# quadram-institute-bioscience/uvaia

Hardware: AMD Instinct MI355X
Metric: ref-seqs scored/sec (higher is better)
Workload: dtype u32 bit-planes / int32 counts

## Files before the change

### include/uvaia_gpu.h

```cpp
#ifndef UVAIA_GPU_H
#define UVAIA_GPU_H

#include <stddef.h>
#include <stdint.h>

#ifdef __cplusplus
extern "C" {
#endif

#define UVAIA_GPU_NSCORE 6

enum {
  UVAIA_GPU_OK         =  0,
  UVAIA_GPU_EINVAL     = -1,
  UVAIA_GPU_ENODEV     = -2,
  UVAIA_GPU_ENOMEM     = -3,
  UVAIA_GPU_EHIP       = -4,
  UVAIA_GPU_EALPHABET  = -5,
  UVAIA_GPU_ESTATE     = -6
};

typedef struct uvaia_gpu_ctx uvaia_gpu_ctx;

typedef struct {
  int n_query;
  int nchar;
  const char *const *seq;
  const char *consensus;
  const size_t *idx_c, *idx_m, *idx;
  int n_idx_c, n_idx_m, n_idx;
  size_t trim;
  int acgt;
} uvaia_gpu_query;

int uvaia_gpu_open (uvaia_gpu_ctx **ctx, const uvaia_gpu_query *query, int heap_size, int device, size_t max_pool);

enum { UVAIA_GPU_SCAN_AUTO = 0,
       UVAIA_GPU_SCAN_PACKED = 1,
       UVAIA_GPU_SCAN_COMPRESSED = 2,
       UVAIA_GPU_SCAN_WIDE = 3 };
typedef struct {
  size_t subslice_refs;
  int rare_max;
  int scan;
  int serial;
  int scan_tiles_per_wave;
  int scan_waves_per_block;
  int rederive_streams;
  int ball_gather;
  int query_tables;
  int replay_extras;
  int replay_cus;
  int scan_streams;
  int pipeline;
  int head_scan;
} uvaia_gpu_tuning;
int uvaia_gpu_export_query_table (uvaia_gpu_ctx *ctx, int which, void *out, size_t cap, size_t *n_bytes);
int uvaia_gpu_open_tuned (uvaia_gpu_ctx **ctx, const uvaia_gpu_query *query, int heap_size, int device, size_t max_pool, const uvaia_gpu_tuning *tuning );
void uvaia_gpu_close (uvaia_gpu_ctx *ctx);
const char *uvaia_gpu_last_error (const uvaia_gpu_ctx *ctx);

int uvaia_gpu_push (uvaia_gpu_ctx *ctx, const char *const *seq, const int *non_n, int n_ref, int64_t ordinal0,
                    uint8_t *entered);

int uvaia_gpu_drain (uvaia_gpu_ctx *ctx, int *n_items, int *max_incompatible, int *scores, int64_t *ordinals);
int uvaia_gpu_heap_slots (const uvaia_gpu_ctx *ctx);
int uvaia_gpu_n_query (const uvaia_gpu_ctx *ctx);
int uvaia_gpu_reset (uvaia_gpu_ctx *ctx);

int uvaia_gpu_db_reserve (uvaia_gpu_ctx *ctx, size_t n_ref_capacity);
int uvaia_gpu_db_append (uvaia_gpu_ctx *ctx, const char *const *seq, const int *non_n, int n_ref);
int uvaia_gpu_db_append_block (uvaia_gpu_ctx *ctx, const char *rows, size_t pitch, const int *non_n, int n_ref);
size_t uvaia_gpu_db_size (const uvaia_gpu_ctx *ctx);
int uvaia_gpu_search_resident (uvaia_gpu_ctx *ctx, size_t pool, int64_t ordinal0, uint8_t *entered);
int uvaia_gpu_sync (uvaia_gpu_ctx *ctx);

size_t uvaia_gpu_state_bytes (const uvaia_gpu_ctx *ctx);
int uvaia_gpu_state_export (uvaia_gpu_ctx *ctx, void *dst);
int uvaia_gpu_state_import (uvaia_gpu_ctx *ctx, const void *src);
int uvaia_gpu_slice_scan (uvaia_gpu_ctx *ctx, size_t first, size_t n, int buf);
int uvaia_gpu_slice_replay (uvaia_gpu_ctx *ctx, int buf, int64_t ordinal0, int stripe_start);
int uvaia_gpu_slice_buffers (void);
size_t uvaia_gpu_state_range_bytes (const uvaia_gpu_ctx *ctx, int q0, int q1);
int uvaia_gpu_state_export_range (uvaia_gpu_ctx *ctx, void *dst, int q0, int q1);
int uvaia_gpu_state_import_range (uvaia_gpu_ctx *ctx, const void *src, int q0, int q1);
int uvaia_gpu_slice_replay_range (uvaia_gpu_ctx *ctx, int buf, int64_t ordinal0, int q0, int q1, int take_snapshot);
int uvaia_gpu_entered_flags (uvaia_gpu_ctx *ctx, uint8_t *out, int clear);

int uvaia_gpu_ball (uvaia_gpu_ctx *ctx, const char *const *seq, int n_ref, int radius, int *mindist);
int uvaia_gpu_ball_resident (uvaia_gpu_ctx *ctx, size_t first, size_t n, int radius, int *mindist);
int uvaia_gpu_ball_packed (uvaia_gpu_ctx *ctx, const void *planes, int n_ref, int radius, int *mindist);
int uvaia_gpu_unpack_rows (uvaia_gpu_ctx *ctx, const int *index, int n, char *rows, size_t pitch);
unsigned long long uvaia_gpu_ball_asked (uvaia_gpu_ctx *ctx, int reset);
void uvaia_gpu_ball_kernel_ms (uvaia_gpu_ctx *ctx, double out[3], int reset);

int uvaia_gpu_agree_on_polymorphic (uvaia_gpu_ctx *ctx, const char *const *seq, int n_seq, uint8_t *out);

int uvaia_gpu_query_columns (const char *const *seq, int n_query, int nchar, size_t trim, int acgt, int device, char *consensus, unsigned char *some_missing);

int uvaia_gpu_last_batch_scores (uvaia_gpu_ctx *ctx, int *out, int n_ref);
int uvaia_gpu_scan_stats (uvaia_gpu_ctx *ctx, double *ms, long long *launches, double *algorithmic_bytes, int reset);
int uvaia_gpu_replay_stats (uvaia_gpu_ctx *ctx, unsigned long long out[3], int reset);
int uvaia_gpu_replay_tiles_opened (uvaia_gpu_ctx *ctx, unsigned long long *out, int reset);
int uvaia_gpu_replay_timing (uvaia_gpu_ctx *ctx, unsigned long long out[12], int reset);
int uvaia_gpu_set_query_tile (uvaia_gpu_ctx *ctx, int qt);
int uvaia_gpu_set_active_queries (uvaia_gpu_ctx *ctx, int q0, int q1);
int uvaia_gpu_max_tolerance (uvaia_gpu_ctx *ctx, int *out);
int uvaia_gpu_search_resident_pool (uvaia_gpu_ctx *ctx, size_t first, size_t n, int64_t ordinal0, int snapshot);

int uvaia_gpu_db_set_shard (uvaia_gpu_ctx *ctx, int rank, int world, size_t piece_refs);
int uvaia_gpu_shard_rows (const uvaia_gpu_ctx *ctx);
size_t uvaia_gpu_shard_aux_bytes (const uvaia_gpu_ctx *ctx, size_t n_tiles);
int uvaia_gpu_shard_scan (uvaia_gpu_ctx *ctx, size_t first, size_t n, void *cnt, void *tmin, void *aux);
int uvaia_gpu_db_skip (uvaia_gpu_ctx *ctx, size_t n_ref);
int uvaia_gpu_shard_set_peer (uvaia_gpu_ctx *ctx, int rank, const void *planes, const void *side_rows);
const void *uvaia_gpu_shard_planes (const uvaia_gpu_ctx *ctx);
const void *uvaia_gpu_shard_side_rows (const uvaia_gpu_ctx *ctx);
int uvaia_gpu_shard_ipc_handle_bytes (void);
int uvaia_gpu_shard_ipc_handles (uvaia_gpu_ctx *ctx, void *out );
int uvaia_gpu_shard_ipc_open (uvaia_gpu_ctx *ctx, int rank, const void *handles);
int uvaia_gpu_shard_ipc_close (uvaia_gpu_ctx *ctx);
int uvaia_gpu_scan_wait (uvaia_gpu_ctx *ctx);
int uvaia_gpu_replay_wait (uvaia_gpu_ctx *ctx);
int uvaia_gpu_set_snapshot (uvaia_gpu_ctx *ctx, int snapshot);
enum { UVAIA_GPU_SCANS = 0, UVAIA_GPU_REPLAYS = 1 };
int uvaia_gpu_mark (uvaia_gpu_ctx *ctx, int what, int slot);
int uvaia_gpu_stream_wait_mark (uvaia_gpu_ctx *ctx, void *stream, int slot);
int uvaia_gpu_wait_stream (uvaia_gpu_ctx *ctx, int what, void *stream);
int uvaia_gpu_shard_replay (uvaia_gpu_ctx *ctx, const void *cnt, const void *tmin, const void *aux, int owner, size_t first, size_t n, int64_t ordinal0, int q0, int q1);

typedef struct uvaia_gpu_group uvaia_gpu_group;
int  uvaia_gpu_group_open (uvaia_gpu_group **group, const uvaia_gpu_query *query, int heap_size, const int *devices, int n_devices, size_t max_pool, size_t piece_refs);
void uvaia_gpu_group_close (uvaia_gpu_group *group);
const char *uvaia_gpu_group_last_error (const uvaia_gpu_group *group);
int  uvaia_gpu_group_size (const uvaia_gpu_group *group);
uvaia_gpu_ctx *uvaia_gpu_group_member (uvaia_gpu_group *group, int i);
int  uvaia_gpu_group_query_shard (const uvaia_gpu_group *group, int i, int *q0, int *q1);
int  uvaia_gpu_group_db_reserve (uvaia_gpu_group *group, size_t n_ref_capacity);
int  uvaia_gpu_group_db_append (uvaia_gpu_group *group, const char *const *seq, const int *non_n, int n_ref);
int  uvaia_gpu_group_db_append_packed (uvaia_gpu_group *group, const void *planes, const int *non_n, const int *side_rows, int n_ref);
int  uvaia_gpu_group_db_clear (uvaia_gpu_group *group);
int  uvaia_gpu_group_db_rederive (uvaia_gpu_group *group);
size_t uvaia_gpu_group_db_size (const uvaia_gpu_group *group);
int  uvaia_gpu_group_reset (uvaia_gpu_group *group);
int  uvaia_gpu_group_search_resident (uvaia_gpu_group *group, size_t pool, int64_t ordinal0, uint8_t *entered);
int  uvaia_gpu_group_push (uvaia_gpu_group *group, const char *const *seq, const int *non_n, int n_ref, int64_t ordinal0, uint8_t *entered);
int  uvaia_gpu_group_drain (uvaia_gpu_group *group, int *n_items, int *max_incompatible, int *scores, int64_t *ordinals);
int  uvaia_gpu_group_sync (uvaia_gpu_group *group);

size_t uvaia_gpu_db_tile_bytes (const uvaia_gpu_ctx *ctx);
int    uvaia_gpu_db_clear (uvaia_gpu_ctx *ctx);
int    uvaia_gpu_db_rederive (uvaia_gpu_ctx *ctx);
int    uvaia_gpu_db_side_row_ints (void);
int    uvaia_gpu_db_export (uvaia_gpu_ctx *ctx, size_t first_tile, size_t n_tiles, void *planes, int *non_n, int *side_rows);
int    uvaia_gpu_db_append_packed (uvaia_gpu_ctx *ctx, const void *planes, const int *non_n, const int *side_rows, int n_ref);

int uvaia_gpu_db_stage_reserve (uvaia_gpu_ctx *ctx, size_t n_tiles);
int uvaia_gpu_db_stage_packed (uvaia_gpu_ctx *ctx, int slot, const void *planes, const int *non_n, const int *side_rows, int n_tiles);
int uvaia_gpu_db_load_staged (uvaia_gpu_ctx *ctx, int slot, const int *sel, int n_ref);
int uvaia_gpu_db_stage_packed_at (uvaia_gpu_ctx *ctx, int slot, size_t tile_offset, const void *planes, const int *non_n, const int *side_rows, int n_tiles);
int uvaia_gpu_db_append_staged (uvaia_gpu_ctx *ctx, int slot, const int *sel, int n_ref);
int uvaia_gpu_db_unpack_rows (uvaia_gpu_ctx *ctx, const int *index, int n, char *rows, size_t pitch);
void uvaia_gpu_window_ms (uvaia_gpu_ctx *ctx, double out[3], int reset);
size_t uvaia_gpu_free_bytes (uvaia_gpu_ctx *ctx);

int uvaia_gpu_rows_census (uvaia_gpu_ctx *ctx, const void *d_rows, size_t pitch, int n, int *non_n, int *n_exc);
int uvaia_gpu_db_append_device (uvaia_gpu_ctx *ctx, const void *d_rows, size_t pitch, const int *row_index, int n_sel, const int *non_n);
int uvaia_gpu_rows_exceptions (uvaia_gpu_ctx *ctx, const void *d_rows, size_t pitch, const int *row_index, int n_sel, const uint64_t *offsets, void *exc_out);
int uvaia_gpu_db_drop_tiles (uvaia_gpu_ctx *ctx, size_t n_tiles);
void uvaia_gpu_rows_kernel_ms (uvaia_gpu_ctx *ctx, double out[3], int reset);
int uvaia_gpu_rows_set_run_cut (uvaia_gpu_ctx *ctx, unsigned cut);

size_t uvaia_gpu_scan_bytes_per_ref (const uvaia_gpu_ctx *ctx);
int uvaia_gpu_scan_variant (const uvaia_gpu_ctx *ctx);
size_t uvaia_gpu_derived_bytes_per_ref (const uvaia_gpu_ctx *ctx);
size_t uvaia_gpu_packed_bytes_per_ref (const uvaia_gpu_ctx *ctx);

#ifdef __cplusplus
}
#endif
#endif
```

### uvaia_amd/capi.py

```python
import ctypes as C
import os
import subprocess

import numpy as np

_HERE = os.path.dirname(os.path.abspath(__file__))
ROOT = os.path.dirname(_HERE)
_LIB = os.path.join(_HERE, "lib", "libuvaia_gpu.so")
NSCORE = 6

SYMBOLS = [
    "uvaia_gpu_open", "uvaia_gpu_open_tuned", "uvaia_gpu_close", "uvaia_gpu_last_error", "uvaia_gpu_push", "uvaia_gpu_drain",
    "uvaia_gpu_heap_slots", "uvaia_gpu_n_query", "uvaia_gpu_reset", "uvaia_gpu_db_reserve", "uvaia_gpu_db_append",
    "uvaia_gpu_db_append_block", "uvaia_gpu_db_size", "uvaia_gpu_search_resident", "uvaia_gpu_sync", "uvaia_gpu_ball", "uvaia_gpu_ball_resident", "uvaia_gpu_ball_packed", "uvaia_gpu_unpack_rows", "uvaia_gpu_ball_asked", "uvaia_gpu_ball_kernel_ms", "uvaia_gpu_export_query_table", "uvaia_gpu_agree_on_polymorphic", "uvaia_gpu_query_columns",
    "uvaia_gpu_last_batch_scores", "uvaia_gpu_scan_stats", "uvaia_gpu_replay_stats", "uvaia_gpu_replay_tiles_opened", "uvaia_gpu_replay_timing",
    "uvaia_gpu_state_bytes", "uvaia_gpu_state_export", "uvaia_gpu_state_import", "uvaia_gpu_slice_scan", "uvaia_gpu_slice_replay",
    "uvaia_gpu_entered_flags", "uvaia_gpu_state_range_bytes", "uvaia_gpu_state_export_range", "uvaia_gpu_state_import_range",
    "uvaia_gpu_slice_replay_range", "uvaia_gpu_slice_buffers", "uvaia_gpu_scan_bytes_per_ref", "uvaia_gpu_derived_bytes_per_ref", "uvaia_gpu_scan_variant", "uvaia_gpu_set_query_tile", "uvaia_gpu_packed_bytes_per_ref",
    "uvaia_gpu_db_tile_bytes", "uvaia_gpu_db_side_row_ints", "uvaia_gpu_db_export", "uvaia_gpu_db_append_packed", "uvaia_gpu_db_clear", "uvaia_gpu_db_rederive",
    "uvaia_gpu_set_active_queries", "uvaia_gpu_max_tolerance", "uvaia_gpu_search_resident_pool",
    "uvaia_gpu_db_set_shard", "uvaia_gpu_shard_rows", "uvaia_gpu_shard_scan", "uvaia_gpu_scan_wait", "uvaia_gpu_replay_wait", "uvaia_gpu_set_snapshot", "uvaia_gpu_shard_replay",
    "uvaia_gpu_mark", "uvaia_gpu_stream_wait_mark", "uvaia_gpu_wait_stream",
    "uvaia_gpu_shard_aux_bytes", "uvaia_gpu_db_skip", "uvaia_gpu_shard_set_peer", "uvaia_gpu_shard_planes", "uvaia_gpu_shard_side_rows",
    "uvaia_gpu_shard_ipc_handle_bytes", "uvaia_gpu_shard_ipc_handles", "uvaia_gpu_shard_ipc_open", "uvaia_gpu_shard_ipc_close",
    "uvaia_gpu_group_open", "uvaia_gpu_group_close", "uvaia_gpu_group_last_error", "uvaia_gpu_group_size", "uvaia_gpu_group_member", "uvaia_gpu_group_query_shard",
    "uvaia_gpu_group_db_reserve", "uvaia_gpu_group_db_append", "uvaia_gpu_group_db_append_packed", "uvaia_gpu_group_db_clear", "uvaia_gpu_group_db_rederive",
    "uvaia_gpu_group_db_size", "uvaia_gpu_group_reset", "uvaia_gpu_group_search_resident", "uvaia_gpu_group_push", "uvaia_gpu_group_drain", "uvaia_gpu_group_sync",
    "uvaia_gpu_rows_census", "uvaia_gpu_db_append_device", "uvaia_gpu_rows_exceptions", "uvaia_gpu_db_drop_tiles", "uvaia_gpu_rows_kernel_ms", "uvaia_gpu_rows_set_run_cut",
    "uvaia_gpu_db_stage_reserve", "uvaia_gpu_db_stage_packed", "uvaia_gpu_db_load_staged", "uvaia_gpu_db_unpack_rows", "uvaia_gpu_window_ms", "uvaia_gpu_free_bytes",
    "uvaia_gpu_db_stage_packed_at", "uvaia_gpu_db_append_staged",
]


class GpuError(RuntimeError):
    def __init__(self, code, msg):
        super().__init__("uvaia_gpu error %d: %s" % (code, msg))
        self.code = code


class Tuning(C.Structure):
    _fields_ = [("subslice_refs", C.c_size_t), ("rare_max", C.c_int), ("scan", C.c_int), ("serial", C.c_int),
                ("scan_tiles_per_wave", C.c_int), ("scan_waves_per_block", C.c_int), ("rederive_streams", C.c_int), ("ball_gather", C.c_int), ("query_tables", C.c_int), ("replay_extras", C.c_int), ("replay_cus", C.c_int), ("scan_streams", C.c_int), ("pipeline", C.c_int), ("head_scan", C.c_int)]

    SCAN = {"auto": 0, "packed": 1, "compressed": 2, "wide": 3}

    @classmethod
    def make(cls, tuning):
        if tuning is None or isinstance(tuning, cls):
            return tuning
        t = cls()
        for k, v in tuning.items():
            setattr(t, k, cls.SCAN[v] if k == "scan" and isinstance(v, str) else int(v))
        return t


class _Query(C.Structure):
    _fields_ = [
        ("n_query", C.c_int), ("nchar", C.c_int),
        ("seq", C.POINTER(C.c_char_p)), ("consensus", C.c_char_p),
        ("idx_c", C.POINTER(C.c_size_t)), ("idx_m", C.POINTER(C.c_size_t)), ("idx", C.POINTER(C.c_size_t)),
        ("n_idx_c", C.c_int), ("n_idx_m", C.c_int), ("n_idx", C.c_int),
        ("trim", C.c_size_t), ("acgt", C.c_int),
    ]


def library_path():
    return _LIB


def build_library(force=False):
    csrc = os.path.join(_HERE, "csrc")
    srcs = [os.path.join(csrc, f) for f in os.listdir(csrc) if f.endswith((".hip", ".inc"))] + [os.path.join(ROOT, "include", "uvaia_gpu.h")]
    if not force and os.path.exists(_LIB) and os.path.getmtime(_LIB) >= max(os.path.getmtime(f) for f in srcs):
        return _LIB
    subprocess.check_call(["make", "-C", os.path.join(_HERE, "csrc"), "-s"])
    return _LIB


_lib = None


def load_library():
    global _lib
    if _lib is not None:
        return _lib
    if not os.path.exists(_LIB):
        raise GpuError(-2, "HIP library %s is missing: run __graft_entry__.build() (no CPU fallback exists)" % _LIB)
    L = C.CDLL(_LIB)
    vp = C.c_void_p
    pp = C.POINTER(C.c_char_p)
    pi = C.POINTER(C.c_int)
    sig = {
        "uvaia_gpu_open": (C.c_int, [C.POINTER(vp), C.POINTER(_Query), C.c_int, C.c_int, C.c_size_t]),
        "uvaia_gpu_open_tuned": (C.c_int, [C.POINTER(vp), C.POINTER(_Query), C.c_int, C.c_int, C.c_size_t, C.POINTER(Tuning)]),
        "uvaia_gpu_close": (None, [vp]),
        "uvaia_gpu_last_error": (C.c_char_p, [vp]),
        "uvaia_gpu_push": (C.c_int, [vp, pp, pi, C.c_int, C.c_int64, C.POINTER(C.c_uint8)]),
        "uvaia_gpu_drain": (C.c_int, [vp, pi, pi, pi, C.POINTER(C.c_int64)]),
        "uvaia_gpu_heap_slots": (C.c_int, [vp]),
        "uvaia_gpu_n_query": (C.c_int, [vp]),
        "uvaia_gpu_reset": (C.c_int, [vp]),
        "uvaia_gpu_db_reserve": (C.c_int, [vp, C.c_size_t]),
        "uvaia_gpu_db_append": (C.c_int, [vp, pp, pi, C.c_int]),
        "uvaia_gpu_db_append_block": (C.c_int, [vp, C.c_void_p, C.c_size_t, pi, C.c_int]),
        "uvaia_gpu_db_size": (C.c_size_t, [vp]),
        "uvaia_gpu_search_resident": (C.c_int, [vp, C.c_size_t, C.c_int64, C.POINTER(C.c_uint8)]),
        "uvaia_gpu_sync": (C.c_int, [vp]),
        "uvaia_gpu_ball": (C.c_int, [vp, pp, C.c_int, C.c_int, pi]),
        "uvaia_gpu_ball_resident": (C.c_int, [vp, C.c_size_t, C.c_size_t, C.c_int, pi]),
        "uvaia_gpu_ball_packed": (C.c_int, [vp, C.c_void_p, C.c_int, C.c_int, pi]),
        "uvaia_gpu_unpack_rows": (C.c_int, [vp, pi, C.c_int, C.c_void_p, C.c_size_t]),
        "uvaia_gpu_ball_asked": (C.c_ulonglong, [vp, C.c_int]),
        "uvaia_gpu_ball_kernel_ms": (None, [vp, C.POINTER(C.c_double), C.c_int]),
        "uvaia_gpu_export_query_table": (C.c_int, [vp, C.c_int, vp, C.c_size_t, C.POINTER(C.c_size_t)]),
        "uvaia_gpu_agree_on_polymorphic": (C.c_int, [vp, pp, C.c_int, C.POINTER(C.c_uint8)]),
        "uvaia_gpu_query_columns": (C.c_int, [pp, C.c_int, C.c_int, C.c_size_t, C.c_int, C.c_int, C.c_char_p, C.POINTER(C.c_uint8)]),
        "uvaia_gpu_last_batch_scores": (C.c_int, [vp, pi, C.c_int]),
        "uvaia_gpu_scan_stats": (C.c_int, [vp, C.POINTER(C.c_double), C.POINTER(C.c_longlong), C.POINTER(C.c_double), C.c_int]),
        "uvaia_gpu_replay_stats": (C.c_int, [vp, C.POINTER(C.c_ulonglong), C.c_int]),
        "uvaia_gpu_replay_tiles_opened": (C.c_int, [vp, C.POINTER(C.c_ulonglong), C.c_int]),
        "uvaia_gpu_replay_timing": (C.c_int, [vp, C.POINTER(C.c_ulonglong), C.c_int]),
        "uvaia_gpu_state_bytes": (C.c_size_t, [vp]),
        "uvaia_gpu_state_export": (C.c_int, [vp, C.c_void_p]),
        "uvaia_gpu_state_import": (C.c_int, [vp, C.c_void_p]),
        "uvaia_gpu_slice_scan": (C.c_int, [vp, C.c_size_t, C.c_size_t, C.c_int]),
        "uvaia_gpu_slice_replay": (C.c_int, [vp, C.c_int, C.c_int64, C.c_int]),
        "uvaia_gpu_entered_flags": (C.c_int, [vp, C.POINTER(C.c_uint8), C.c_int]),
        "uvaia_gpu_state_range_bytes": (C.c_size_t, [vp, C.c_int, C.c_int]),
        "uvaia_gpu_state_export_range": (C.c_int, [vp, C.c_void_p, C.c_int, C.c_int]),
        "uvaia_gpu_state_import_range": (C.c_int, [vp, C.c_void_p, C.c_int, C.c_int]),
        "uvaia_gpu_slice_replay_range": (C.c_int, [vp, C.c_int, C.c_int64, C.c_int, C.c_int, C.c_int]),
        "uvaia_gpu_slice_buffers": (C.c_int, []),
        "uvaia_gpu_scan_bytes_per_ref": (C.c_size_t, [vp]),
        "uvaia_gpu_derived_bytes_per_ref": (C.c_size_t, [vp]),
        "uvaia_gpu_scan_variant": (C.c_int, [vp]),
        "uvaia_gpu_set_query_tile": (C.c_int, [vp, C.c_int]),
        "uvaia_gpu_packed_bytes_per_ref": (C.c_size_t, [vp]),
        "uvaia_gpu_set_active_queries": (C.c_int, [vp, C.c_int, C.c_int]),
        "uvaia_gpu_max_tolerance": (C.c_int, [vp, pi]),
        "uvaia_gpu_search_resident_pool": (C.c_int, [vp, C.c_size_t, C.c_size_t, C.c_int64, C.c_int]),
        "uvaia_gpu_db_tile_bytes": (C.c_size_t, [vp]),
        "uvaia_gpu_db_clear": (C.c_int, [vp]),
        "uvaia_gpu_db_rederive": (C.c_int, [vp]),
        "uvaia_gpu_db_side_row_ints": (C.c_int, []),
        "uvaia_gpu_db_export": (C.c_int, [vp, C.c_size_t, C.c_size_t, C.c_void_p, pi, pi]),
        "uvaia_gpu_db_append_packed": (C.c_int, [vp, C.c_void_p, pi, pi, C.c_int]),
        "uvaia_gpu_db_set_shard": (C.c_int, [vp, C.c_int, C.c_int, C.c_size_t]),
        "uvaia_gpu_shard_rows": (C.c_int, [vp]),
        "uvaia_gpu_shard_scan": (C.c_int, [vp, C.c_size_t, C.c_size_t, C.c_void_p, C.c_void_p, C.c_void_p]),
        "uvaia_gpu_shard_aux_bytes": (C.c_size_t, [vp, C.c_size_t]), "uvaia_gpu_db_skip": (C.c_int, [vp, C.c_size_t]),
        "uvaia_gpu_shard_set_peer": (C.c_int, [vp, C.c_int, C.c_void_p, C.c_void_p]),
        "uvaia_gpu_shard_planes": (C.c_void_p, [vp]), "uvaia_gpu_shard_side_rows": (C.c_void_p, [vp]),
        "uvaia_gpu_shard_ipc_handle_bytes": (C.c_int, []), "uvaia_gpu_shard_ipc_handles": (C.c_int, [vp, C.c_void_p]),
        "uvaia_gpu_shard_ipc_open": (C.c_int, [vp, C.c_int, C.c_void_p]), "uvaia_gpu_shard_ipc_close": (C.c_int, [vp]),
        "uvaia_gpu_scan_wait": (C.c_int, [vp]),
        "uvaia_gpu_replay_wait": (C.c_int, [vp]),
        "uvaia_gpu_set_snapshot": (C.c_int, [vp, C.c_int]),
        "uvaia_gpu_shard_replay": (C.c_int, [vp, C.c_void_p, C.c_void_p, C.c_void_p, C.c_int, C.c_size_t, C.c_size_t, C.c_int64, C.c_int, C.c_int]),
        "uvaia_gpu_mark": (C.c_int, [vp, C.c_int, C.c_int]), "uvaia_gpu_stream_wait_mark": (C.c_int, [vp, C.c_void_p, C.c_int]),
        "uvaia_gpu_wait_stream": (C.c_int, [vp, C.c_int, C.c_void_p]),
        "uvaia_gpu_group_open": (C.c_int, [C.POINTER(vp), C.POINTER(_Query), C.c_int, pi, C.c_int, C.c_size_t, C.c_size_t]),
        "uvaia_gpu_group_close": (None, [vp]),
        "uvaia_gpu_group_last_error": (C.c_char_p, [vp]),
        "uvaia_gpu_group_size": (C.c_int, [vp]),
        "uvaia_gpu_group_member": (vp, [vp, C.c_int]),
        "uvaia_gpu_group_query_shard": (C.c_int, [vp, C.c_int, pi, pi]),
        "uvaia_gpu_group_db_reserve": (C.c_int, [vp, C.c_size_t]),
        "uvaia_gpu_group_db_append": (C.c_int, [vp, pp, pi, C.c_int]),
        "uvaia_gpu_group_db_append_packed": (C.c_int, [vp, C.c_void_p, pi, pi, C.c_int]),
        "uvaia_gpu_group_db_clear": (C.c_int, [vp]),
        "uvaia_gpu_group_db_rederive": (C.c_int, [vp]),
        "uvaia_gpu_group_db_size": (C.c_size_t, [vp]),
        "uvaia_gpu_group_reset": (C.c_int, [vp]),
        "uvaia_gpu_group_search_resident": (C.c_int, [vp, C.c_size_t, C.c_int64, C.POINTER(C.c_uint8)]),
        "uvaia_gpu_group_push": (C.c_int, [vp, pp, pi, C.c_int, C.c_int64, C.POINTER(C.c_uint8)]),
        "uvaia_gpu_group_drain": (C.c_int, [vp, pi, pi, pi, C.POINTER(C.c_int64)]),
        "uvaia_gpu_group_sync": (C.c_int, [vp]),
        "uvaia_gpu_rows_census": (C.c_int, [vp, C.c_void_p, C.c_size_t, C.c_int, pi, pi]),
        "uvaia_gpu_db_append_device": (C.c_int, [vp, C.c_void_p, C.c_size_t, pi, C.c_int, pi]),
        "uvaia_gpu_rows_exceptions": (C.c_int, [vp, C.c_void_p, C.c_size_t, pi, C.c_int, C.POINTER(C.c_uint64), C.c_void_p]),
        "uvaia_gpu_db_drop_tiles": (C.c_int, [vp, C.c_size_t]),
        "uvaia_gpu_rows_kernel_ms": (None, [vp, C.POINTER(C.c_double), C.c_int]),
        "uvaia_gpu_rows_set_run_cut": (C.c_int, [vp, C.c_uint]),
        "uvaia_gpu_db_stage_reserve": (C.c_int, [vp, C.c_size_t]),
        "uvaia_gpu_db_stage_packed": (C.c_int, [vp, C.c_int, C.c_void_p, pi, pi, C.c_int]),
        "uvaia_gpu_db_load_staged": (C.c_int, [vp, C.c_int, pi, C.c_int]),
        "uvaia_gpu_db_stage_packed_at": (C.c_int, [vp, C.c_int, C.c_size_t, C.c_void_p, pi, pi, C.c_int]),
        "uvaia_gpu_db_append_staged": (C.c_int, [vp, C.c_int, pi, C.c_int]),
        "uvaia_gpu_db_unpack_rows": (C.c_int, [vp, pi, C.c_int, C.c_void_p, C.c_size_t]),
        "uvaia_gpu_window_ms": (None, [vp, C.POINTER(C.c_double), C.c_int]),
        "uvaia_gpu_free_bytes": (C.c_size_t, [vp]),
    }
    for name, (res, args) in sig.items():
        fn = getattr(L, name)
        fn.restype, fn.argtypes = res, args
    _lib = L
# ... 361 lines not shown
        self._staged[int(slot)] = (planes, non_n, side_rows)
        self._chk(self.L.uvaia_gpu_db_stage_packed(self.ctx, int(slot), planes.ctypes.data, non_n.ctypes.data_as(C.POINTER(C.c_int)),
                                                   side_rows.ctypes.data_as(C.POINTER(C.c_int)), int(n_tiles)))

    def db_load_staged(self, slot, sel, n_ref):
        _k, sp = _int_ptr(sel)
        self._chk(self.L.uvaia_gpu_db_load_staged(self.ctx, int(slot), sp, int(n_ref)))

    def db_stage_packed_at(self, slot, tile_offset, planes, non_n, side_rows, n_tiles):
        planes = np.ascontiguousarray(planes, dtype=np.uint8)
        non_n = np.ascontiguousarray(non_n, dtype=np.int32)
        side_rows = np.ascontiguousarray(side_rows, dtype=np.int32)
        tb = self.L.uvaia_gpu_db_tile_bytes(self.ctx)
        if planes.size < int(n_tiles) * tb or non_n.size < int(n_tiles) * 64 or side_rows.size < int(n_tiles) * 64 * self.L.uvaia_gpu_db_side_row_ints():
            raise ValueError("arrays shorter than %d tiles" % n_tiles)
        if not hasattr(self, "_staged_at"):
            self._staged_at = {}
        if int(tile_offset) == 0:
            self._staged_at[int(slot)] = []
        self._staged_at.setdefault(int(slot), []).append((planes, non_n, side_rows))
        self._chk(self.L.uvaia_gpu_db_stage_packed_at(self.ctx, int(slot), int(tile_offset), planes.ctypes.data, non_n.ctypes.data_as(C.POINTER(C.c_int)),
                                                      side_rows.ctypes.data_as(C.POINTER(C.c_int)), int(n_tiles)))

    def db_append_staged(self, slot, sel, n_ref):
        _k, sp = _int_ptr(sel)
        self._chk(self.L.uvaia_gpu_db_append_staged(self.ctx, int(slot), sp, int(n_ref)))

    def db_unpack_rows(self, index, pitch=None):
        idx = np.ascontiguousarray(index, dtype=np.int32)
        pitch = (self.nchar + 15) // 16 * 16 if pitch is None else int(pitch)
        rows = np.zeros((max(len(idx), 1), pitch), dtype=np.uint8)
        self._chk(self.L.uvaia_gpu_db_unpack_rows(self.ctx, idx.ctypes.data_as(C.POINTER(C.c_int)), len(idx), rows.ctypes.data, pitch))
        return [rows[k, :self.nchar].tobytes() for k in range(len(idx))]

    def window_ms(self, reset=False):
        out = (C.c_double * 3)()
        self.L.uvaia_gpu_window_ms(self.ctx, out, int(reset))
        return tuple(out)

    def free_bytes(self):
        return int(self.L.uvaia_gpu_free_bytes(self.ctx))

    def ball_asked(self, reset=False):
        return int(self.L.uvaia_gpu_ball_asked(self.ctx, int(reset)))

    def query_table(self, which):
        n = C.c_size_t(0)
        self._chk(self.L.uvaia_gpu_export_query_table(self.ctx, int(which), None, 0, C.byref(n)))
        out = np.zeros(n.value, dtype=np.uint8)
        if n.value:
            self._chk(self.L.uvaia_gpu_export_query_table(self.ctx, int(which), out.ctypes.data_as(C.c_void_p), n.value, C.byref(n)))
        return out

    def ball_kernel_ms(self, reset=False):
        out = (C.c_double * 3)()
        self.L.uvaia_gpu_ball_kernel_ms(self.ctx, out, int(reset))
        return tuple(out)


def finalise_heaps(n, scores, ordinals):
    out = []
    for q in range(len(n)):
        k = int(n[q])
        order = ([k] + list(range(1, k))) if k else []
        rows = [(tuple(int(x) for x in scores[q, s]), int(ordinals[q, s])) for s in order]
        rows.sort(key=lambda r: tuple(-v for v in r[0]))
        out.append(rows)
    return out


class Group:

    def __init__(self, q, devices, nbest=100, max_pool=4096, piece_refs=0):
        self.L = load_library()
        self.nq, self.nchar = len(q.seqs), len(q.consensus)
        self._keep = [_cstrs(q.seqs), q.consensus,
                      (C.c_size_t * len(q.idx_c))(*[int(x) for x in q.idx_c]),
                      (C.c_size_t * len(q.idx_m))(*[int(x) for x in q.idx_m]),
                      (C.c_size_t * len(q.idx))(*[int(x) for x in q.idx])]
        qq = _Query(self.nq, self.nchar, self._keep[0], q.consensus, self._keep[2], self._keep[3], self._keep[4],
                    len(q.idx_c), len(q.idx_m), len(q.idx), int(q.trim), int(bool(q.acgt)))
        self.g = C.c_void_p()
        dev = (C.c_int * len(devices))(*[int(d) for d in devices])
        rc = self.L.uvaia_gpu_group_open(C.byref(self.g), C.byref(qq), int(nbest), dev, len(devices), int(max_pool), int(piece_refs))
        if rc != 0:
            msg = self.L.uvaia_gpu_group_last_error(None)
            self.g = None
            raise GpuError(rc, msg.decode() if msg else "?")
        self.slots = self.L.uvaia_gpu_heap_slots(self.L.uvaia_gpu_group_member(self.g, 0))

    def _chk(self, rc):
        if rc != 0:
            msg = self.L.uvaia_gpu_group_last_error(self.g)
            raise GpuError(rc, msg.decode() if msg else "?")

    def close(self):
        if getattr(self, "g", None):
            self.L.uvaia_gpu_group_close(self.g)
            self.g = None

    def __enter__(self):
        return self

    def __exit__(self, *a):
        self.close()

# ... 68 lines not shown
```

### uvaia_amd/csrc/host_batch.inc

```

extern "C" {

int uvaia_gpu_agree_on_polymorphic(uvaia_gpu_ctx *c, const char *const *seq, int n_seq, uint8_t *out)
{
  if (!c) return UVAIA_GPU_EINVAL;
  if (n_seq < 0 || (n_seq > 0 && (!seq || !out))) return fail(c, UVAIA_GPU_EINVAL, "bad batch");
  if ((size_t)n_seq > c->max_pool) return fail(c, UVAIA_GPU_ESTATE, "batch of %d exceeds max_pool %zu", n_seq, c->max_pool);
  if (n_seq == 0) return 0;
  int rc = ensure_batch_buffers(c); if (rc) return rc;
  rc = pack_rows(c, seq, nullptr, 0, nullptr, n_seq, c->batch, 0);
  if (rc) return rc;
  const int n_tiles = (n_seq + 63) / 64, ppad = n_tiles * 64;
  rc = ensure_cnt4(c, (size_t)c->nq_pad * c->pool_pad); if (rc) return rc;
  const bool prof = c->profile; c->profile = false;
  rc = ensure_qpoly(c); if (rc) return rc;
  rc = launch_scan(c, c->batch, 0, n_tiles, c->d_qpoly, c->nq, c->d_cnt, ppad, 0.0);
  c->profile = prof;
  if (rc) return rc;
  uint8_t *d_out = nullptr;
  const size_t bytes = (size_t)n_seq * c->nq;
  HIPCHK(c, hipMalloc(&d_out, bytes));
  dim3 grid((n_seq + 255) / 256, c->nq);
  if (c->acgt) hipLaunchKernelGGL((agree_kernel<true>), grid, dim3(256), 0, c->stream, c->d_cnt, ppad, c->nq, n_seq, d_out);
  else         hipLaunchKernelGGL((agree_kernel<false>), grid, dim3(256), 0, c->stream, c->d_cnt, ppad, c->nq, n_seq, d_out);
// ... 35 lines not shown
  QCHK(hipMalloc(&d_first, (size_t)nchar)); QCHK(hipMalloc(&d_flags, (size_t)nchar));
  QCHK(hipMemsetAsync(d_first, 'N', (size_t)nchar, st)); QCHK(hipMemsetAsync(d_flags, 0, (size_t)nchar, st));
  for (int i = 0; i < 2; i++) QCHK(hipEventCreateWithFlags(&freed[i], hipEventDisableTiming));
  const unsigned gx = (unsigned)((hi - lo + 255) / 256);
  int k = 0;
  for (int a = 0; a < n_query; a += batch, k++) {
    const int m = std::min(batch, n_query - a), b = k & 1;
    if (k >= 2) QCHK(hipEventSynchronize(freed[b]));
    uint8_t *hb = h_rows + (size_t)b * batch * pitch, *db = d_rows + (size_t)b * batch * pitch;
    for (int i = 0; i < m; i++) if (!seq[a + i]) return done(fail(nullptr, UVAIA_GPU_EINVAL, "query %d is NULL", a + i));
    parallel_for(m, [&](int i) { memcpy(hb + (size_t)i * pitch, seq[a + i], (size_t)nchar); });
    QCHK(hipMemcpyAsync(db, hb, (size_t)m * pitch, hipMemcpyHostToDevice, st));
    const int ng = (m + 63) / 64;
    hipLaunchKernelGGL(query_columns_partial_kernel, dim3(gx, (unsigned)ng), dim3(256), 0, st, db, pitch, m, lo, hi, acgt ? 1 : 0, d_pf, d_pl, nchar);
    hipLaunchKernelGGL(query_columns_merge_kernel, dim3(gx), dim3(256), 0, st, d_pf, d_pl, ng, lo, hi, nchar, d_first, d_flags);
    QCHK(hipGetLastError());
    QCHK(hipEventRecord(freed[b], st));
  }
  std::vector<uint8_t> first((size_t)nchar), flags((size_t)nchar);
  QCHK(hipMemcpyAsync(first.data(), d_first, (size_t)nchar, hipMemcpyDeviceToHost, st));
  QCHK(hipMemcpyAsync(flags.data(), d_flags, (size_t)nchar, hipMemcpyDeviceToHost, st));
  QCHK(hipStreamSynchronize(st));
#undef QCHK
  for (int c = lo; c < hi; c++) {
    consensus[c] = (flags[(size_t)c] & 1) ? '#' : (char)first[(size_t)c];
    some_missing[c] = (flags[(size_t)c] & 2) ? 1 : 0;
  }
  return done(0);
}

int uvaia_gpu_push(uvaia_gpu_ctx *c, const char *const *seq, const int *non_n, int n_ref, int64_t ordinal0, uint8_t *entered)
{
  if (!c) return UVAIA_GPU_EINVAL;
  if (n_ref < 0 || (n_ref > 0 && !seq)) return fail(c, UVAIA_GPU_EINVAL, "bad batch");
  if ((size_t)n_ref > c->max_pool) return fail(c, UVAIA_GPU_ESTATE, "batch of %d exceeds max_pool %zu", n_ref, c->max_pool);
  if (c->act_q0 != 0 || c->act_q1 != c->nq) return fail(c, UVAIA_GPU_ESTATE, "streamed batches act on the whole query set: query shards use the resident calls");
  if (n_ref == 0) return 0;
  int rc = ensure_batch_buffers(c); if (rc) return rc;
  rc = pack_rows(c, seq, nullptr, 0, non_n, n_ref, c->batch, 0);
  if (rc) return rc;
  const int n_tiles = (n_ref + 63) / 64;
  HIPCHK(c, hipMemsetAsync(c->d_entered, 0, (size_t)n_tiles * 64, c->stream));
  rc = run_batch(c, c->batch, 0, n_tiles, 0, n_ref, ordinal0);
  if (rc) return rc;
  if (entered) HIPCHK(c, hipMemcpyAsync(entered, c->d_entered, (size_t)n_ref, hipMemcpyDeviceToHost, c->stream));
  HIPCHK(c, hipStreamSynchronize(c->stream));
  return collect_events(c);
}

int uvaia_gpu_drain(uvaia_gpu_ctx *c, int *n_items, int *max_incompatible, int *scores, int64_t *ordinals)
{
  if (!c || !n_items || !scores || !ordinals) return c ? fail(c, UVAIA_GPU_EINVAL, "NULL output") : UVAIA_GPU_EINVAL;
  HIPCHK(c, hipStreamSynchronize(c->stream));
  const size_t ne = (size_t)c->nq * (c->k + 1);
  std::vector<int> h(ne * HEAP_ENTRY), T(c->nq);
  HIPCHK(c, hipMemcpy(h.data(), c->d_heap, h.size() * sizeof(int), hipMemcpyDeviceToHost));
  HIPCHK(c, hipMemcpy(n_items, c->d_n, (size_t)c->nq * sizeof(int), hipMemcpyDeviceToHost));
  HIPCHK(c, hipMemcpy(T.data(), c->d_T, (size_t)c->nq * sizeof(int), hipMemcpyDeviceToHost));
  for (size_t e = 0; e < ne; e++) {
    for (int s = 0; s < 6; s++) scores[e * 6 + s] = h[e * HEAP_ENTRY + s];
    ordinals[e] = (int64_t)(((uint64_t)(uint32_t)h[e * HEAP_ENTRY + 7] << 32) | (uint32_t)h[e * HEAP_ENTRY + 6]);
  }
  if (max_incompatible) memcpy(max_incompatible, T.data(), (size_t)c->nq * sizeof(int));
  return collect_events(c);
}


}
```

### uvaia_amd/csrc/host_launch.inc

```

namespace {

template <class F>
static void parallel_for(int n, F f)
{
  const unsigned nt = std::min<unsigned>(std::max(1u, std::thread::hardware_concurrency()), 64u);
  if (n < 32 || nt < 2) { for (int i = 0; i < n; i++) f(i); return; }
  std::atomic<int> next(0);
  std::vector<std::thread> th;
  for (unsigned t = 0; t < nt; t++) th.emplace_back([&]() { for (;;) { const int a = next.fetch_add(4); if (a >= n) break; for (int i = a; i < std::min(n, a + 4); i++) f(i); } });
  for (auto &x : th) x.join();
}

__global__ void mask_query_planes_kernel(const uint32_t *__restrict__ qp, const uint32_t *__restrict__ pmask, uint32_t *__restrict__ out, size_t n_words_total, int words_per_row, int nq_planes)
{
  const size_t i = (size_t)blockIdx.x * blockDim.x + threadIdx.x;
  if (i >= n_words_total) return;
  const int w = (int)((i / (size_t)nq_planes) % (size_t)words_per_row);
  out[i] = qp[i] & pmask[w];
}

int ensure_qpoly(uvaia_gpu_ctx *c)
{
  if (c->d_qpoly) return 0;
// ... 78 lines not shown
int store_alloc(uvaia_gpu_ctx *c, TileStore &s, size_t tiles)
{
  store_free(s);
  uint4 *planes = nullptr;
  const size_t refs = tiles * 64, tile_u4 = (size_t)c->W4 * c->P * 64;
  HIPCHK(c, hipMalloc(&s.nonn, refs * sizeof(int)));
  HIPCHK(c, hipMemset(s.nonn, 0, refs * sizeof(int)));
  HIPCHK(c, hipMalloc(&s.ev, tiles * (size_t)c->W4 * 2 * 64 * sizeof(uint4)));
  HIPCHK(c, hipMalloc(&s.grp, tiles * (size_t)c->W4 * 64 * sizeof(uint32_t)));
  HIPCHK(c, hipMalloc(&s.poly, tiles * (size_t)std::max(c->NP4 + c->NR4, 1) * 3 * 64 * sizeof(uint4)));
  HIPCHK(c, hipMalloc(&s.tote, refs * sizeof(int)));
  HIPCHK(c, hipMalloc(&s.tot, refs * sizeof(int)));
  HIPCHK(c, hipMemset(s.tot, 0, refs * sizeof(int)));
  HIPCHK(c, hipMalloc(&s.amb, refs * AMB_ROW * sizeof(int)));
  HIPCHK(c, hipMemset(s.amb, 0, refs * AMB_ROW * sizeof(int)));
  HIPCHK(c, hipMalloc(&planes, tiles * tile_u4 * sizeof(uint4)));
  HIPCHK(c, hipMemset(planes, 0, tiles * tile_u4 * sizeof(uint4)));
  s.planes = planes;
  return 0;
}

int ensure_batch_buffers(uvaia_gpu_ctx *c)
{
  if (c->batch.planes) return 0;
  HIPCHK(c, hipSetDevice(c->device));
  return store_alloc(c, c->batch, c->pool_pad / 64);
}

int pack_query_row(const uint8_t *code_tab, const char *row, int nchar, int lo, int hi, const uint8_t *keep, const uint8_t *is_poly,
                   bool acgt, int NQ, uint32_t *dst, int *bad_byte)
{
  for (int s = lo; s < hi; s++) {
    if (keep && !keep[s]) continue;
    const uint8_t code = code_tab[(unsigned char)row[s]];
    if (code == 0xFF) { *bad_byte = (unsigned char)row[s]; return -1; }
    if (!code) continue;
    const int w = s >> 5, b = s & 31;
    uint32_t *d = dst + (size_t)w * NQ;
    const bool one = (code & (code - 1)) == 0;
    if (acgt) {
      if (!one) continue;
      const uint32_t two = code == 2 ? 1u : code == 4 ? 2u : code == 8 ? 3u : 0u;
      d[0] |= (two & 1u) << b; d[1] |= (two >> 1) << b; d[2] |= 1u << b;
      if (is_poly && is_poly[s]) d[3] |= 1u << b;
    } else {
      for (int p = 0; p < 4; p++) d[p] |= (uint32_t)((code >> p) & 1u) << b;
      d[4] |= 1u << b;
      if (one) d[5] |= 1u << b;
    }
  }
  return 0;
}

int take_scan_events(uvaia_gpu_ctx *c, ScanEvt &ev)
{
  for (hipEvent_t *e : {&ev.a, &ev.b}) {
    if (!c->ev_pool.empty()) { *e = c->ev_pool.back(); c->ev_pool.pop_back(); }
    else HIPCHK(c, hipEventCreate(e));
  }
  return 0;
}

int launch_scan(uvaia_gpu_ctx *c, const TileStore &s, long long tile_first, int n_tiles, const uint32_t *qp, int n_rows, int4 *out, int ppad, double bytes)
{
  if (n_tiles <= 0) return 0;
  dim3 grid((unsigned)((n_rows + c->qt - 1) / c->qt), (unsigned)((n_tiles + 3) / 4)), block(256);
  ScanEvt ev{};
  if (c->profile) {
    { int rc_ = take_scan_events(c, ev); if (rc_) return rc_; }
    HIPCHK(c, hipEventRecord(ev.a, c->stream));
  }
#define LAUNCH(K, QT) hipLaunchKernelGGL((K<QT>), grid, block, 0, c->stream, s.planes, tile_first, n_tiles, c->W4, qp, out, ppad)
  if (c->acgt) { switch (c->qt) { case 8: LAUNCH(scan_acgt_kernel, 8); break; case 32: LAUNCH(scan_acgt_kernel, 32); break; default: LAUNCH(scan_acgt_kernel, 16); } }
  else         { switch (c->qt) { case 8: LAUNCH(scan_iupac_kernel, 8); break; case 32: LAUNCH(scan_iupac_kernel, 32); break; default: LAUNCH(scan_iupac_kernel, 16); } }
#undef LAUNCH
  HIPCHK(c, hipGetLastError());
  if (c->profile) { HIPCHK(c, hipEventRecord(ev.b, c->stream)); ev.bytes = bytes; c->evts.push_back(ev); }
  return 0;
}

int launch_pair_extras(uvaia_gpu_ctx *c, const TileStore &s, long long tile_first, int n_tiles, uint32_t *ext, int ppad, hipStream_t stream)
{
  if (n_tiles <= 0) return 0;
  hipLaunchKernelGGL(pair_extras_kernel, dim3((unsigned)n_tiles, (unsigned)((c->nq + 15) / 16)), dim3(256), 0, stream, s.planes, tile_first, n_tiles, c->W4,
                     s.amb, c->d_qp, c->d_amb_q, c->nq, ext, ppad);
  HIPCHK(c, hipGetLastError());
  return 0;
}

int launch_scan2(uvaia_gpu_ctx *c, const TileStore &s, long long tile_first, int n_tiles, uint32_t *out, int ppad, double bytes, hipStream_t stream,
                 int2 *tmin, int r_lo, int r_hi, int4 *rt, uint32_t *ext = nullptr , uint32_t *rtp = nullptr, uint4 *tb8 = nullptr,
                 unsigned *progress = nullptr )
{
  if (n_tiles <= 0) return 0;
  if (!stream) stream = c->stream;
  const bool cons = c->n_idx_c > 0;
  if (cons && !rt) return fail(c, UVAIA_GPU_ESTATE, "no buffer for the consensus pre-score");
  const uint4 *tiles = s.planes; const int *tot_tile0 = s.tot + tile_first * 64;
  const long long ptile_first = tile_first;
  auto consensus_rt = [&]() {
    if (!cons) return;
    if (c->acgt) hipLaunchKernelGGL((consensus_rt_kernel<true>), dim3((n_tiles + 3) / 4), dim3(256), 0, stream, tiles, ptile_first, n_tiles, c->W4, c->d_cp, rt);
    else         hipLaunchKernelGGL((consensus_rt_kernel<false>), dim3((n_tiles + 3) / 4), dim3(256), 0, stream, tiles, ptile_first, n_tiles, c->W4, c->d_cp, rt);
  };
  const int qt2 = c->qt != 8 ? 16 : c->nq <= 1 ? 1 : c->nq <= 2 ? 2 : c->nq <= 4 ? 4 : 8;
  const int n_qtiles = (c->nq + qt2 - 1) / qt2;
  dim3 grid(scan_grid_size(n_qtiles, n_tiles)), block(256);
  ScanEvt ev_{};
  if (c->profile) {
    { int rc_ = take_scan_events(c, ev_); if (rc_) return rc_; }
    HIPCHK(c, hipEventRecord(ev_.a, stream));
  }
  const uint32_t *qp = c->acgt ? c->d_qp : c->d_qp2;
  if (c->scan_variant == 2) {
    const int *tote = s.tote + tile_first * 64;
    constexpr int QS = 64;
    if (c->act_q0 % QS) return fail(c, UVAIA_GPU_ESTATE, "the scan works on super-tiles of %d queries: active queries start at a multiple of that", QS);
    const int st_first = c->act_q0 / QS, n_st = (c->act_q1 + QS - 1) / QS - st_first;
    const int R = c->scan_R;
    dim3 grid3(scan_grid_size(n_st, (n_tiles + R - 1) / R));
#define SCAN3_LAUNCH(NWW, A, RR) hipLaunchKernelGGL((scan3_kernel<NWW, A, RR>), grid3, dim3(64 * NWW), 0, stream, s.ev, s.poly, tile_first, n_tiles, c->W4, c->NP4, c->NP4 + c->NR4, c->d_qpl, c->d_stream, c->d_sdir, s.grp, tote, tot_tile0, out, ppad, n_st, tmin, r_lo, r_hi, st_first, progress)
#define SCAN3_NW(A, RR) { if (c->scan_NW == 8) SCAN3_LAUNCH(8, A, RR); else SCAN3_LAUNCH(4, A, RR); }
    if (progress) { consensus_rt(); HIPCHK(c, hipGetLastError()); }
    if (R == 4)      { if (c->acgt) SCAN3_LAUNCH(8, true, 4); else SCAN3_LAUNCH(8, false, 4); }
    else if (R == 2) { if (c->acgt) SCAN3_NW(true, 2) else SCAN3_NW(false, 2) }
    else             { if (c->acgt) SCAN3_NW(true, 1) else SCAN3_NW(false, 1) }
#undef SCAN3_NW
#undef SCAN3_LAUNCH
    HIPCHK(c, hipGetLastError());
    if (c->profile) { HIPCHK(c, hipEventRecord(ev_.b, stream)); ev_.bytes = bytes; c->evts.push_back(ev_); }
    if (!progress) consensus_rt();
    HIPCHK(c, hipGetLastError());
    if (tb8 && !c->acgt) {
      hipLaunchKernelGGL(tile_bounds_kernel, dim3((unsigned)n_tiles), dim3(256), 0, stream, out, ppad, n_tiles, c->nq, r_lo, r_hi, tb8, cons ? rt : (const int4 *)nullptr, rtp);
      HIPCHK(c, hipGetLastError());
      if (ext) { int rc_ = launch_pair_extras(c, s, ptile_first, n_tiles, ext, ppad, stream); if (rc_) return rc_; }
    }
    return 0;
  }
  const int *amb0 = s.amb;
#define LAUNCH(K, QT, CN) hipLaunchKernelGGL((K<QT, CN>), grid, block, 0, stream, tiles, tile_first, n_tiles, c->W4, qp, out, ppad, n_qtiles, tot_tile0, tmin, r_lo, r_hi, c->d_cp, rt)
#define LAUNCHX(K, QT, CN) hipLaunchKernelGGL((K<QT, CN>), grid, block, 0, stream, tiles, tile_first, n_tiles, c->W4, qp, out, ppad, n_qtiles, tot_tile0, tmin, r_lo, r_hi, c->d_cp, rt, ext, rtp, tb8, amb0, c->d_qp, c->d_amb_q, c->nq)
#define LAUNCH_QT(L, K, CN) switch (qt2) { case 1: L(K, 1, CN); break; case 2: L(K, 2, CN); break; case 4: L(K, 4, CN); break; case 8: L(K, 8, CN); break; default: L(K, 16, CN); }
  if (c->acgt) { if (cons) { LAUNCH_QT(LAUNCH, scan2_acgt_kernel, true) } else { LAUNCH_QT(LAUNCH, scan2_acgt_kernel, false) } }
  else         { if (cons) { LAUNCH_QT(LAUNCHX, scan2_iupac_kernel, true) } else { LAUNCH_QT(LAUNCHX, scan2_iupac_kernel, false) } }
#undef LAUNCH_QT
#undef LAUNCHX
#undef LAUNCH
  HIPCHK(c, hipGetLastError());
  if (c->profile) { HIPCHK(c, hipEventRecord(ev_.b, stream)); ev_.bytes = bytes; c->evts.push_back(ev_); }
  return 0;
}

size_t replay3_lds_bytes(const uvaia_gpu_ctx *c)
{ return (size_t)(c->k + 1) * HEAP_ENTRY * sizeof(int) + 128 + (size_t)16 * 1024 + (size_t)2 * c->replay_half * (c->n_idx_c > 0 ? 4 : 3) * 256; }
int ensure_cnt4(uvaia_gpu_ctx *c, size_t elems)
{
  if (c->cnt_cap >= elems) return 0;
  if (c->d_cnt) { HIPCHK(c, hipFree(c->d_cnt)); c->d_cnt = nullptr; c->cnt_cap = 0; }
  HIPCHK(c, hipMalloc(&c->d_cnt, elems * sizeof(int4)));
  c->cnt_cap = elems;
  return 0;
}

int collect_events(uvaia_gpu_ctx *c)
{
  for (auto &e : c->evts) {
    HIPCHK(c, hipEventSynchronize(e.b));
    float ms = 0; HIPCHK(c, hipEventElapsedTime(&ms, e.a, e.b));
    c->scan_ms += ms; c->scan_bytes += e.bytes; c->scan_launches++;
    c->ev_pool.push_back(e.a); c->ev_pool.push_back(e.b);
  }
  c->evts.clear();
  return 0;
}

struct ReplayLaunch {
  hipStream_t stream; int q0, q1;
  const uint32_t *cnt, *ext; int ppad; const int4 *rt; const uint32_t *rtp; const int2 *tmin; const uint4 *tb8;
  const uint4 *planes; long long tile_first; const int *nonn, *amb; uint8_t *entered;
  int rb, re; long long ord_base;
  const uint32_t *qpl; const uint4 *poly; int nr4; const uint32_t *qrare;
  int prefetch;
  const unsigned *progress; unsigned blocks_per_group; int scan_R; int *pipe_err;
};
int launch_replay(uvaia_gpu_ctx *c, const ReplayLaunch &L)
{
  const dim3 grid(L.q1 - L.q0), block(64);
  const size_t lds = (size_t)(c->k + 1) * HEAP_ENTRY * sizeof(int);
  if (c->fullscan) {
#define REPLAY(A) hipLaunchKernelGGL((replay_kernel<A>), grid, block, lds, L.stream, c->d_cnt, L.ppad, c->d_rt, c->d_tr, L.nonn, L.rb, L.re, L.ord_base, c->d_heap, c->d_n, c->d_T, c->d_snap, L.entered, c->k)
    if (c->acgt) REPLAY(true); else REPLAY(false);
#undef REPLAY
  } else if (L.ext) {
#define REPLAY3(B, H) hipLaunchKernelGGL((replay3_kernel<B, H>), grid, block, replay3_lds_bytes(c), L.stream, L.cnt, L.ext, L.ppad, L.rt, L.rtp, c->d_cp, L.nonn, L.amb, L.rb, L.re, L.ord_base, \
                                         c->d_heap, c->d_n, c->d_T, c->d_snap, L.entered, c->k, L.planes, L.tile_first, c->W4, c->d_qp, c->d_amb_q, c->d_stats, L.q0, L.tb8, c->replay_prio)
#define REPLAY3_HALF(B) { if (c->replay_half == 32) REPLAY3(B, 32); else if (c->replay_half == 16) REPLAY3(B, 16); else REPLAY3(B, 8); }
    if (c->n_idx_c > 0) REPLAY3_HALF(true) else REPLAY3_HALF(false)
#undef REPLAY3_HALF
#undef REPLAY3
  } else {
    const int lq_words = (c->replay_lq && !c->acgt && lds + (size_t)c->W4 * 4 * 6 * 4 + 128 <= 64 * 1024) ? c->W4 * 4 * 6 : 0;
    const int2 *tmin = (c->scan_variant == 2 || c->scan_variant == 0) ? L.tmin : nullptr;
#define REPLAY2(A, B, PF_) hipLaunchKernelGGL((replay2_kernel<A, B, PF_>), grid, block, lds + (size_t)lq_words * 4 + 128, L.stream, L.cnt, L.ppad, L.rt, c->d_cp, L.nonn, L.amb, L.rb, L.re, L.ord_base, \
                                              c->d_heap, c->d_n, c->d_T, c->d_snap, L.entered, c->k, L.planes, L.tile_first, c->W4, c->d_qp, c->d_amb_q, c->d_stats, L.q0, tmin, L.qpl, lq_words, c->replay_prio, \
                                              L.poly, c->NP4 + c->NR4, c->NP4, L.nr4, L.qrare, L.progress, L.blocks_per_group, L.scan_R, L.pipe_err)
#define REPLAY2_PF(A, B) { if (L.prefetch == 1) REPLAY2(A, B, 1); else if (L.prefetch == 2) REPLAY2(A, B, 2); else REPLAY2(A, B, 3); }
    if (c->acgt) { if (c->n_idx_c > 0) REPLAY2_PF(true, true) else REPLAY2_PF(true, false) }
    else         { if (c->n_idx_c > 0) REPLAY2_PF(false, true) else REPLAY2_PF(false, false) }
#undef REPLAY2_PF
#undef REPLAY2
  }
  HIPCHK(c, hipGetLastError());
  return 0;
}

int run_batch(uvaia_gpu_ctx *c, const TileStore &s, long long tile_first, int n_tiles, int r_begin, int r_end,
              long long ord_base, size_t cnt4_cols = 0 )
{
  if (r_end <= r_begin) return 0;
  const int ppad = n_tiles * 64;
  const SliceBuf &b = c->slice[0];
  hipLaunchKernelGGL(snapshot_kernel, dim3(1), dim3(256), 0, c->stream, c->d_T, c->nq, c->d_snap);
  if (c->n_idx_c > 0 && c->fullscan) {
    if (c->acgt) hipLaunchKernelGGL((consensus_kernel<true>), dim3((n_tiles + 3) / 4), dim3(256), 0, c->stream, s.planes, tile_first, n_tiles, c->W4, c->d_cp, c->d_snap, c->d_rt, c->d_tr);
    else         hipLaunchKernelGGL((consensus_kernel<false>), dim3((n_tiles + 3) / 4), dim3(256), 0, c->stream, s.planes, tile_first, n_tiles, c->W4, c->d_cp, c->d_snap, c->d_rt, c->d_tr);
  }
  HIPCHK(c, hipGetLastError());
  const double bytes = (double)(r_end - r_begin) * (double)c->W4 * 16.0 * c->P + (double)c->nq * (double)c->W4 * 16.0 * c->P;
  uint32_t *ext = c->use_ext ? b.ext : nullptr;
  int rc = 0;
  if (c->fullscan) {
    rc = ensure_cnt4(c, (size_t)c->nq_pad * (cnt4_cols ? std::max<size_t>(cnt4_cols, (size_t)ppad) : c->pool_pad)); if (rc) return rc;
    rc = launch_scan(c, s, tile_first, n_tiles, c->d_qp, c->nq, c->d_cnt, ppad, bytes);
  } else rc = launch_scan2(c, s, tile_first, n_tiles, b.cnt, ppad, bytes, nullptr, b.tmin, r_begin, r_end, b.rt, ext, b.rtp, b.tb8);
  if (rc) return rc;
  rc = launch_replay(c, {c->stream, 0, c->nq, b.cnt, ext, ppad, b.rt, b.rtp, b.tmin, b.tb8,
                             s.planes, tile_first, s.nonn + tile_first * 64, s.amb + tile_first * 64 * AMB_ROW, c->d_entered + tile_first * 64, r_begin, r_end, ord_base,
                             c->scan_variant == 2 ? c->d_qpl : nullptr, s.poly, c->NR4, c->d_qrare, 3, nullptr, 0, 2, nullptr});
  if (rc) return rc;
  c->last = {&s, tile_first, n_tiles, r_end - r_begin, r_begin, ppad, c->fullscan ? c->d_rt : b.rt};
  return 0;
}

int derive_rows(uvaia_gpu_ctx *c, const TileStore &s, long long slot0, int n_ref, hipStream_t st = nullptr, bool v_in_place = false)
{
  if (!st) st = c->stream;
  if (c->fullscan || c->scan_variant != 2 || n_ref <= 0 || !c->d_split) return 0;
  const long long a = slot0 / 64, t1 = (slot0 + n_ref - 1) / 64;
  const int nblk = (int)(t1 - a + 1);
#define DERIVE_ALL(A, V) hipLaunchKernelGGL((derive_all_kernel<A, V>), dim3(nblk), dim3(256), 0, st, s.planes, a, a, c->W4, c->d_cls, c->d_rmask, c->d_split, c->NP4, c->NR4, s.ev, s.tote, s.grp, s.poly)
  if (c->acgt) { if (v_in_place) DERIVE_ALL(true, false); else DERIVE_ALL(true, true); }
  else         { if (v_in_place) DERIVE_ALL(false, false); else DERIVE_ALL(false, true); }
#undef DERIVE_ALL
  HIPCHK(c, hipGetLastError());
  return 0;
}

int sync_scan_streams(uvaia_gpu_ctx *c) { for (hipStream_t st : c->scan_streams) if (st) HIPCHK(c, hipStreamSynchronize(st)); return 0; }
int sync_derive_streams(uvaia_gpu_ctx *c) { for (hipStream_t st : c->derive_streams) if (st) HIPCHK(c, hipStreamSynchronize(st)); return 0; }

template <class T> int regrow(uvaia_gpu_ctx *c, T *&p, size_t n) { if (p) hipFree(p); p = nullptr; HIPCHK(c, hipMalloc(&p, n * sizeof(T))); return 0; }

int slice_reserve(uvaia_gpu_ctx *c, SliceBuf &b, size_t need, size_t ppad)
{
  need = std::max(need, b.cap);
  if (need <= b.cap && b.tmin) return 0;
  if (int rc = sync_scan_streams(c)) return rc;
  HIPCHK(c, hipStreamSynchronize(c->stream));
  const size_t cap = std::max(need, (size_t)c->nq_pad * c->pool_pad), refs = std::max(cap / (size_t)c->nq_pad, ppad) + 64;
  if (cap > b.cap || !b.cnt) { if (int rc = regrow(c, b.cnt, cap)) return rc; }
  if (int rc = regrow(c, b.tmin, cap / 64)) return rc;
  if (c->use_ext) {
    if (int rc = regrow(c, b.ext, cap)) return rc;
    if (int rc = regrow(c, b.tb8, cap / 64)) return rc;
    if (int rc = regrow(c, b.rtp, refs)) return rc;
  }
  if (int rc = regrow(c, b.rt, refs)) return rc;
  b.cap = cap;
  return 0;
}

static int settle_derive(uvaia_gpu_ctx *c)
{
  if (c->derive_pending) { if (int rc = sync_derive_streams(c)) return rc; c->derive_pending = 0; }
  return 0;
}

int pack_rows(uvaia_gpu_ctx *c, const char *const *seq, const char *rows, size_t rows_pitch, const int *non_n, int n_ref, const TileStore &s, long long slot0)
{
  for (int done = 0, k = 0; done < n_ref; done += PACK_CHUNK, k ^= 1) {
    const int m = std::min(PACK_CHUNK, n_ref - done);
    if (c->stage_busy[k]) { HIPCHK(c, hipEventSynchronize(c->stage_free[k])); c->stage_busy[k] = false; }
    uint8_t *hs = c->h_stage + (size_t)k * PACK_CHUNK * c->pitch, *ds = c->d_stage + (size_t)k * PACK_CHUNK * c->pitch;
    for (int i = 0; i < m; i++) if (!(seq ? seq[done + i] : rows)) return fail(c, UVAIA_GPU_EINVAL, "NULL sequence at position %d", done + i);
    parallel_for(m, [&](int i) {
      const char *src = seq ? seq[done + i] : rows + (size_t)(done + i) * rows_pitch;
      memcpy(hs + (size_t)i * c->pitch, src, (size_t)c->nchar);
    });
    HIPCHK(c, hipMemcpyAsync(ds, hs, (size_t)m * c->pitch, hipMemcpyHostToDevice, c->stream));
    const long long s0 = slot0 + done, t0 = s0 / 64, t1 = (s0 + m - 1) / 64;
    const int nblk = (int)(t1 - t0 + 1);
    int *nn_out = non_n ? nullptr : s.nonn;
    if (c->acgt) hipLaunchKernelGGL((pack_refs_kernel<3>), dim3(nblk), dim3(256), 0, c->stream, ds, c->pitch, c->nchar, s0, m, c->W4, s.planes, t0, nn_out, (int *)nullptr, s.tot, c->d_err);
    else         hipLaunchKernelGGL((pack_refs_kernel<4>), dim3(nblk), dim3(256), 0, c->stream, ds, c->pitch, c->nchar, s0, m, c->W4, s.planes, t0, nn_out, s.amb, s.tot, c->d_err);
    HIPCHK(c, hipGetLastError());
    if (non_n) HIPCHK(c, hipMemcpyAsync(s.nonn + s0, non_n + done, (size_t)m * sizeof(int), hipMemcpyHostToDevice, c->stream));
    HIPCHK(c, hipEventRecord(c->stage_free[k], c->stream)); c->stage_busy[k] = true;
  }
  { int rc = derive_rows(c, s, slot0, n_ref); if (rc) return rc; }
  HIPCHK(c, hipStreamSynchronize(c->stream));
  int bad = 0;
  HIPCHK(c, hipMemcpy(&bad, c->d_err, sizeof(int), hipMemcpyDeviceToHost));
  if (bad) {
    HIPCHK(c, hipMemset(c->d_err, 0, sizeof(int)));
    return fail(c, UVAIA_GPU_EALPHABET, "a reference sequence holds a byte outside ACGT / MRWSYKVHDB / NX-?O.");
  }
  return 0;
}

}
```

### uvaia_amd/csrc/host_open.inc

```

extern "C" {

const char *uvaia_gpu_last_error(const uvaia_gpu_ctx *ctx) { return ctx ? ctx->err.c_str() : g_open_error.c_str(); }

void uvaia_gpu_close(uvaia_gpu_ctx *c)
{
  if (!c) return;
  if (c->stream) hipStreamSynchronize(c->stream);
  for (auto &e : c->evts) { hipEventDestroy(e.a); hipEventDestroy(e.b); }
  for (hipEvent_t e : c->ev_pool) hipEventDestroy(e);
  for (hipEvent_t e : c->rows_evs) hipEventDestroy(e);
  void *dev[] = {c->d_idx_cols, c->d_qg, c->d_ball_masks, c->d_ball_key, c->d_split, c->d_qrare, c->d_rmask, c->d_cls, c->d_qpl, c->d_stream, c->d_sdir, c->d_mindist, c->d_ball_list, c->d_ball_cdist, c->d_ball_n, c->d_ball_tiles, c->d_ball_ga,
                 c->d_qp2, c->d_amb_q, c->d_stats, c->d_qp, c->d_cp, c->d_cpm, c->d_qpoly, c->d_pmask, c->d_heap, c->d_n, c->d_T, c->d_snap, c->d_err, c->d_cnt, c->d_rt, c->d_tr, c->d_entered, c->d_stage, c->d_pipe_err, c->d_pk, c->d_rows, c->d_row_idx, c->d_rsel, c->d_rcnt, c->d_roff, c->d_rexc, c->d_wsel, c->d_win4};
  for (void *p : dev) if (p) hipFree(p);
  store_free(c->batch); store_free(c->db);
  for (SliceBuf &b : c->slice) slice_free(b);
  if (c->h_stage) hipHostFree(c->h_stage);
  for (int i = 0; i < 2; i++) if (c->stage_free[i]) hipEventDestroy(c->stage_free[i]);
  for (int i = 0; i < 16; i++) if (c->order_ev[i]) hipEventDestroy(c->order_ev[i]);
  for (int i = 0; i < 4; i++) if (c->ball_ev[i]) hipEventDestroy(c->ball_ev[i]);
  if (c->copy_stream) { hipStreamSynchronize(c->copy_stream); hipStreamDestroy(c->copy_stream); }
  for (auto &sl : c->wstage) { for (void *p : {(void *)sl.planes, (void *)sl.nonn, (void *)sl.side}) if (p) hipFree(p); for (hipEvent_t e : {sl.copied, sl.read}) if (e) hipEventDestroy(e); }
  for (int i = 0; i < 5; i++) if (c->win_ev[i]) hipEventDestroy(c->win_ev[i]);
  for (int i = 0; i < 64; i++) for (int j = 0; j < 2; j++) if (c->ipc_opened[i][j]) hipIpcCloseMemHandle(c->ipc_opened[i][j]);
  for (int i = 0; i < 8; i++) for (int j = 0; j < 3; j++) if (c->mark_ev[i][j]) hipEventDestroy(c->mark_ev[i][j]);
  for (int i_ = 0; i_ < 3; i_++) if (c->derive_streams[i_]) { hipStreamSynchronize(c->derive_streams[i_]); hipStreamDestroy(c->derive_streams[i_]); }
  for (auto &d : c->derive_chunks) hipEventDestroy(d.done);
  for (int i = 0; i < 4; i++) if (c->derive_fence[i]) hipEventDestroy(c->derive_fence[i]);
  if (c->scan_stream) hipStreamDestroy(c->scan_stream);
  for (int i = 1; i < 3; i++) if (c->scan_streams[i]) hipStreamDestroy(c->scan_streams[i]);
  if (c->stream) hipStreamDestroy(c->stream);
  if (c->rep_stream) { hipStreamSynchronize(c->rep_stream); hipStreamDestroy(c->rep_stream); }
  for (int i = 0; i < 2; i++) if (c->rep_ev[i]) hipEventDestroy(c->rep_ev[i]);
  delete c;
}

int uvaia_gpu_open(uvaia_gpu_ctx **out, const uvaia_gpu_query *q, int heap_size, int device, size_t max_pool)
{ return uvaia_gpu_open_tuned(out, q, heap_size, device, max_pool, nullptr); }

int uvaia_gpu_open_tuned(uvaia_gpu_ctx **out, const uvaia_gpu_query *q, int heap_size, int device, size_t max_pool, const uvaia_gpu_tuning *tune)
{
  uvaia_gpu_tuning tn;
  memset(&tn, 0, sizeof tn);
  if (tune) tn = *tune;
  if (tn.scan < 0 || tn.scan > UVAIA_GPU_SCAN_WIDE || tn.query_tables < 0 || tn.query_tables > 2 || (tn.scan_tiles_per_wave != 0 && tn.scan_tiles_per_wave != 1 && tn.scan_tiles_per_wave != 2 && tn.scan_tiles_per_wave != 4) ||
      (tn.scan_waves_per_block != 0 && tn.scan_waves_per_block != 4 && tn.scan_waves_per_block != 8) || (tn.subslice_refs != 0 && tn.subslice_refs < 64))
    return fail(nullptr, UVAIA_GPU_EINVAL, "bad tuning values");
  if (!out) return fail(nullptr, UVAIA_GPU_EINVAL, "ctx is NULL");
  *out = nullptr;
  if (!q || q->n_query < 1 || q->nchar < 1 || !q->seq || !q->consensus) return fail(nullptr, UVAIA_GPU_EINVAL, "empty or incomplete query set");
  if ((q->n_idx_c && !q->idx_c) || (q->n_idx_m && !q->idx_m) || (q->n_idx && !q->idx)) return fail(nullptr, UVAIA_GPU_EINVAL, "index arrays missing");
  if (max_pool < 1) return fail(nullptr, UVAIA_GPU_EINVAL, "max_pool must be >= 1");
  int ndev = 0;
  if (hipGetDeviceCount(&ndev) != hipSuccess || ndev < 1) return fail(nullptr, UVAIA_GPU_ENODEV, "no HIP device available: the MI355X engine has no CPU fallback");
  if (device < 0) { if (hipGetDevice(&device) != hipSuccess) device = 0; }
  if (device >= ndev) return fail(nullptr, UVAIA_GPU_ENODEV, "device %d out of range (%d devices)", device, ndev);
  if (hipSetDevice(device) != hipSuccess) return fail(nullptr, UVAIA_GPU_ENODEV, "hipSetDevice(%d) failed", device);

  uvaia_gpu_ctx *c = new uvaia_gpu_ctx();
  c->device = device;
  c->nq = q->n_query; c->act_q0 = 0; c->act_q1 = q->n_query; c->nchar = q->nchar; c->acgt = q->acgt ? 1 : 0; c->trim = q->trim; c->n_idx_c = q->n_idx_c; c->n_idx_m = q->n_idx_m;
  c->P = c->acgt ? 3 : 4; c->NQ = c->acgt ? 4 : 6;
  c->W = (c->nchar + 31) / 32; c->W4 = (c->W + 3) / 4;
  c->k = heap_size < 2 ? 2 : heap_size;
  c->qt = c->nq <= 8 ? 8 : 16;
  c->scan_variant = tn.scan == UVAIA_GPU_SCAN_PACKED ? 0 : tn.scan == UVAIA_GPU_SCAN_COMPRESSED ? 2 : (c->nq <= 32 ? 0 : 2);
  c->fullscan = tn.scan == UVAIA_GPU_SCAN_WIDE;
  c->serial = tn.serial != 0;
  if (tn.scan_tiles_per_wave) c->scan_R = tn.scan_tiles_per_wave;
  if (tn.scan_waves_per_block) c->scan_NW = tn.scan_waves_per_block;
  if (c->scan_R == 4 && c->scan_NW != 8) { delete c; return fail(nullptr, UVAIA_GPU_EINVAL, "four reference tiles per wave go with eight waves per block"); }
  if (tn.subslice_refs) { c->subslice = tn.subslice_refs; c->subslice_forced = true; }
  if (tn.scan_streams >= 1 && tn.scan_streams <= 3) c->scan_nstreams_forced = tn.scan_streams;
  if (tn.scan_streams > 100 && tn.scan_streams < 200) c->first_slice_pct = tn.scan_streams == 199 ? 0 : tn.scan_streams - 100;
  if (tn.pipeline == 2) c->pipeline = true;
  if (tn.head_scan == 2) c->head_full = true;
  if (tn.ball_gather == 1 || tn.ball_gather == 2) c->ball_fused = tn.ball_gather == 2;
  if (tn.rederive_streams >= 1 && tn.rederive_streams <= 3) { c->derive_nstreams = tn.rederive_streams; c->derive_forced = true; }
  if (c->nchar > 49000) c->fullscan = true;
  c->nq_pad = ((c->nq + 127) / 128) * 128;
  c->max_pool = max_pool; c->pool_pad = ((max_pool + 63) / 64) * 64 + 64;
  c->pitch = ((size_t)c->nchar + 63) / 64 * 64;
  if ((size_t)(c->k + 1) * HEAP_ENTRY * sizeof(int) + 128 > 160 * 1024) { delete c; return fail(nullptr, UVAIA_GPU_EINVAL, "nbest=%d does not fit the per-query LDS heap (max 5115)", heap_size); }

#define OPENCHK(call) HIP_TRY(call, { const int rc_ = fail(nullptr, code_, "%s failed: %s", #call, hipGetErrorString(e_)); uvaia_gpu_close(c); return rc_; })
  c->use_ext = !c->fullscan && !c->acgt && tn.replay_extras != 1 && (c->scan_variant == 0 || (c->scan_variant == 2 && c->nq <= 128 && tn.replay_extras == 2));
  {
    int prio_least = 0, prio_greatest = 0;
    OPENCHK(hipDeviceGetStreamPriorityRange(&prio_least, &prio_greatest));
    bool split = false;
    const int want_half = tn.replay_cus >= 1000 ? tn.replay_cus / 1000 : 0, want_cus = tn.replay_cus >= 1000 ? tn.replay_cus % 1000 : tn.replay_cus;
    c->replay_half = (want_half == 32 || want_half == 16 || want_half == 8) ? want_half : c->nq <= 8 ? 32 : c->nq <= 24 ? 16 : 8;
    int per_cu = (int)std::min<size_t>(4, (size_t)160 * 1024 / replay3_lds_bytes(c));
    while (c->use_ext && c->replay_half > 8 && per_cu * 8 < std::min(c->nq, 32)) { c->replay_half /= 2; per_cu = (int)std::min<size_t>(4, (size_t)160 * 1024 / replay3_lds_bytes(c)); }
    if (c->use_ext && replay3_lds_bytes(c) > (size_t)160 * 1024) c->use_ext = false;
    const int rep_cus = want_cus < 0 ? 0 : want_cus > 0 ? want_cus : (c->use_ext && per_cu > 0 ? std::max(8, ((c->nq + per_cu - 1) / per_cu + 7) / 8 * 8) : 0);
    hipDeviceProp_t prop;
    if (rep_cus > 0 && hipGetDeviceProperties(&prop, device) == hipSuccess && prop.multiProcessorCount >= 4 * rep_cus) {
      const int ncu = prop.multiProcessorCount, words = (ncu + 31) / 32;
      std::vector<uint32_t> m_rep((size_t)words, 0u), m_scan((size_t)words, 0u);
      for (int b = 0; b < ncu; b++) (b < rep_cus ? m_rep : m_scan)[(size_t)b >> 5] |= 1u << (b & 31);
      hipStream_t st[7] = {};
      bool ok = hipExtStreamCreateWithCUMask(&st[0], (uint32_t)words, m_rep.data()) == hipSuccess;
      for (int i = 1; i < 7 && ok; i++) ok = hipExtStreamCreateWithCUMask(&st[i], (uint32_t)words, m_scan.data()) == hipSuccess;
      if (ok) ok = hipEventCreateWithFlags(&c->rep_ev[0], hipEventDisableTiming) == hipSuccess && hipEventCreateWithFlags(&c->rep_ev[1], hipEventDisableTiming) == hipSuccess;
      if (ok) {
        c->rep_stream = st[0]; c->scan_stream = st[1]; c->scan_streams[0] = st[1]; c->scan_streams[1] = st[2]; c->scan_streams[2] = st[3];
        for (int i = 0; i < 3; i++) c->derive_streams[i] = st[4 + i];
        split = true; c->replay_cus = rep_cus;
      } else { (void)hipGetLastError(); for (int i = 0; i < 7; i++) if (st[i]) hipStreamDestroy(st[i]); }
    }
    OPENCHK(hipStreamCreateWithPriority(&c->stream, hipStreamNonBlocking, prio_greatest));
    if (!split) {
      OPENCHK(hipStreamCreateWithPriority(&c->scan_stream, hipStreamNonBlocking, prio_least));
      c->scan_streams[0] = c->scan_stream;
      for (int i = 1; i < 3; i++) OPENCHK(hipStreamCreateWithPriority(&c->scan_streams[i], hipStreamNonBlocking, prio_least));
      for (int i = 0; i < 3; i++) OPENCHK(hipStreamCreateWithPriority(&c->derive_streams[i], hipStreamNonBlocking, (prio_least + prio_greatest) / 2));
    }
    for (SliceBuf &b : c->slice) { OPENCHK(hipEventCreateWithFlags(&b.scan_done, hipEventDisableTiming)); OPENCHK(hipEventCreateWithFlags(&b.replay_done, hipEventDisableTiming)); }
    c->derive_stream = c->derive_streams[0];
  }
  uint8_t code_tab[256]; fill_code_table(code_tab);
  OPENCHK(hipMemcpyToSymbol(HIP_SYMBOL(c_code), code_tab, 256));

  const int lo = (int)std::min<size_t>(c->trim, (size_t)c->nchar), hi = std::max(lo, c->nchar - (int)c->trim);
  const size_t row_words = (size_t)c->W4 * 4 * c->NQ;
  std::vector<uint8_t> in_c(c->nchar, 0), in_m(c->nchar, 0), in_p(c->nchar, 0);
  for (int i = 0; i < q->n_idx_c; i++) if (q->idx_c[i] < (size_t)c->nchar) in_c[q->idx_c[i]] = 1;
  for (int i = 0; i < q->n_idx_m; i++) if (q->idx_m[i] < (size_t)c->nchar) in_m[q->idx_m[i]] = 1;
// ... 41 lines not shown
    const size_t l3 = replay3_lds_bytes(c);
    if (l3 > 160 * 1024) { uvaia_gpu_close(c); return fail(nullptr, UVAIA_GPU_EINVAL, "nbest=%d does not fit the LDS of the replay next to its staging buffers", heap_size); }
#define BIGLDS(K, N) OPENCHK(hipFuncSetAttribute(reinterpret_cast<const void *>(&K), hipFuncAttributeMaxDynamicSharedMemorySize, (int)(N)))
    BIGLDS((replay3_kernel<true, 32>), l3); BIGLDS((replay3_kernel<false, 32>), l3); BIGLDS((replay3_kernel<true, 16>), l3);
    BIGLDS((replay3_kernel<false, 16>), l3); BIGLDS((replay3_kernel<true, 8>), l3); BIGLDS((replay3_kernel<false, 8>), l3);
  }
  OPENCHK(hipMalloc(&b0.tmin, (size_t)c->nq_pad * (c->pool_pad / 64) * sizeof(int2)));
  OPENCHK(hipMalloc(&b0.rt, c->pool_pad * sizeof(int4)));
  OPENCHK(hipMemset(b0.rt, 0, c->pool_pad * sizeof(int4)));
  OPENCHK(hipMalloc(&c->d_stats, 16 * sizeof(unsigned long long)));
  OPENCHK(hipMemset(c->d_stats, 0, 16 * sizeof(unsigned long long)));
  OPENCHK(hipMalloc(&c->d_rt, c->pool_pad * sizeof(int4)));
  OPENCHK(hipMalloc(&c->d_tr, c->pool_pad * sizeof(int4)));
  OPENCHK(hipMemset(c->d_rt, 0, c->pool_pad * sizeof(int4)));
  OPENCHK(hipMemset(c->d_tr, 0, c->pool_pad * sizeof(int4)));
  OPENCHK(hipMalloc(&c->d_entered, c->pool_pad)); c->entered_cap = c->pool_pad;
  OPENCHK(hipMemset(c->d_entered, 0, c->pool_pad));
  const size_t lds = (size_t)(c->k + 1) * HEAP_ENTRY * sizeof(int) + 128;
  if (lds > 64 * 1024) {
    BIGLDS(replay_kernel<true>, lds); BIGLDS(replay_kernel<false>, lds);
#define BIGHEAP(PF_) BIGLDS((replay2_kernel<true, true, PF_>), lds); BIGLDS((replay2_kernel<true, false, PF_>), lds); BIGLDS((replay2_kernel<false, true, PF_>), lds); BIGLDS((replay2_kernel<false, false, PF_>), lds)
    BIGHEAP(1); BIGHEAP(2); BIGHEAP(3);
#undef BIGHEAP
  }
#undef BIGLDS
#undef OPENCHK
  int rc = uvaia_gpu_reset(c);
  if (rc) { g_open_error = c->err; uvaia_gpu_close(c); return rc; }
  *out = c;
  return UVAIA_GPU_OK;
}

int uvaia_gpu_export_query_table(uvaia_gpu_ctx *c, int which, void *out, size_t cap, size_t *n_bytes)
{
  if (!c || !n_bytes || which < 0 || which > 10) return UVAIA_GPU_EINVAL;
  if (which == 10) {
    const int v[11] = {c->NP, c->NR, c->NP4, c->NR4, c->rare_max, c->scan_variant, c->need_e_groups, c->need_v_groups, c->need_g_groups, c->need_r_groups, c->replay_lq};
    *n_bytes = sizeof v;
    if (out && cap >= sizeof v) memcpy(out, v, sizeof v);
    return UVAIA_GPU_OK;
  }
  *n_bytes = c->qtab[which].p ? c->qtab[which].n : 0;
  if (out && *n_bytes && cap >= *n_bytes) {
    HIPCHK(c, hipSetDevice(c->device));
    HIPCHK(c, hipStreamSynchronize(c->stream));
    HIPCHK(c, hipMemcpy(out, c->qtab[which].p, *n_bytes, hipMemcpyDeviceToHost));
  }
  return UVAIA_GPU_OK;
}

int uvaia_gpu_reset(uvaia_gpu_ctx *c)
{
  if (!c) return UVAIA_GPU_EINVAL;
  HIPCHK(c, hipMemsetAsync(c->d_heap, 0, (size_t)c->nq * (c->k + 1) * HEAP_ENTRY * sizeof(int), c->stream));
  hipLaunchKernelGGL(init_state_kernel, dim3((c->nq + 255) / 256), dim3(256), 0, c->stream, c->d_T, c->d_n, c->nq, c->nchar);
  HIPCHK(c, hipGetLastError());
  HIPCHK(c, hipMemcpyAsync(c->d_snap, &c->nchar, sizeof(int), hipMemcpyHostToDevice, c->stream));
  if (c->d_entered && c->db_n) HIPCHK(c, hipMemsetAsync(c->d_entered, 0, ((c->db_n + 63) / 64) * 64, c->stream));
  if (int rc = sync_scan_streams(c)) return rc;
  HIPCHK(c, hipStreamSynchronize(c->stream));
  return 0;
}

int uvaia_gpu_heap_slots(const uvaia_gpu_ctx *c) { return c ? c->k : 0; }
int uvaia_gpu_n_query(const uvaia_gpu_ctx *c) { return c ? c->nq : 0; }
size_t uvaia_gpu_packed_bytes_per_ref(const uvaia_gpu_ctx *c) { return c ? (size_t)c->W4 * 16 * c->P : 0; }
size_t uvaia_gpu_scan_bytes_per_ref(const uvaia_gpu_ctx *c)
{
  if (!c) return 0;
  return (c->fullscan || c->scan_variant != 2) ? (size_t)c->W4 * 16 * c->P
                                                : (size_t)(c->need_e_groups + c->need_v_groups) * 16 + (size_t)c->need_g_groups * 4 + (size_t)(c->NP4 + c->need_r_groups) * 16 * 3;
}

int uvaia_gpu_scan_variant(const uvaia_gpu_ctx *c)
{
  return !c ? -2 : c->fullscan ? -1 : c->scan_variant;
}

size_t uvaia_gpu_derived_bytes_per_ref(const uvaia_gpu_ctx *c)
{
  if (!c || c->fullscan || c->scan_variant != 2) return 0;
  return (size_t)c->W4 * 16 + (size_t)c->W4 * 4 + (size_t)(c->NP4 + c->NR4) * 48 + 4;
}

int uvaia_gpu_set_query_tile(uvaia_gpu_ctx *c, int qt)
{
  if (!c) return UVAIA_GPU_EINVAL;
  if (qt == 0) qt = 16;
  if (qt != 8 && qt != 16 && qt != 32) return fail(c, UVAIA_GPU_EINVAL, "query tile must be 8, 16 or 32");
  c->qt = qt;
  return 0;
}


}
```

### uvaia_amd/csrc/host_qprep.inc

```
namespace {

template <typename T>
int qprep_alloc(T **p, size_t n_elems, bool zero, hipStream_t s)
{
  hipError_t e = hipMalloc(p, std::max<size_t>(n_elems, 1) * sizeof(T));
  if (e == hipSuccess && zero) e = hipMemsetAsync(*p, 0, std::max<size_t>(n_elems, 1) * sizeof(T), s);
  if (e != hipSuccess) { *p = nullptr; return fail(nullptr, e == hipErrorOutOfMemory ? UVAIA_GPU_ENOMEM : UVAIA_GPU_EHIP, "query tables: %s", hipGetErrorString(e)); }
  return 0;
}

struct QprepScratch { std::vector<void *> p; ~QprepScratch() { for (void *x : p) if (x) hipFree(x); } };

int build_query_tables_device(uvaia_gpu_ctx *c, const uvaia_gpu_query *q, const uvaia_gpu_tuning &tn, int lo, int hi)
{
#define OPENCHK(call) HIP_TRY(call, return fail(nullptr, code_, "%s failed: %s", #call, hipGetErrorString(e_)))
#define QALLOC(ptr, n, zero) do { const int rc_ = qprep_alloc(&(ptr), (n), (zero), s); if (rc_) return rc_; } while (0)
  hipStream_t s = c->stream;
  const int Wp = c->W4 * 4, nq = c->nq;
  const size_t row_words = (size_t)Wp * c->NQ;
  QprepScratch tmp;
#define TALLOC(ptr, n, zero) do { const int rc_ = qprep_alloc(&(ptr), (n), (zero), s); if (rc_) return rc_; tmp.p.push_back(ptr); } while (0)

  QALLOC(c->d_qp, (size_t)c->nq_pad * row_words, true);
  c->qtab[0] = {c->d_qp, (size_t)c->nq_pad * row_words * 4};
// ... 11 lines not shown
    else         hipLaunchKernelGGL((qprep_pack_rows_kernel<false>), grid, dim3(128), 0, s, ds, c->pitch, m, done, c->nchar, lo, hi, c->d_pmask, Wp, c->d_qp, d_bad);
    OPENCHK(hipGetLastError());
    OPENCHK(hipEventRecord(c->stage_free[k], s)); c->stage_busy[k] = true;
  }
  QALLOC(c->d_amb_q, (size_t)nq * AMB_STRIDE, true);
  c->qtab[2] = {c->d_amb_q, (size_t)nq * AMB_STRIDE * sizeof(int)};
  if (!c->acgt) {
    QALLOC(c->d_qp2, (size_t)c->nq_pad * Wp * 4, true);
    c->qtab[1] = {c->d_qp2, (size_t)c->nq_pad * Wp * 4 * 4};
    hipLaunchKernelGGL(qprep_recode_kernel, dim3((unsigned)nq), dim3(64), 0, s, c->d_qp, Wp, c->d_qp2, c->d_amb_q);
    OPENCHK(hipGetLastError());
  }
  const int n_shares = std::max(1, std::min(64, nq / 32)), per_share = (nq + n_shares - 1) / n_shares;
  uint32_t *d_acc = nullptr; int *d_cnt = nullptr;
  TALLOC(d_acc, (size_t)Wp * 5, true);
  QALLOC(c->d_cls, (size_t)Wp * 4, true);
  QALLOC(c->d_rmask, (size_t)Wp, true);
  c->qtab[3] = {c->d_cls, (size_t)Wp * 4 * 4}; c->qtab[4] = {c->d_rmask, (size_t)Wp * 4};
  {
    dim3 grid((unsigned)((Wp + 63) / 64), (unsigned)n_shares);
    if (c->acgt) hipLaunchKernelGGL((qprep_classes_kernel<true>), grid, dim3(64), 0, s, c->d_qp, nq, Wp, per_share, d_acc);
    else         hipLaunchKernelGGL((qprep_classes_kernel<false>), grid, dim3(64), 0, s, c->d_qp, nq, Wp, per_share, d_acc);
    hipLaunchKernelGGL(qprep_classes_finish_kernel, dim3((unsigned)((Wp + 63) / 64)), dim3(64), 0, s, d_acc, Wp, c->d_cls);
    OPENCHK(hipGetLastError());
  }
  c->rare_max = tn.rare_max > 0 ? tn.rare_max : tn.rare_max < 0 ? 0 : (nq < 64 ? 0 : std::min(64, std::max(4, nq / 64)));
  if (c->fullscan || c->scan_variant != 2) c->rare_max = 0;
  if (c->rare_max > 0) {
    TALLOC(d_cnt, (size_t)Wp * 32 * 4, true);
    dim3 grid((unsigned)((Wp * 32 + 63) / 64), (unsigned)n_shares);
    if (c->acgt) hipLaunchKernelGGL((qprep_rare_count_kernel<true>), grid, dim3(64), 0, s, c->d_qp, nq, Wp, per_share, c->d_cls, d_cnt);
    else         hipLaunchKernelGGL((qprep_rare_count_kernel<false>), grid, dim3(64), 0, s, c->d_qp, nq, Wp, per_share, c->d_cls, d_cnt);
    hipLaunchKernelGGL(qprep_rare_finish_kernel, dim3((unsigned)((Wp * 32 + 63) / 64)), dim3(64), 0, s, d_cnt, Wp, c->rare_max, c->d_cls, c->d_rmask);
    OPENCHK(hipGetLastError());
  }
  std::vector<uint32_t> cls((size_t)Wp * 4), rmask((size_t)Wp);
  unsigned long long bad = ~0ull;
  OPENCHK(hipMemcpyAsync(cls.data(), c->d_cls, cls.size() * 4, hipMemcpyDeviceToHost, s));
  OPENCHK(hipMemcpyAsync(rmask.data(), c->d_rmask, rmask.size() * 4, hipMemcpyDeviceToHost, s));
  OPENCHK(hipMemcpyAsync(&bad, d_bad, sizeof bad, hipMemcpyDeviceToHost, s));
  OPENCHK(hipStreamSynchronize(s));
  c->stage_busy[0] = c->stage_busy[1] = false;
  if (bad != ~0ull) return fail(nullptr, UVAIA_GPU_EALPHABET, "query %d holds byte 0x%02x outside the supported alphabet", (int)(bad >> 40), (unsigned)(bad & 0xFFu));
  std::vector<int> cols_p, cols_r;
  for (int w = 0; w < Wp; w++) {
    for (uint32_t m = cls[(size_t)w * 4 + 3]; m; m &= m - 1) cols_p.push_back(w * 32 + __builtin_ctz(m));
    for (uint32_t m = rmask[(size_t)w]; m; m &= m - 1) cols_r.push_back(w * 32 + __builtin_ctz(m));
  }
  c->NP = (int)cols_p.size(); c->NR = (int)cols_r.size();
  c->NP4 = ((c->NP + 31) / 32 + 3) / 4;
  c->NR4 = ((c->NR + 31) / 32 + 3) / 4;
  if (c->scan_variant == 2 && (size_t)c->NP4 * 128 + (size_t)c->NR4 * 128 > SCAN3_BIAS - 256) c->scan_variant = 0;
  {
    int split[15];
    for (int v = 0; v <= 4; v++) split[v] = (int)((long long)c->W4 * v / 4);
    for (int v = 0; v <= 4; v++) {
      int nd = 0, nr = 0;
      for (int w = 0; w < split[v] * 4; w++) { nd += __builtin_popcount(cls[(size_t)w * 4 + 3]); nr += __builtin_popcount(rmask[(size_t)w]); }
      split[5 + v] = nd; split[10 + v] = nr;
    }
    QALLOC(c->d_split, 15, false);
    OPENCHK(hipMemcpyAsync(c->d_split, split, sizeof split, hipMemcpyHostToDevice, s));
    OPENCHK(hipStreamSynchronize(s));
    c->qtab[9] = {c->d_split, sizeof split};
  }
  const size_t prow = (size_t)std::max(c->NP4, 1) * 16;
  QALLOC(c->d_qpl, (size_t)c->nq_pad * prow, true);
  QALLOC(c->d_qrare, (size_t)nq * std::max(c->NR4, 1) * 12, true);
  c->qtab[5] = {c->d_qpl, (size_t)c->nq_pad * prow * 4}; c->qtab[6] = {c->d_qrare, (size_t)nq * std::max(c->NR4, 1) * 12 * 4};
  int *d_cols = nullptr; uint32_t *d_qmin = nullptr;
  TALLOC(d_cols, cols_p.size() + cols_r.size(), false);
  TALLOC(d_qmin, (size_t)nq * std::max(c->NR4, 1) * 12, true);
  if (!cols_p.empty()) OPENCHK(hipMemcpyAsync(d_cols, cols_p.data(), cols_p.size() * sizeof(int), hipMemcpyHostToDevice, s));
  if (!cols_r.empty()) OPENCHK(hipMemcpyAsync(d_cols + cols_p.size(), cols_r.data(), cols_r.size() * sizeof(int), hipMemcpyHostToDevice, s));
  if (c->NP4 > 0) {
    dim3 grid((unsigned)nq, (unsigned)((c->NP4 * 4 + 63) / 64));
    if (c->acgt) hipLaunchKernelGGL((qprep_compress_kernel<true, false>), grid, dim3(64), 0, s, c->d_qp, nq, Wp, d_cols, c->NP, c->NP4 * 4, c->d_cls, c->d_qpl, prow, (uint32_t *)nullptr);
    else         hipLaunchKernelGGL((qprep_compress_kernel<false, false>), grid, dim3(64), 0, s, c->d_qp, nq, Wp, d_cols, c->NP, c->NP4 * 4, c->d_cls, c->d_qpl, prow, (uint32_t *)nullptr);
    OPENCHK(hipGetLastError());
  }
  if (c->NR4 > 0) {
    dim3 grid((unsigned)nq, (unsigned)((c->NR4 * 4 + 63) / 64));
    if (c->acgt) hipLaunchKernelGGL((qprep_compress_kernel<true, true>), grid, dim3(64), 0, s, c->d_qp, nq, Wp, d_cols + cols_p.size(), c->NR, c->NR4 * 4, c->d_cls, c->d_qrare, (size_t)0, d_qmin);
    else         hipLaunchKernelGGL((qprep_compress_kernel<false, true>), grid, dim3(64), 0, s, c->d_qp, nq, Wp, d_cols + cols_p.size(), c->NR, c->NR4 * 4, c->d_cls, c->d_qrare, (size_t)0, d_qmin);
    OPENCHK(hipGetLastError());
  }
  const int NWs = c->scan_NW, QS = 64, n_st = c->nq_pad / QS, NX = c->W4 + c->NR4;
  const uint32_t row_b = 256u * (uint32_t)c->scan_R;
  uint8_t *d_kind = nullptr; int *d_need = nullptr, *d_len = nullptr, *d_cost = nullptr;
  TALLOC(d_kind, (size_t)nq * c->W4, false);
  TALLOC(d_need, (size_t)c->W4, true);
  TALLOC(d_len, (size_t)n_st * NX, false);
  TALLOC(d_cost, (size_t)n_st * NX, false);
  {
    dim3 grid((unsigned)nq, (unsigned)((c->W4 + 63) / 64));
    if (c->acgt) hipLaunchKernelGGL((qprep_kinds_kernel<true>), grid, dim3(64), 0, s, c->d_qp, nq, Wp, c->d_cls, d_kind, d_need);
    else         hipLaunchKernelGGL((qprep_kinds_kernel<false>), grid, dim3(64), 0, s, c->d_qp, nq, Wp, c->d_cls, d_kind, d_need);
    hipLaunchKernelGGL(qprep_stream_sizes_kernel, dim3((unsigned)NX, (unsigned)n_st), dim3(64), 0, s, d_kind, d_qmin, nq, c->W4, c->NR4, d_len, d_cost);
    OPENCHK(hipGetLastError());
  }
  std::vector<int> need((size_t)c->W4), len((size_t)n_st * NX), cost((size_t)n_st * NX);
  OPENCHK(hipMemcpyAsync(need.data(), d_need, need.size() * sizeof(int), hipMemcpyDeviceToHost, s));
  OPENCHK(hipMemcpyAsync(len.data(), d_len, len.size() * sizeof(int), hipMemcpyDeviceToHost, s));
  OPENCHK(hipMemcpyAsync(cost.data(), d_cost, cost.size() * sizeof(int), hipMemcpyDeviceToHost, s));
  OPENCHK(hipStreamSynchronize(s));
  for (int g = 0; g < c->W4; g++) { c->need_e_groups += (need[(size_t)g] & 1) != 0; c->need_v_groups += (need[(size_t)g] & 2) != 0; c->need_g_groups += (need[(size_t)g] & 4) != 0; }
  if (c->replay_lq < 0) c->replay_lq = (nq < 256) ? 1 : 0;
  std::vector<long long> at((size_t)n_st * (NX + 1), 0);
  std::vector<uint32_t> sdir((size_t)n_st * 4 * NWs, 0u);
  std::vector<uint8_t> rare_group_used((size_t)std::max(c->NR4, 1), 0);
  size_t total = 0;
  struct Rec { size_t at; uint32_t cost; };
  auto shares = [NWs](const std::vector<Rec> &r, size_t base, size_t end_at, uint32_t *dir) {
    uint64_t tot = 0;
// ... 46 lines not shown
```

### uvaia_amd/csrc/host_qtables.inc

```
namespace {

int build_query_tables_host(uvaia_gpu_ctx *c, const uvaia_gpu_query *q, const uvaia_gpu_tuning &tn, const uint8_t *code_tab, int lo, int hi, const std::vector<uint8_t> &in_p)
{
#define OPENCHK(call) HIP_TRY(call, return fail(nullptr, code_, "%s failed: %s", #call, hipGetErrorString(e_)))
  const size_t row_words = (size_t)c->W4 * 4 * c->NQ;
  std::vector<uint32_t> qp((size_t)c->nq_pad * row_words, 0u);
  {
    std::atomic<int> first_bad(c->nq);
    std::vector<int> bad_byte((size_t)c->nq, 0);
    parallel_for(c->nq, [&](int i) {
      if (pack_query_row(code_tab, q->seq[i], c->nchar, lo, hi, nullptr, in_p.data(), c->acgt, c->NQ, qp.data() + (size_t)i * row_words, &bad_byte[(size_t)i])) {
        int cur = first_bad.load();
        while (i < cur && !first_bad.compare_exchange_weak(cur, i)) {}
      }
    });
    if (first_bad.load() < c->nq) {
      const int i = first_bad.load();
      return fail(nullptr, UVAIA_GPU_EALPHABET, "query %d holds byte 0x%02x outside the supported alphabet", i, bad_byte[(size_t)i]);
    }
  }
  OPENCHK(hipMalloc(&c->d_qp, qp.size() * 4)); OPENCHK(hipMemcpy(c->d_qp, qp.data(), qp.size() * 4, hipMemcpyHostToDevice));
  c->qtab[0] = {c->d_qp, qp.size() * 4};
  {
    std::vector<int> ambq((size_t)c->nq * AMB_STRIDE, 0);
// ... 56 lines not shown
      }
      for (int w = 0; w < Wp; w++) { c->NP += __builtin_popcount(cls[(size_t)w * 4 + 3]); c->NR += __builtin_popcount(rmask[(size_t)w]); }
      c->NP4 = ((c->NP + 31) / 32 + 3) / 4;
      c->NR4 = ((c->NR + 31) / 32 + 3) / 4;
      if (c->scan_variant == 2 && (size_t)c->NP4 * 128 + (size_t)c->NR4 * 128 > SCAN3_BIAS - 256) c->scan_variant = 0;
      struct RareWord { int word; uint32_t m, l, h; };
      std::vector<std::vector<RareWord>> rare_q((size_t)c->nq_pad);
      std::vector<uint32_t> qrare((size_t)c->nq * std::max(c->NR4, 1) * 12, 0u);
      const size_t prow = (size_t)std::max(c->NP4, 1) * 16, crow = (size_t)c->W4 * 8;
      std::vector<uint32_t> qpl((size_t)c->nq_pad * prow, 0u), qcv((size_t)c->nq_pad * crow, 0u), flg((size_t)(c->nq_pad / 16) * c->W4 * 2, 0u);
      parallel_for(c->nq_pad / 16, [&](int tile_) { for (int i = tile_ * 16; i < tile_ * 16 + 16; i++) {
        int k = 0, kr = 0;
        bool full = false;
        for (int w = 0; w < Wp; w++) {
          const bool real = i < c->nq;
          const uint32_t qL = real ? QL(i, w, 0) : 0u, qH = real ? QL(i, w, 1) : 0u, qI = real ? QL(i, w, 2) : 0u, qV = real ? QL(i, w, 3) : 0u;
          for (uint32_t m = cls[(size_t)w * 4 + 3]; m; m &= m - 1, k++) {
            const int b = __builtin_ctz(m);
            uint32_t *d = qpl.data() + (size_t)i * prow + (size_t)(k >> 7) * 16 + ((k >> 5) & 3);
            d[0] |= ((qL >> b) & 1u) << (k & 31); d[4] |= ((qH >> b) & 1u) << (k & 31); d[8] |= ((qI >> b) & 1u) << (k & 31);
          }
          const uint32_t eqb = qI & ~((qL ^ cls[(size_t)w * 4 + 0]) | (qH ^ cls[(size_t)w * 4 + 1]));
          const uint32_t nI = ~eqb & cls[(size_t)w * 4 + 2], nV = ~qV;
          for (uint32_t m = rmask[(size_t)w]; m; m &= m - 1, kr++) {
            const int b = __builtin_ctz(m);
            if (real) { uint32_t *d = qrare.data() + ((size_t)i * c->NR4 * 4 + (size_t)(kr >> 5)) * 3;
                        d[0] |= ((qL >> b) & 1u) << (kr & 31); d[1] |= ((qH >> b) & 1u) << (kr & 31); d[2] |= ((qI >> b) & 1u) << (kr & 31); }
            if (!real || !((qI >> b) & 1u) || ((eqb >> b) & 1u)) continue;
            if (rare_q[(size_t)i].empty() || rare_q[(size_t)i].back().word != (kr >> 5)) rare_q[(size_t)i].push_back({kr >> 5, 0u, 0u, 0u});
            RareWord &rw = rare_q[(size_t)i].back();
            rw.m |= 1u << (kr & 31); rw.l |= ((qL >> b) & 1u) << (kr & 31); rw.h |= ((qH >> b) & 1u) << (kr & 31);
          }
          qcv[(size_t)i * crow + (size_t)(w >> 2) * 8 + (w & 3)] = nI; qcv[(size_t)i * crow + (size_t)(w >> 2) * 8 + 4 + (w & 3)] = nV;
          uint32_t *fw = &flg[((size_t)(i / 16) * c->W4 + (w >> 2)) * 2];
          if (real && nI) fw[0] |= 1u << (i % 16);
          if (real && nV) fw[0] |= 0x10000u << (i % 16);
          if ((w & 3) == 0) full = real;
          full = full && nI == cls[(size_t)w * 4 + 2] && nV == 0xFFFFFFFFu;
          if ((w & 3) == 3 && full) { fw[0] &= ~(0x10001u << (i % 16)); fw[1] |= 1u << (i % 16); }
        }
      } });
      for (int g = 0; g < c->W4; g++) {
        uint32_t u = 0;
        uint32_t uy = 0;
        for (int t = 0; t < c->nq_pad / 16; t++) { u |= flg[((size_t)t * c->W4 + g) * 2]; uy |= flg[((size_t)t * c->W4 + g) * 2 + 1]; }
        c->need_e_groups += (u & 0xFFFFu) != 0; c->need_v_groups += (u >> 16) != 0; c->need_g_groups += uy != 0;
      }
      if (c->replay_lq < 0) c->replay_lq = (c->nq < 256) ? 1 : 0;
      OPENCHK(hipMalloc(&c->d_cls, cls.size() * 4)); OPENCHK(hipMemcpy(c->d_cls, cls.data(), cls.size() * 4, hipMemcpyHostToDevice));
      OPENCHK(hipMalloc(&c->d_qrare, qrare.size() * 4)); OPENCHK(hipMemcpy(c->d_qrare, qrare.data(), qrare.size() * 4, hipMemcpyHostToDevice));
      OPENCHK(hipMalloc(&c->d_rmask, rmask.size() * 4)); OPENCHK(hipMemcpy(c->d_rmask, rmask.data(), rmask.size() * 4, hipMemcpyHostToDevice));
      c->qtab[3] = {c->d_cls, cls.size() * 4}; c->qtab[4] = {c->d_rmask, rmask.size() * 4}; c->qtab[6] = {c->d_qrare, qrare.size() * 4};
      {
        int split[15];
        for (int v = 0; v <= 4; v++) split[v] = (int)((long long)c->W4 * v / 4);
        for (int v = 0; v <= 4; v++) {
          int nd = 0, nr = 0;
          for (int w = 0; w < split[v] * 4; w++) { nd += __builtin_popcount(cls[(size_t)w * 4 + 3]); nr += __builtin_popcount(rmask[(size_t)w]); }
          split[5 + v] = nd; split[10 + v] = nr;
        }
        OPENCHK(hipMalloc(&c->d_split, sizeof split)); OPENCHK(hipMemcpy(c->d_split, split, sizeof split, hipMemcpyHostToDevice));
        c->qtab[9] = {c->d_split, sizeof split};
      }
      OPENCHK(hipMalloc(&c->d_qpl, qpl.size() * 4)); OPENCHK(hipMemcpy(c->d_qpl, qpl.data(), qpl.size() * 4, hipMemcpyHostToDevice));
      c->qtab[5] = {c->d_qpl, qpl.size() * 4};
      const int NWs = c->scan_NW, QS = 64;
      const uint32_t row_b = 256u * (uint32_t)c->scan_R;
      struct Rec { size_t at; uint32_t cost; };
      struct TileStream { std::vector<uint32_t> u; std::vector<Rec> rec, rare; };
      const int n_st = c->nq_pad / QS;
      std::vector<TileStream> ts((size_t)n_st);
      std::vector<uint8_t> rare_groups_needed((size_t)std::max(c->NR4, 1), 0);
      parallel_for(n_st, [&](int st) {
        TileStream &S = ts[(size_t)st];
        std::vector<uint32_t> &strm = S.u;
        std::vector<int> full, gen, wrd[4];
        for (int g = 0; g < c->W4; g++) {
          full.clear(); gen.clear(); for (auto &w : wrd) w.clear();
          uint32_t wmask[64]; bool any_run = false;
          for (int ql = 0; ql < QS; ql++) {
            const int q = st * QS + ql, t = q / 16, b = q % 16;
            const uint32_t fx = flg[((size_t)t * c->W4 + g) * 2], fy = flg[((size_t)t * c->W4 + g) * 2 + 1];
            if ((fy >> b) & 1u) { full.push_back(ql); continue; }
            if (!(((fx | (fx >> 16)) >> b) & 1u)) continue;
            const uint32_t *src = qcv.data() + (size_t)q * crow + (size_t)g * 8;
            int n_part = 0, part = 0, last_full = 0;
            uint32_t fm = 0u;
            for (int j = 0; j < 4; j++) {
              if (!(src[j] | src[4 + j])) continue;
              if (src[4 + j] == 0xFFFFFFFFu && src[j] == cls[(size_t)(g * 4 + j) * 4 + 2]) { last_full = j; fm |= 0xFFu << (8 * j); }
              else { n_part++; part = j; }
            }
            int jsel = -1;
            if (n_part == 1) jsel = part;
            else if (n_part == 0) { jsel = last_full; fm &= ~(0xFFu << (8 * last_full)); }
            if (jsel >= 0) { wrd[jsel].push_back(ql); wmask[ql] = fm; any_run |= fm != 0u; } else gen.push_back(ql);
          }
          if (full.empty() && gen.empty() && wrd[0].empty() && wrd[1].empty() && wrd[2].empty() && wrd[3].empty()) continue;
          const size_t hdr = strm.size();
          const uint32_t n_full4 = (uint32_t)(full.size() + 3) / 4u;
          strm.push_back((uint32_t)g * 2048u | (any_run ? 1u : 0u));
          strm.push_back(n_full4 | (uint32_t)gen.size() << 16);
          strm.push_back((uint32_t)wrd[0].size() | (uint32_t)wrd[1].size() << 8 | (uint32_t)wrd[2].size() << 16 | (uint32_t)wrd[3].size() << 24);
          strm.push_back(0u);
          for (int ql : full) strm.push_back((uint32_t)ql * row_b);
          while (strm.size() & 3) strm.push_back((uint32_t)QS * row_b);
          for (int ql : gen) {
            const uint32_t *src = qcv.data() + (size_t)(st * QS + ql) * crow + (size_t)g * 8;
            strm.insert(strm.end(), src, src + 8);
            strm.push_back((uint32_t)ql * row_b); strm.push_back(0u); strm.push_back(0u); strm.push_back(0u);
          }
          for (int j = 0; j < 4; j++)
            for (int ql : wrd[j]) {
// ... 59 lines not shown
```

### uvaia_amd/csrc/host_resident.inc

```

extern "C" {

int uvaia_gpu_db_reserve(uvaia_gpu_ctx *c, size_t cap)
{
  if (!c) return UVAIA_GPU_EINVAL;
  if (cap <= c->db_cap) return 0;
  if (c->db_n) return fail(c, UVAIA_GPU_ESTATE, "reserve the database before appending to it");
  const size_t tiles = (cap + 63) / 64 + 1;
  const size_t dtiles = derived_tiles(c, tiles) + (c->shard_world > 1 ? 1 : 0);
  if (int rc = store_alloc(c, c->db, dtiles)) return rc;
  c->db_local_tiles = dtiles;
  c->peer_db[c->shard_rank] = c->db.planes; c->peer_amb[c->shard_rank] = c->db.amb;
  c->db_cap = tiles * 64 - 64;
  if (c->entered_cap < tiles * 64) {
    hipFree(c->d_entered); c->d_entered = nullptr;
    HIPCHK(c, hipMalloc(&c->d_entered, tiles * 64)); c->entered_cap = tiles * 64;
  }
  HIPCHK(c, hipMemset(c->d_entered, 0, c->entered_cap));
  return 0;
}

static int db_canonical_side_rows(uvaia_gpu_ctx *c, long long slot0, int n_ref)
{
  if (c->acgt || n_ref <= 0 || !c->db.amb) return 0;
  const long long t0 = slot0 / 64, t1 = (slot0 + n_ref - 1) / 64;
  hipLaunchKernelGGL(side_rows_canonical_kernel, dim3((unsigned)(t1 - t0 + 1)), dim3(64), 0, c->stream, c->db.planes, c->W4, t0, slot0, n_ref, c->db.amb);
  HIPCHK(c, hipGetLastError());
  HIPCHK(c, hipStreamSynchronize(c->stream));
  return 0;
}

static int db_append_common(uvaia_gpu_ctx *c, const char *const *seq, const char *rows, size_t pitch, const int *non_n, int n_ref)
{
  if (!c) return UVAIA_GPU_EINVAL;
  if (n_ref < 0) return fail(c, UVAIA_GPU_EINVAL, "negative count");
  if (n_ref == 0) return 0;
  { int rc = settle_derive(c); if (rc) return rc; }
  if (c->db_n + (size_t)n_ref > c->db_cap) {
    if (c->db_n) return fail(c, UVAIA_GPU_ESTATE, "database capacity %zu exceeded: call uvaia_gpu_db_reserve first", c->db_cap);
    int rc = uvaia_gpu_db_reserve(c, (size_t)n_ref); if (rc) return rc;
  }
  const long long s0 = (long long)c->db_n, s1 = s0 + n_ref;
  for (long long a = s0; a < s1;) {
    const long long pe = c->shard_world == 1 ? s1 : std::min(s1, (a / (c->shard_pt * 64) + 1) * c->shard_pt * 64);
    if (owns_tile(c, a / 64)) {
      const long long off = a - s0, local = dtile_of(c, a / 64) * 64 + a % 64;
      int rc = pack_rows(c, seq ? seq + off : nullptr, rows ? rows + (size_t)off * pitch : nullptr, pitch, non_n ? non_n + off : nullptr, (int)(pe - a), c->db, local);
      if (rc) return rc;
      rc = db_canonical_side_rows(c, local, (int)(pe - a));
      if (rc) return rc;
    }
    a = pe;
  }
  c->db_n += (size_t)n_ref;
  c->win_n = 0;
  return 0;
}

int uvaia_gpu_db_skip(uvaia_gpu_ctx *c, size_t n_ref)
{
  if (!c) return UVAIA_GPU_EINVAL;
  if (!n_ref) return 0;
  if (c->db_n + n_ref > c->db_cap) return fail(c, UVAIA_GPU_ESTATE, "database capacity %zu exceeded: call uvaia_gpu_db_reserve first", c->db_cap);
  for (size_t a = c->db_n; a < c->db_n + n_ref; a = (a / 64 + 1) * 64)
    if (owns_tile(c, (long long)(a / 64))) return fail(c, UVAIA_GPU_EINVAL, "reference %zu belongs to a piece of this context: it cannot be skipped", a);
  c->db_n += n_ref;
  return 0;
}

int uvaia_gpu_db_append(uvaia_gpu_ctx *c, const char *const *seq, const int *non_n, int n_ref)
{ if (c && n_ref > 0 && !seq) return fail(c, UVAIA_GPU_EINVAL, "NULL seq"); return db_append_common(c, seq, nullptr, 0, non_n, n_ref); }

int uvaia_gpu_db_append_block(uvaia_gpu_ctx *c, const char *rows, size_t pitch, const int *non_n, int n_ref)
{
  if (c && n_ref > 0 && (!rows || pitch < (size_t)c->nchar)) return fail(c, UVAIA_GPU_EINVAL, "bad block");
  return db_append_common(c, nullptr, rows, pitch, non_n, n_ref);
}

size_t uvaia_gpu_db_size(const uvaia_gpu_ctx *c) { return c ? c->db_n : 0; }

int uvaia_gpu_db_clear(uvaia_gpu_ctx *c)
{
  if (!c) return UVAIA_GPU_EINVAL;
  c->win_n = 0;
  if (!c->db.planes || !c->db_n) { c->db_n = 0; return 0; }
  { int rc = settle_derive(c); if (rc) return rc; }
  HIPCHK(c, hipStreamSynchronize(c->stream));
  if (int rc = sync_scan_streams(c)) return rc;
  const size_t tiles = c->shard_world == 1 ? (c->db_n + 63) / 64 : c->db_local_tiles;
  HIPCHK(c, hipMemsetAsync(c->db.planes, 0, tiles * (size_t)c->W4 * c->P * 64 * sizeof(uint4), c->stream));
  HIPCHK(c, hipMemsetAsync(c->db.nonn, 0, tiles * 64 * sizeof(int), c->stream));
  HIPCHK(c, hipMemsetAsync(c->db.tot, 0, tiles * 64 * sizeof(int), c->stream));
  HIPCHK(c, hipMemsetAsync(c->db.amb, 0, tiles * 64 * AMB_ROW * sizeof(int), c->stream));
  HIPCHK(c, hipStreamSynchronize(c->stream));
  c->db_n = 0;
  return 0;
}

size_t uvaia_gpu_db_tile_bytes(const uvaia_gpu_ctx *c) { return c ? (size_t)c->W4 * 4 * 64 * sizeof(uint4) : 0; }
int uvaia_gpu_db_side_row_ints(void) { return AMB_ROW; }

int uvaia_gpu_db_export(uvaia_gpu_ctx *c, size_t first_tile, size_t n_tiles, void *planes, int *non_n, int *side_rows)
{
  if (!c || !planes || !non_n || !side_rows) return UVAIA_GPU_EINVAL;
  if (c->acgt) return fail(c, UVAIA_GPU_ESTATE, "the interchange form is the four IUPAC planes: export from a default-mode context");
  if (c->shard_world > 1) return fail(c, UVAIA_GPU_ESTATE, "a context of a reference shard holds its own pieces only: export from a plain context");
  if ((first_tile + n_tiles) * 64 > ((c->db_n + 63) / 64) * 64) return fail(c, UVAIA_GPU_EINVAL, "tiles %zu..%zu lie outside the database", first_tile, first_tile + n_tiles);
  if (!n_tiles) return 0;
  HIPCHK(c, hipStreamSynchronize(c->stream));
  const size_t tb = uvaia_gpu_db_tile_bytes(c);
  HIPCHK(c, hipMemcpy(planes, reinterpret_cast<const char *>(c->db.planes) + first_tile * tb, n_tiles * tb, hipMemcpyDeviceToHost));
  HIPCHK(c, hipMemcpy(non_n, c->db.nonn + first_tile * 64, n_tiles * 64 * sizeof(int), hipMemcpyDeviceToHost));
  HIPCHK(c, hipMemcpy(side_rows, c->db.amb + first_tile * 64 * AMB_ROW, n_tiles * 64 * AMB_ROW * sizeof(int), hipMemcpyDeviceToHost));
  return 0;
}

int uvaia_gpu_db_append_packed(uvaia_gpu_ctx *c, const void *planes, const int *non_n, const int *side_rows, int n_ref)
{
  if (!c) return UVAIA_GPU_EINVAL;
  if (n_ref < 0) return fail(c, UVAIA_GPU_EINVAL, "negative count");
  if (n_ref == 0) return 0;
  if (!planes || !non_n || (!c->acgt && !side_rows)) return fail(c, UVAIA_GPU_EINVAL, "NULL packed arrays");
  if (c->db_n % 64) return fail(c, UVAIA_GPU_ESTATE, "packed tiles can only follow a whole number of tiles (database holds %zu references)", c->db_n);
  { int rc = settle_derive(c); if (rc) return rc; }
  if (c->db_n + (size_t)n_ref > c->db_cap) {
    if (c->db_n) return fail(c, UVAIA_GPU_ESTATE, "database capacity %zu exceeded: call uvaia_gpu_db_reserve first", c->db_cap);
    int rc = uvaia_gpu_db_reserve(c, (size_t)n_ref); if (rc) return rc;
  }
  const size_t tb = uvaia_gpu_db_tile_bytes(c), n_tiles_all = ((size_t)n_ref + 63) / 64;
  const long long t0g = (long long)(c->db_n / 64);
  int rc = for_owned_tiles(c, t0g, t0g + (long long)n_tiles_all, [&](long long gt, long long t0, long long nt) -> int {
    const size_t n_tiles = (size_t)nt, off = (size_t)(gt - t0g);
    const char *pl = reinterpret_cast<const char *>(planes) + off * tb;
    if (!c->acgt) {
      HIPCHK(c, hipMemcpyAsync(reinterpret_cast<char *>(c->db.planes) + (size_t)t0 * tb, pl, n_tiles * tb, hipMemcpyHostToDevice, c->stream));
      hipLaunchKernelGGL((import_tiles_kernel<4>), dim3((unsigned)n_tiles), dim3(256), 0, c->stream, c->db.planes + (size_t)t0 * c->W4 * 4 * 64, c->W4, (uint4 *)nullptr, t0, c->db.tot);
      HIPCHK(c, hipGetLastError());
      HIPCHK(c, hipMemcpyAsync(c->db.amb + (size_t)t0 * 64 * AMB_ROW, side_rows + off * 64 * AMB_ROW, n_tiles * 64 * AMB_ROW * sizeof(int), hipMemcpyHostToDevice, c->stream));
    } else {
      const size_t chunk = 64;
      uint4 *d_tmp = nullptr;
      HIPCHK(c, hipMalloc(&d_tmp, chunk * tb));
      for (size_t a = 0; a < n_tiles; a += chunk) {
        const size_t m = std::min(chunk, n_tiles - a);
        hipError_t e = hipMemcpyAsync(d_tmp, pl + a * tb, m * tb, hipMemcpyHostToDevice, c->stream);
        if (e == hipSuccess) { hipLaunchKernelGGL((import_tiles_kernel<3>), dim3((unsigned)m), dim3(256), 0, c->stream, d_tmp, c->W4, c->db.planes, t0 + (long long)a, c->db.tot); e = hipGetLastError(); }
        if (e == hipSuccess) e = hipStreamSynchronize(c->stream);
        if (e != hipSuccess) { hipFree(d_tmp); return fail(c, UVAIA_GPU_EHIP, "import of packed tiles: %s", hipGetErrorString(e)); }
      }
      hipFree(d_tmp);
    }
    HIPCHK(c, hipMemcpyAsync(c->db.nonn + (size_t)t0 * 64, non_n + off * 64, n_tiles * 64 * sizeof(int), hipMemcpyHostToDevice, c->stream));
    hipLaunchKernelGGL(sanitise_import_kernel, dim3((unsigned)((n_tiles * 64 + 255) / 256)), dim3(256), 0, c->stream, c->acgt ? (int *)nullptr : c->db.amb + (size_t)t0 * 64 * AMB_ROW,
                       c->db.nonn + (size_t)t0 * 64, (long long)(n_tiles * 64), c->W4 * 4, c->nchar);
    HIPCHK(c, hipGetLastError());
    return derive_rows(c, c->db, t0 * 64, (int)(n_tiles * 64));
  });
  if (rc) return rc;
  HIPCHK(c, hipStreamSynchronize(c->stream));
  c->db_n += (size_t)n_ref;
  c->win_n = 0;
  return 0;
}

struct SubSlice { size_t first, n; bool pool_start; };
#ifndef HEAD_TAIL_NQT
#define HEAD_TAIL_NQT 17
#endif
static std::vector<SubSlice> plan_subslices(const uvaia_gpu_ctx *c, size_t first, size_t n, size_t pool)
{
  std::vector<SubSlice> subs;
  const int nq_act = c->act_q1 - c->act_q0, nqt = (c->act_q1 + 15) / 16 - c->act_q0 / 16;
  if (c->n_idx_c == 0) pool = std::max<size_t>(n, 1);
  size_t sub = c->subslice;
  if (nqt <= 32) sub /= 2;
  if (nqt < 63) sub = std::min(pool, (sub * 63 / (size_t)std::max(nqt, 1) + 63) / 64 * 64);
  if (nqt < 4) sub = std::min(pool, std::max<size_t>(65536, ((pool + 3) / 4 + 63) / 64 * 64));
  if (c->subslice_forced) sub = std::min(pool, c->subslice);
  (void)nq_act;
  for (size_t a = first; a < first + n; a += pool) {
    const size_t pe = std::min(first + n, a + pool);
    if (nqt < HEAD_TAIL_NQT && !c->subslice_forced && pe - a >= 8 * 65536) {
      const size_t head = 65536, tail = 65536, pre = (nqt < 4 && pe - a >= 12 * 65536) ? 131072 : 0, mid = pe - a - head - tail - pre, nm = std::max<size_t>(1, (mid + sub / 2) / sub);
      const size_t each = ((mid + nm - 1) / nm + 63) / 64 * 64;
      subs.push_back({a, head, true});
      for (size_t x = a + head; x < pe - tail - pre; x += each) subs.push_back({x, std::min(each, pe - tail - pre - x), false});
      if (pre) subs.push_back({pe - tail - pre, pre, false});
      subs.push_back({pe - tail, tail, false});
      continue;
    }
    const size_t len = pe - a, ns = std::max<size_t>(1, (len + sub / 2) / sub);
    const size_t each = ((len + ns - 1) / ns + 63) / 64 * 64;
    if (c->first_slice_pct > 0 && c->first_slice_pct < 100 && ns >= 3 && !c->subslice_forced) {
      const size_t first_n = std::max<size_t>(64, each * (size_t)c->first_slice_pct / 100 / 64 * 64), rest = len - first_n;
      const size_t each2 = ((rest + (ns - 1) - 1) / (ns - 1) + 63) / 64 * 64;
      subs.push_back({a, first_n, true});
      for (size_t x = a + first_n; x < pe; x += each2) subs.push_back({x, std::min(each2, pe - x), false});
      continue;
    }
    for (size_t x = a; x < pe; x += each) subs.push_back({x, std::min(each, pe - x), x == a});
  }
  return subs;
}

int uvaia_gpu_db_rederive(uvaia_gpu_ctx *c)
{
  if (!c) return UVAIA_GPU_EINVAL;
  if (!c->db.planes || !c->db_n || c->fullscan || c->scan_variant != 2) return 0;
  HIPCHK(c, hipSetDevice(c->device));
  {
    hipStream_t busy[4] = {c->stream, c->scan_streams[0], c->scan_streams[1], c->scan_streams[2]};
    for (int i = 0; i < 4; i++) {
      if (!busy[i]) continue;
      if (!c->derive_fence[i]) HIPCHK(c, hipEventCreateWithFlags(&c->derive_fence[i], hipEventDisableTiming));
      HIPCHK(c, hipEventRecord(c->derive_fence[i], busy[i]));
      for (int j = 0; j < c->derive_nstreams; j++) HIPCHK(c, hipStreamWaitEvent(c->derive_streams[j], c->derive_fence[i], 0));
    }
  }
  std::vector<SubSlice> plan;
  if (c->shard_world == 1) plan = plan_subslices(c, 0, c->db_n, c->max_pool);
  else {
    const size_t piece = (size_t)c->shard_pt * 64;
    for (size_t a = (size_t)c->shard_rank * piece; a < c->db_n; a += piece * (size_t)c->shard_world) plan.push_back({a, std::min(piece, c->db_n - a), false});
  }
  const int n_derive_streams = (c->derive_forced || plan.size() <= 3) ? c->derive_nstreams : 1;
  size_t k = 0;
  long long t_done = 0;
  for (const SubSlice &sl : plan) {
    const long long t0 = std::max(t_done, (long long)(sl.first / 64)), t1 = (long long)((sl.first + sl.n + 63) / 64);
    if (t0 >= t1) continue;
    t_done = t1;
    if (k == c->derive_chunks.size()) {
      uvaia_gpu_ctx::DeriveChunk d{0, 0, nullptr};
      HIPCHK(c, hipEventCreateWithFlags(&d.done, hipEventDisableTiming));
      c->derive_chunks.push_back(d);
    }
    hipStream_t ds = c->derive_streams[k % (size_t)n_derive_streams];
    int rc = for_owned_tiles(c, t0, t1, [&](long long, long long lt, long long nt) -> int { return derive_rows(c, c->db, lt * 64, (int)(nt * 64), ds, true); });
    if (rc) return rc;
    c->derive_chunks[k].t0 = t0; c->derive_chunks[k].t1 = t1;
    HIPCHK(c, hipEventRecord(c->derive_chunks[k].done, ds));
    k++;
  }
  c->derive_pending = k;
  return 0;
}

static int pipe_check(uvaia_gpu_ctx *c)
{
  if (!c->pipe_used || !c->d_pipe_err) return 0;
  int bad = 0;
  HIPCHK(c, hipMemcpy(&bad, c->d_pipe_err, sizeof(int), hipMemcpyDeviceToHost));
  c->pipe_used = false;
  if (bad) { HIPCHK(c, hipMemset(c->d_pipe_err, 0, sizeof(int))); return fail(c, UVAIA_GPU_EHIP, "pipelined search: a replay gave up waiting for the scan of its slice (results are incomplete)"); }
  return 0;
}

static int run_subslices(uvaia_gpu_ctx *c, const std::vector<SubSlice> &subs_in, int64_t ordinal_of_db0, int snapshot)
{
  std::vector<SubSlice> subs = subs_in;
  const bool piped = c->pipeline && c->scan_variant == 2 && !c->use_ext && !c->fullscan && !c->serial && c->shard_world == 1 && subs_in.size() > 1;
  if (piped) {
    const size_t rows = std::min<size_t>((size_t)c->nq_pad, ((size_t)c->act_q1 + 63) / 64 * 64);
    const size_t cap_refs = std::max<size_t>(subs_in[0].n, std::min<size_t>(262144, ((size_t)512 << 20) / (rows * 4) / 64 * 64));
    subs.clear();
    for (size_t i = 0; i < subs_in.size(); i++) {
      const bool first_of_pool = subs_in[i].pool_start, second_of_pool = i > 0 && subs_in[i - 1].pool_start;
      if (!subs.empty() && !first_of_pool && !second_of_pool && subs.back().n + subs_in[i].n <= cap_refs && !(c->n_idx_c > 0 && subs.back().n + subs_in[i].n > c->max_pool)) subs.back().n += subs_in[i].n;
      else subs.push_back(subs_in[i]);
    }
  }
  struct PipeGuard { uvaia_gpu_ctx *c; ~PipeGuard() { c->pipeline_now = false; } } guard{c};
  c->pipeline_now = piped;
  const size_t ns = subs.size();
  size_t issued = 0;
  {
    const int nqt = (c->act_q1 + 15) / 16 - c->act_q0 / 16;
    size_t longest = 0;
    for (const SubSlice &sl : subs) longest = std::max(longest, sl.n);
    const size_t waves = ns ? (size_t)nqt * ((longest + 63) / 64) : 0;
    c->scan_nstreams = (waves && waves < 16000 && nqt >= 4 && !c->use_ext) ? 3 : 1;
    if (c->scan_nstreams_forced) c->scan_nstreams = c->scan_nstreams_forced;
  }
  for (size_t i = 0; i < ns; i++) {
    const bool serial_ = c->serial;
    while (issued < ns && issued < i + (serial_ ? 1 : NBUF)) {
      int rc = uvaia_gpu_slice_scan(c, subs[issued].first, subs[issued].n, (int)(issued % NBUF));
      if (rc) return rc;
      issued++;
      if (serial_) (void)sync_scan_streams(c);
    }
    int take = subs[i].pool_start ? 1 : 0;
    if (take && snapshot >= 0) { HIPCHK(c, hipMemcpyAsync(c->d_snap, &snapshot, sizeof(int), hipMemcpyHostToDevice, c->stream)); HIPCHK(c, hipStreamSynchronize(c->stream)); take = 0; }
    int rc = uvaia_gpu_slice_replay(c, (int)(i % NBUF), ordinal_of_db0 + (long long)subs[i].first, take);
    if (rc) return rc;
    if (serial_) hipStreamSynchronize(c->stream);
  }
  return 0;
}

int uvaia_gpu_search_resident(uvaia_gpu_ctx *c, size_t pool, int64_t ordinal0, uint8_t *entered)
{
  if (!c) return UVAIA_GPU_EINVAL;
  if (c->shard_world > 1) return fail(c, UVAIA_GPU_ESTATE, "a context of a reference shard keeps its own pieces only: use uvaia_gpu_shard_scan / uvaia_gpu_shard_replay (or a group)");
  if (pool < 1 || pool > c->max_pool) return fail(c, UVAIA_GPU_EINVAL, "pool must be in [1, max_pool=%zu]", c->max_pool);
  if (!c->db_n) return 0;
  HIPCHK(c, hipMemsetAsync(c->d_entered, 0, ((c->db_n + 63) / 64) * 64, c->stream));
  if (!c->fullscan) {
    size_t head = 0;
    if (c->scan_variant == 2 && c->head_full && c->n_idx_c == 0 && c->db_n > 4096 && !c->serial) {
      head = 128;
      const bool fs = c->fullscan, prof = c->profile;
      c->fullscan = true; c->profile = false;
      const int rc = run_batch(c, c->db, 0, 2, 0, (int)head, (long long)ordinal0, 128);
      c->fullscan = fs; c->profile = prof;
      if (rc) return rc;
    }
    int rc = run_subslices(c, plan_subslices(c, head, c->db_n - head, pool), ordinal0, -1);
    if (rc) return rc;
  } else
  for (size_t a = 0; a < c->db_n; a += pool) {
    const size_t b = std::min(c->db_n, a + pool);
    const long long tf = (long long)(a / 64);
    const int n_tiles = (int)((b + 63) / 64 - a / 64);
    const int rb = (int)(a - (size_t)tf * 64), re = (int)(b - (size_t)tf * 64);
    int rc = run_batch(c, c->db, tf, n_tiles, rb, re, ordinal0 + (long long)a);
    if (rc) return rc;
  }
  if (entered) {
    HIPCHK(c, hipMemcpyAsync(entered, c->d_entered, c->db_n, hipMemcpyDeviceToHost, c->stream));
    HIPCHK(c, hipStreamSynchronize(c->stream));
    { int rc = pipe_check(c); if (rc) return rc; }
    return collect_events(c);
  }
  return 0;
}

int uvaia_gpu_search_resident_pool(uvaia_gpu_ctx *c, size_t first, size_t n, int64_t ordinal0, int snapshot)
{
  if (!c) return UVAIA_GPU_EINVAL;
  if (c->fullscan) return fail(c, UVAIA_GPU_ESTATE, "per-pool search needs the default scan");
  if (n < 1 || n > c->max_pool || first + n > c->db_n) return fail(c, UVAIA_GPU_EINVAL, "pool [%zu,+%zu) outside the database or above max_pool=%zu", first, n, c->max_pool);
  return run_subslices(c, plan_subslices(c, first, n, n), ordinal0 - (int64_t)first, snapshot);
}

int uvaia_gpu_sync(uvaia_gpu_ctx *c)
{
  if (!c) return UVAIA_GPU_EINVAL;
  if (int rc = sync_derive_streams(c)) return rc;
  c->derive_pending = 0;
  if (int rc = sync_scan_streams(c)) return rc;
  HIPCHK(c, hipStreamSynchronize(c->stream));
  if (c->rep_stream) HIPCHK(c, hipStreamSynchronize(c->rep_stream));
  { int rc = pipe_check(c); if (rc) return rc; }
  return collect_events(c);
}

int uvaia_gpu_last_batch_scores(uvaia_gpu_ctx *c, int *out, int n_ref)
{
  if (!c || !out) return UVAIA_GPU_EINVAL;
  if (n_ref != c->last.n || !c->last.store) return fail(c, UVAIA_GPU_ESTATE, "last batch held %d references, not %d", c->last.n, n_ref);
  const int *nonn = c->last.store->nonn + c->last.tile_first * 64;
  int *d_out = nullptr;
  const size_t bytes = (size_t)n_ref * c->nq * 6 * sizeof(int);
  if (!c->fullscan) {
    int rc = ensure_cnt4(c, (size_t)c->nq_pad * c->last.ppad); if (rc) return rc;
    const bool prof = c->profile; c->profile = false;
    rc = launch_scan(c, *c->last.store, c->last.tile_first, c->last.n_tiles, c->d_qp, c->nq, c->d_cnt, c->last.ppad, 0.0);
    c->profile = prof;
    if (rc) return rc;
  }
  HIPCHK(c, hipMalloc(&d_out, bytes));
  dim3 grid((n_ref + 255) / 256, c->nq);
  if (c->acgt) hipLaunchKernelGGL((batch_scores_kernel<true>), grid, dim3(256), 0, c->stream, c->d_cnt, c->last.ppad, c->last.rt, nonn, c->last.rbegin, n_ref, c->nq, d_out);
  else         hipLaunchKernelGGL((batch_scores_kernel<false>), grid, dim3(256), 0, c->stream, c->d_cnt, c->last.ppad, c->last.rt, nonn, c->last.rbegin, n_ref, c->nq, d_out);
  hipError_t e = hipGetLastError();
  if (e == hipSuccess) e = hipMemcpyAsync(out, d_out, bytes, hipMemcpyDeviceToHost, c->stream);
  if (e == hipSuccess) e = hipStreamSynchronize(c->stream);
  hipFree(d_out);
  if (e != hipSuccess) return fail(c, UVAIA_GPU_EHIP, "batch_scores: %s", hipGetErrorString(e));
  return 0;
}

int uvaia_gpu_scan_stats(uvaia_gpu_ctx *c, double *ms, long long *launches, double *bytes, int reset)
{
  if (!c) return UVAIA_GPU_EINVAL;
  int rc = collect_events(c); if (rc) return rc;
  if (ms) *ms = c->scan_ms;
  if (launches) *launches = c->scan_launches;
  if (bytes) *bytes = c->scan_bytes;
  if (reset) { c->scan_ms = 0; c->scan_bytes = 0; c->scan_launches = 0; }
  return 0;
}

int uvaia_gpu_replay_stats(uvaia_gpu_ctx *c, unsigned long long out[3], int reset)
{
  if (!c || !out) return UVAIA_GPU_EINVAL;
  HIPCHK(c, hipStreamSynchronize(c->stream));
  unsigned long long h[3] = {0, 0, 0};
  HIPCHK(c, hipMemcpy(h, c->d_stats, sizeof h, hipMemcpyDeviceToHost));
  out[0] = h[0]; out[1] = h[1]; out[2] = h[2];
  if (reset) HIPCHK(c, hipMemset(c->d_stats, 0, sizeof h));
  return 0;
}

int uvaia_gpu_replay_timing(uvaia_gpu_ctx *c, unsigned long long out[12], int reset)
// ... 48 lines not shown
  if (nqr) {
    HIPCHK(c, hipMemcpyAsync(c->d_n + q0, d + 4, nqr * sizeof(int), hipMemcpyDefault, c->stream));
    HIPCHK(c, hipMemcpyAsync(c->d_T + q0, d + 4 + nqr, nqr * sizeof(int), hipMemcpyDefault, c->stream));
    HIPCHK(c, hipMemcpyAsync(c->d_heap + (size_t)q0 * he, d + 4 + 2 * nqr, nqr * he * sizeof(int), hipMemcpyDefault, c->stream));
  }
  HIPCHK(c, hipStreamSynchronize(c->stream));
  return 0;
}

int uvaia_gpu_state_export(uvaia_gpu_ctx *c, void *dst) { return c ? uvaia_gpu_state_export_range(c, dst, 0, c->nq) : UVAIA_GPU_EINVAL; }
int uvaia_gpu_state_import(uvaia_gpu_ctx *c, const void *src) { return c ? uvaia_gpu_state_import_range(c, src, 0, c->nq) : UVAIA_GPU_EINVAL; }

int uvaia_gpu_slice_scan(uvaia_gpu_ctx *c, size_t first, size_t n, int buf)
{
  if (!c || buf < 0 || buf >= NBUF) return UVAIA_GPU_EINVAL;
  if (c->fullscan) return fail(c, UVAIA_GPU_ESTATE, "ring mode needs the two-counter scan");
  if (c->shard_world > 1) return fail(c, UVAIA_GPU_ESTATE, "a context of a reference shard keeps its own pieces only: use uvaia_gpu_shard_scan / uvaia_gpu_shard_replay");
  if (first + n > c->db_n) return fail(c, UVAIA_GPU_EINVAL, "slice [%zu,+%zu) outside the database", first, n);
  if (n > c->max_pool && c->n_idx_c > 0) return fail(c, UVAIA_GPU_EINVAL, "slice of %zu references above max_pool %zu", n, c->max_pool);
  SliceBuf &b = c->slice[buf];
  const size_t ppad_ = ((first + n + 63) / 64 - first / 64) * 64;
  const size_t qtile = c->scan_variant == 2 ? 64 : 16;
  const size_t rows = std::min<size_t>((size_t)c->nq_pad, ((size_t)c->act_q1 + qtile - 1) / qtile * qtile);
  if (int rc = slice_reserve(c, b, rows * ppad_, ppad_)) return rc;
  hipStream_t ss = c->scan_streams[c->scan_nstreams > 1 ? (c->scan_rr++ % c->scan_nstreams) : 0];
  if (b.replay_recorded) HIPCHK(c, hipStreamWaitEvent(ss, b.replay_done, 0));
  for (size_t k = 0; k < c->derive_pending; k++) {
    const auto &d = c->derive_chunks[k];
    if (d.t0 < (long long)((first + n + 63) / 64) && d.t1 > (long long)(first / 64)) HIPCHK(c, hipStreamWaitEvent(ss, d.done, 0));
  }
  b.tf = (long long)(first / 64);
  b.tiles = n ? (int)((first + n + 63) / 64 - first / 64) : 0;
  b.rb = (int)(first - (size_t)b.tf * 64); b.re = b.rb + (int)n;
  b.scanned = true; b.cons_done = false;
  unsigned *progress = nullptr;
  b.piped = false;
  if (c->pipeline_now && c->scan_variant == 2 && b.tiles > 0) {
    const size_t stripes = (size_t)(b.tiles + SCAN_STRIPE_TILES - 1) / SCAN_STRIPE_TILES;
    if (stripes > b.progress_cap) {
      if (b.progress) { HIPCHK(c, hipStreamSynchronize(c->stream)); if (c->rep_stream) HIPCHK(c, hipStreamSynchronize(c->rep_stream)); hipFree(b.progress); b.progress = nullptr; }
      HIPCHK(c, hipMalloc(&b.progress, (stripes + 64) * sizeof(unsigned))); b.progress_cap = stripes + 64;
    }
    if (!b.scan_started) HIPCHK(c, hipEventCreateWithFlags(&b.scan_started, hipEventDisableTiming));
    if (!c->d_pipe_err) { HIPCHK(c, hipMalloc(&c->d_pipe_err, sizeof(int))); HIPCHK(c, hipMemset(c->d_pipe_err, 0, sizeof(int))); }
    progress = b.progress;
    HIPCHK(c, hipMemsetAsync(progress, 0, stripes * sizeof(unsigned), ss));
    HIPCHK(c, hipEventRecord(b.scan_started, ss));
    b.piped = true; c->pipe_used = true;
  }
  const double bytes = (double)n * (double)c->W4 * 16.0 * c->P + (double)c->nq * (double)c->W4 * 16.0 * c->P;
  int rc = launch_scan2(c, c->db, b.tf, b.tiles, b.cnt, b.tiles * 64, bytes, ss, b.tmin, b.rb, b.re, b.rt, c->use_ext ? b.ext : nullptr, b.rtp, b.tb8, progress);
  if (rc) return rc;
  HIPCHK(c, hipEventRecord(b.scan_done, ss));
  return 0;
}

int uvaia_gpu_slice_replay_range(uvaia_gpu_ctx *c, int buf, int64_t ordinal0, int q0, int q1, int take_snapshot)
{
  if (!c || buf < 0 || buf >= NBUF) return UVAIA_GPU_EINVAL;
  SliceBuf &b = c->slice[buf];
  if (!b.scanned) return fail(c, UVAIA_GPU_ESTATE, "slice_replay without slice_scan");
  if (q0 < 0 || q1 > c->nq || q1 < q0) return fail(c, UVAIA_GPU_EINVAL, "bad query range [%d,%d)", q0, q1);
  if (take_snapshot) { hipLaunchKernelGGL(snapshot_kernel, dim3(1), dim3(256), 0, c->stream, c->d_T + c->act_q0, c->act_q1 - c->act_q0, c->d_snap); b.cons_done = false; }
  if (b.re <= b.rb || q1 == q0) return 0;
  HIPCHK(c, hipStreamWaitEvent(c->stream, b.piped ? b.scan_started : b.scan_done, 0));
  const int ppad = b.tiles * 64;
  const uint32_t *ext = c->use_ext ? b.ext : nullptr;
  hipStream_t rs = (c->rep_stream && ext) ? c->rep_stream : c->stream;
  if (rs != c->stream) { HIPCHK(c, hipEventRecord(c->rep_ev[0], c->stream)); HIPCHK(c, hipStreamWaitEvent(rs, c->rep_ev[0], 0)); }
  const int pf = (q1 - q0) <= 64 ? 1 : 2;
  const unsigned blocks_per_group = (unsigned)((c->act_q1 + 63) / 64 - c->act_q0 / 64);
  int rc = launch_replay(c, {rs, q0, q1, b.cnt, ext, ppad, b.rt, b.rtp, b.tmin, b.tb8,
                             c->db.planes, b.tf, c->db.nonn + b.tf * 64, c->db.amb + b.tf * 64 * AMB_ROW, c->d_entered + b.tf * 64, b.rb, b.re, (long long)ordinal0,
                             (c->scan_variant == 2 && c->shard_world == 1) ? c->d_qpl : nullptr, c->db.poly, c->NR4, c->d_qrare, pf,
                             b.piped ? b.progress : nullptr, blocks_per_group, c->scan_R, c->d_pipe_err});
  if (rc) return rc;
  if (rs != c->stream) { HIPCHK(c, hipEventRecord(c->rep_ev[1], rs)); HIPCHK(c, hipStreamWaitEvent(c->stream, c->rep_ev[1], 0)); }
  HIPCHK(c, hipEventRecord(b.replay_done, c->stream));
  b.replay_recorded = true;
  c->last = {&c->db, b.tf, b.tiles, b.re - b.rb, b.rb, ppad, b.rt};
  return 0;
}

int uvaia_gpu_slice_buffers(void) { return NBUF; }

int uvaia_gpu_slice_replay(uvaia_gpu_ctx *c, int buf, int64_t ordinal0, int stripe_start)
{ return c ? uvaia_gpu_slice_replay_range(c, buf, ordinal0, c->act_q0, c->act_q1, stripe_start) : UVAIA_GPU_EINVAL; }

int uvaia_gpu_set_active_queries(uvaia_gpu_ctx *c, int q0, int q1)
{
  if (!c) return UVAIA_GPU_EINVAL;
  if (q0 < 0 || q1 > c->nq || q1 <= q0 || ((q0 % 64) && c->shard_world == 1))
    return fail(c, UVAIA_GPU_EINVAL, "active queries [%d,%d): need 0 <= q0 < q1 <= %d and q0 a multiple of 64", q0, q1, c->nq);
  if ((c->fullscan || c->scan_variant != 2) && c->shard_world == 1) { if (q0 != 0 || q1 != c->nq) return fail(c, UVAIA_GPU_ESTATE, "query shards need the default scan"); }
  c->act_q0 = q0; c->act_q1 = q1;
  return 0;
}

int uvaia_gpu_max_tolerance(uvaia_gpu_ctx *c, int *out)
{
  if (!c || !out) return UVAIA_GPU_EINVAL;
  int *d_tmp = nullptr;
  HIPCHK(c, hipMalloc(&d_tmp, sizeof(int)));
  hipLaunchKernelGGL(snapshot_kernel, dim3(1), dim3(256), 0, c->stream, c->d_T + c->act_q0, c->act_q1 - c->act_q0, d_tmp);
  hipError_t e = hipGetLastError();
  if (e == hipSuccess) e = hipMemcpyAsync(out, d_tmp, sizeof(int), hipMemcpyDeviceToHost, c->stream);
  if (e == hipSuccess) e = hipStreamSynchronize(c->stream);
  hipFree(d_tmp);
  if (e != hipSuccess) return fail(c, UVAIA_GPU_EHIP, "max_tolerance: %s", hipGetErrorString(e));
  return 0;
}

int uvaia_gpu_entered_flags(uvaia_gpu_ctx *c, uint8_t *out, int clear)
{
  if (!c) return UVAIA_GPU_EINVAL;
  HIPCHK(c, hipStreamSynchronize(c->stream));
  if (out && c->db_n) HIPCHK(c, hipMemcpy(out, c->d_entered, c->db_n, hipMemcpyDeviceToHost));
  if (clear && c->db_n) HIPCHK(c, hipMemset(c->d_entered, 0, ((c->db_n + 63) / 64) * 64));
  return 0;
}


}
```

### uvaia_amd/csrc/kernels_replay.inc

```

template <bool ACGT>
static __device__ __forceinline__ void assemble_scores(const int4 cnt, const int4 rt, const int4 rc, int nn, int S[6], int &mism)
{
  if (ACGT) {
    const int pmm = cnt.x - rt.x, pba = cnt.y - rt.y;
    S[0] = (pba + rc.y) - (pmm + rc.x);
    S[1] = pba + rc.y;
    S[2] = S[0] - (rc.y - rc.x);
    S[3] = nn;
    S[4] = rc.x + (pmm - cnt.z);
    S[5] = cnt.z;
    mism = S[1] - S[0];
  } else {
    const int p0 = cnt.x - rt.x;
    S[0] = p0 + rc.x;
    S[1] = cnt.y - rt.y + rc.y;
    S[2] = cnt.z - rt.z + rc.z;
    S[3] = cnt.w - rt.w + rc.w;
    S[4] = p0;
    S[5] = nn;
    mism = S[3] - S[0];
  }
}

// ... 850 lines not shown
          __syncthreads();
          full = (n == k);
          if (full) {
            if (!(was_full && use_mc)) {
#pragma unroll
              for (int sidx = 0; sidx < 6; sidx++) W[sidx] = h[HEAP_ENTRY + sidx];
            }
            if (!was_full && use_mc) mc = wave_minchild_init(h, n, lane);
            T = W[3] - W[0] + 1;
          }
          mask = __ballot(lane > i && may_enter());
        }
        if (admitted_here || T != T_used) P = needed(tbv) & half_mask & ~((2ull << tsel) - 1ull);
        TT_ADD(tt_admit, ta_);
        TT_ADD(tt_tile, tt0_);
      }
    }
  }
  replay_wait_staged();
#ifdef REPLAY_TIMING
  if (lane == 0) { atomicAdd(&stats[4], tt_wait); atomicAdd(&stats[5], tt_fetch); atomicAdd(&stats[6], tt_tile); atomicAdd(&stats[7], tt_admit); atomicAdd(&stats[8], tt_late); atomicAdd(&stats[9], n_late); atomicAdd(&stats[10], wall_clock64() - tt_begin);
                   atomicAdd(&stats[11], tt_prologue_end - tt_kernel); atomicAdd(&stats[12], 1ull); }
#endif
#undef TT_START
#undef TT_ADD
  if (dirty) {
    __syncthreads();
    for (int i = lane; i < (n + 1) * HEAP_ENTRY; i += 64) hg[i] = h[i];
    if (lane == 0) { n_g[q] = n; T_g[q] = T; }
  }
  if (stats && lane == 0) { atomicAdd(&stats[0], (unsigned long long)n_admit); atomicAdd(&stats[1], (unsigned long long)n_demand); atomicAdd(&stats[2], (unsigned long long)n_dense); atomicAdd(&stats[3], (unsigned long long)n_open); }
}

template <bool ACGT>
__global__ void agree_kernel(const int4 *__restrict__ cnt_q, int ppad, int nq, int n_ref, uint8_t *__restrict__ out)
{
  const int r = blockIdx.x * blockDim.x + threadIdx.x, q = blockIdx.y;
  if (r >= n_ref) return;
  const int4 c = cnt_q[(size_t)q * ppad + r];
  out[(size_t)r * nq + q] = (uint8_t)((ACGT ? c.x : (c.w - c.y)) == 0);
}

__global__ void snapshot_kernel(const int *__restrict__ T, int nq, int *__restrict__ snap)
{
  __shared__ int red[256];
  int v = -0x7fffffff;
  for (int i = threadIdx.x; i < nq; i += 256) v = max(v, T[i]);
  red[threadIdx.x] = v;
  __syncthreads();
  for (int s = 128; s > 0; s >>= 1) { if ((int)threadIdx.x < s) red[threadIdx.x] = max(red[threadIdx.x], red[threadIdx.x + s]); __syncthreads(); }
  if (threadIdx.x == 0) *snap = red[0];
}

__global__ void init_state_kernel(int *__restrict__ T, int *__restrict__ n, int nq, int nchar)
{
  const int i = blockIdx.x * blockDim.x + threadIdx.x;
  if (i < nq) { T[i] = nchar; n[i] = 0; }
}

template <bool ACGT>
__global__ void batch_scores_kernel(const int4 *__restrict__ cnt, int ppad, const int4 *__restrict__ rt, const int *__restrict__ nonn,
                                    int r_begin, int n_ref, int nq, int *__restrict__ out)
{
  const int i = blockIdx.x * blockDim.x + threadIdx.x, q = blockIdx.y;
  if (i >= n_ref) return;
  const int r = r_begin + i;
  int S[6], m;
  assemble_scores<ACGT>(cnt[(size_t)q * ppad + r], rt[r], rt[r], nonn[r], S, m);
  for (int s = 0; s < 6; s++) out[((size_t)i * nq + q) * 6 + s] = S[s];
}
```

### uvaia_amd/csrc/kernels_scan3.inc

```


typedef uint32_t u32x4_nt __attribute__((ext_vector_type(4)));
static __device__ __forceinline__ void st_stream(uint4 *p, const uint4 &v)
{
  const u32x4_nt x = {v.x, v.y, v.z, v.w};
  __builtin_nontemporal_store(x, reinterpret_cast<u32x4_nt *>(p));
}
struct GatherStage { uint32_t bL, bH, bI; int fill, ow; };

static __device__ __forceinline__ int shared_slot(const int *__restrict__ bit, int word)
{
  for (int k = 1; k <= 3; k++) if ((bit[k] & 31) != 0 && (bit[k] >> 5) == word) return k;
  return 0;
}
static __device__ __forceinline__ uint32_t take_bit(uint32_t x, int b, int at, uint32_t acc)
{
  return (__builtin_amdgcn_ubfe(x, (uint32_t)b, 1u) << at) | acc;
}

template <bool ACGT, bool WRITE_V>
__global__ __launch_bounds__(256) __attribute__((amdgpu_waves_per_eu(8, 8)))
void derive_all_kernel(const uint4 *__restrict__ tiles, long long tile_base, long long dtile_base, int W4,
                       const uint32_t *__restrict__ cls, const uint32_t *__restrict__ rmask,
                       const int *__restrict__ split, int NP4, int NR4,
                       uint4 *__restrict__ ev, int *__restrict__ tot_e, uint32_t *__restrict__ grp, uint4 *__restrict__ poly)
{
  constexpr int P = ACGT ? 3 : 4;
  __shared__ int partial[4][64];
  __shared__ uint32_t shr[6][3][64];
  for (int i = threadIdx.x; i < 6 * 3 * 64; i += 256) (&shr[0][0][0])[i] = 0u;
  __syncthreads();
  const int lane = threadIdx.x & 63, wv = __builtin_amdgcn_readfirstlane(threadIdx.x >> 6);
  const long long ptile = tile_base + blockIdx.x, tile = dtile_base + blockIdx.x;
  const uint4 *t = tiles + (size_t)ptile * W4 * P * 64 + lane;
  uint4 *o = ev + (size_t)tile * W4 * 2 * 64 + lane;
  const int NG = NP4 + NR4;
  uint32_t *po = reinterpret_cast<uint32_t *>(poly + (size_t)tile * NG * 3 * 64 + lane);
  const int lo = split[wv], hi = split[wv + 1];
  const int *dbit = split + 5, *rbit = split + 10;

  GatherStage D, R;
  D.bL = D.bH = D.bI = 0u; D.fill = dbit[wv] & 31; D.ow = dbit[wv] >> 5;
  R.bL = R.bH = R.bI = 0u; R.fill = rbit[wv] & 31; R.ow = rbit[wv] >> 5;
  int sw[2][3];
#pragma unroll
  for (int sec = 0; sec < 2; sec++) {
    const int *bit = sec ? rbit : dbit;
#pragma unroll
    for (int k = 1; k <= 3; k++) sw[sec][k - 1] = (bit[k] & 31) != 0 ? (bit[k] >> 5) : -1;
  }
  auto push_word = [&](GatherStage &g, int sec) {
    const int k = (sw[sec][0] == g.ow) ? 1 : (sw[sec][1] == g.ow) ? 2 : (sw[sec][2] == g.ow) ? 3 : 0;
    if (k) {
      uint32_t (*dst)[64] = shr[sec * 3 + k - 1];
      if (g.bL) atomicOr(&dst[0][lane], g.bL);
      if (g.bH) atomicOr(&dst[1][lane], g.bH);
      if (g.bI) atomicOr(&dst[2][lane], g.bI);
    } else {
      uint32_t *d = po + (size_t)((sec ? NP4 : 0) + (g.ow >> 2)) * 3 * 256 + (g.ow & 3);
      d[0] = g.bL; d[256] = g.bH; d[512] = g.bI;
    }
    g.bL = g.bH = g.bI = 0u; g.fill = 0; g.ow++;
  };

  int te = 0;
  uint4 nxt[P];
#pragma unroll
  for (int p = 0; p < P; p++) nxt[p] = lo < hi ? ld_stream(t + (size_t)(lo * P + p) * 64) : make_uint4(0u, 0u, 0u, 0u);
  for (int w4 = lo; w4 < hi; w4++) {
    uint4 pl[P];
#pragma unroll
    for (int p = 0; p < P; p++) pl[p] = nxt[p];
    if (w4 + 1 < hi) {
#pragma unroll
      for (int p = 0; p < P; p++) nxt[p] = ld_stream(t + (size_t)((w4 + 1) * P + p) * 64);
    }
    uint32_t e[4], v[4];
    int ge = 0, gv = 0;
#pragma unroll
    for (int j = 0; j < 4; j++) {
      uint32_t rL, rH, rI, rV;
      if (ACGT) { rL = u4c(pl[0], j); rH = u4c(pl[1], j); rI = u4c(pl[2], j); rV = rI; }
      else {
        const uint32_t a = u4c(pl[0], j), cc = u4c(pl[1], j), g = u4c(pl[2], j), tt = u4c(pl[P - 1], j);
        const uint32_t par = a ^ cc ^ g ^ tt, three = (a & cc & (g | tt)) | (g & tt & (a | cc));
        rI = par & ~three; rL = (cc | tt) & rI; rH = (g | tt) & rI; rV = a | cc | g | tt;
      }
      const uint32_t *c4 = cls + (size_t)(w4 * 4 + j) * 4;
      const uint32_t diff = (rL ^ c4[0]) | (rH ^ c4[1]);
      e[j] = rI & c4[2] & (ACGT ? diff : ~diff);
      v[j] = rV;
      ge += __popc(e[j]); gv += __popc(v[j]);
      for (uint32_t m = c4[3]; m; m &= m - 1) {
        const int b = __ffs(m) - 1;
        D.bL = take_bit(rL, b, D.fill, D.bL); D.bH = take_bit(rH, b, D.fill, D.bH); D.bI = take_bit(rI, b, D.fill, D.bI);
        if (++D.fill == 32) push_word(D, 0);
      }
      for (uint32_t m = rmask[w4 * 4 + j]; m; m &= m - 1) {
        const int b = __ffs(m) - 1;
        R.bL = take_bit(rL, b, R.fill, R.bL); R.bH = take_bit(rH, b, R.fill, R.bH); R.bI = take_bit(rI, b, R.fill, R.bI);
        if (++R.fill == 32) push_word(R, 1);
      }
    }
    te += ge;
    __builtin_nontemporal_store((uint32_t)ge | ((uint32_t)gv << 16), grp + ((size_t)tile * W4 + w4) * 64 + lane);
    st_stream(o + (size_t)(w4 * 2 + 0) * 64, make_uint4(e[0], e[1], e[2], e[3]));
    if (WRITE_V) st_stream(o + (size_t)(w4 * 2 + 1) * 64, make_uint4(v[0], v[1], v[2], v[3]));
  }
  if (NP4 && D.fill > 0) push_word(D, 0);
  if (NR4 && R.fill > 0) push_word(R, 1);
  if (wv == 3) {
    for (int w = (dbit[4] + 31) >> 5; w < NP4 * 4; w++) { uint32_t *d = po + (size_t)(w >> 2) * 3 * 256 + (w & 3); d[0] = 0u; d[256] = 0u; d[512] = 0u; }
    for (int w = (rbit[4] + 31) >> 5; w < NR4 * 4; w++) { uint32_t *d = po + (size_t)(NP4 + (w >> 2)) * 3 * 256 + (w & 3); d[0] = 0u; d[256] = 0u; d[512] = 0u; }
  }
  partial[wv][lane] = te;
  __syncthreads();
  if (wv == 0) tot_e[tile * 64 + lane] = partial[0][lane] + partial[1][lane] + partial[2][lane] + partial[3][lane];
  else {
    for (int sec = 0; sec < 2; sec++) {
      const int *bit = sec ? rbit : dbit;
      if ((sec ? NR4 : NP4) == 0 || (bit[wv] & 31) == 0) continue;
      const int w = bit[wv] >> 5;
      if (shared_slot(bit, w) != wv) continue;
      const uint32_t (*src)[64] = shr[sec * 3 + wv - 1];
      uint32_t *d = po + (size_t)((sec ? NP4 : 0) + (w >> 2)) * 3 * 256 + (w & 3);
      d[0] = src[0][lane]; d[256] = src[1][lane]; d[512] = src[2][lane];
    }
  }
}

template <int R> struct Scan3Acc;
template <> struct Scan3Acc<1> { typedef uint32_t type; };
template <> struct Scan3Acc<2> { typedef unsigned long long type; };
struct Scan3Acc4 { unsigned long long a, b; };
template <> struct Scan3Acc<4> { typedef Scan3Acc4 type; };
static __device__ __forceinline__ uint32_t acc_part(uint32_t v, int) { return v; }
static __device__ __forceinline__ uint32_t acc_part(unsigned long long v, int rr) { return (uint32_t)(v >> (32 * rr)); }
static __device__ __forceinline__ uint32_t acc_part(const Scan3Acc4 &v, int rr) { return (uint32_t)((rr < 2 ? v.a : v.b) >> (32 * (rr & 1))); }
typedef __attribute__((address_space(3))) char scan3_lds_char;
static __device__ __forceinline__ void lds_counter_add(scan3_lds_char *p, uint32_t v)
{ __hip_atomic_fetch_add((__attribute__((address_space(3))) uint32_t *)p, v, __ATOMIC_RELAXED, __HIP_MEMORY_SCOPE_WORKGROUP); }
static __device__ __forceinline__ void lds_counter_add(scan3_lds_char *p, unsigned long long v)
{ __hip_atomic_fetch_add((__attribute__((address_space(3))) unsigned long long *)p, v, __ATOMIC_RELAXED, __HIP_MEMORY_SCOPE_WORKGROUP); }
static __device__ __forceinline__ void lds_counter_add(scan3_lds_char *p, const Scan3Acc4 &v)
{
  __hip_atomic_fetch_add((__attribute__((address_space(3))) unsigned long long *)p, v.a, __ATOMIC_RELAXED, __HIP_MEMORY_SCOPE_WORKGROUP);
  __hip_atomic_fetch_add((__attribute__((address_space(3))) unsigned long long *)(p + 8), v.b, __ATOMIC_RELAXED, __HIP_MEMORY_SCOPE_WORKGROUP);
}
template <class T> static __device__ __forceinline__ void lds_counter_store(scan3_lds_char *p, const T &v) { *(__attribute__((address_space(3))) T *)p = v; }
static __device__ __forceinline__ void lds_counter_store(scan3_lds_char *p, const Scan3Acc4 &v)
{ *(__attribute__((address_space(3))) unsigned long long *)p = v.a; *(__attribute__((address_space(3))) unsigned long long *)(p + 8) = v.b; }
template <class T> static __device__ __forceinline__ void lds_counter_load(scan3_lds_char *p, T &v) { v = *(__attribute__((address_space(3))) T *)p; }
static __device__ __forceinline__ void lds_counter_load(scan3_lds_char *p, Scan3Acc4 &v)
{ v.a = *(__attribute__((address_space(3))) unsigned long long *)p; v.b = *(__attribute__((address_space(3))) unsigned long long *)(p + 8); }
static __device__ __forceinline__ void lds_counter_sub(scan3_lds_char *p, uint32_t v)
{ __hip_atomic_fetch_sub((__attribute__((address_space(3))) uint32_t *)p, v, __ATOMIC_RELAXED, __HIP_MEMORY_SCOPE_WORKGROUP); }
static __device__ __forceinline__ void lds_counter_sub(scan3_lds_char *p, unsigned long long v)
{ __hip_atomic_fetch_sub((__attribute__((address_space(3))) unsigned long long *)p, v, __ATOMIC_RELAXED, __HIP_MEMORY_SCOPE_WORKGROUP); }
static __device__ __forceinline__ void lds_counter_sub(scan3_lds_char *p, const Scan3Acc4 &v)
{
  __hip_atomic_fetch_sub((__attribute__((address_space(3))) unsigned long long *)p, v.a, __ATOMIC_RELAXED, __HIP_MEMORY_SCOPE_WORKGROUP);
  __hip_atomic_fetch_sub((__attribute__((address_space(3))) unsigned long long *)(p + 8), v.b, __ATOMIC_RELAXED, __HIP_MEMORY_SCOPE_WORKGROUP);
}

template <int NW , bool ACGT, int R, int QS = 64 >
__global__ __launch_bounds__(64 * NW) __attribute__((amdgpu_waves_per_eu(4, 8))) void scan3_kernel(const uint4 *__restrict__ ev, const uint4 *__restrict__ poly, long long tile_first, int n_tiles,
                                                     int W4, int NP4, int NPT, const uint32_t *__restrict__ qpl, const uint32_t *__restrict__ stream,
                                                     const uint32_t *__restrict__ sdir, const uint32_t *__restrict__ grp,
                                                     const int *__restrict__ tot_e, const int *__restrict__ tot_v,
                                                     uint32_t *__restrict__ out, int ppad, int n_stiles, int2 *__restrict__ tmin, int r_lo, int r_hi,
                                                     int stile_first, unsigned *__restrict__ progress )
{
  constexpr int QT = QS / NW;
  static_assert((NW == 4 || NW == 8 || NW == 16) && (QS == 64 || QS == 128) && QT >= 4 && QT <= 16, "waves and queries of a super-tile");
  static_assert(R == 1 || R == 2 || R == 4, "one, two or four reference tiles per wave");
  typedef typename Scan3Acc<R>::type acc_t;
  constexpr uint32_t RARE_BIAS = SCAN3_BIAS;
// ... 309 lines not shown
```

### uvaia_amd/csrc/uvaia_gpu.hip

```cpp
#include <hip/hip_runtime.h>

#include <algorithm>
#include <atomic>
#include <cstdarg>
#include <cstdint>
#include <cstdio>
#include <cstdlib>
#include <condition_variable>
#include <cstring>
#include <functional>
#include <mutex>
#include <string>
#include <thread>
#include <vector>

#include "../../include/uvaia_gpu.h"
#include "iupac_decode.h"

#define TT_A 0xF0u
#define TT_B 0xCCu
#define TT_C 0xAAu
#define B3(a, b, c, tt) __builtin_amdgcn_bitop3_b32((a), (b), (c), (tt) & 0xFFu)

static __device__ __forceinline__ uint32_t u4c(const uint4 &v, int j)
// ... 23 lines not shown
constexpr int AMB_ROW = 64;
constexpr int PACK_CHUNK = 4096;
constexpr uint32_t SCAN3_BIAS = 16384u;
constexpr int SCAN_STRIPE_TILES = 64;
constexpr int NBUF = 4;

thread_local std::string g_open_error;

struct ScanEvt { hipEvent_t a, b; double bytes; };

struct TileStore {
  uint4 *planes = nullptr;
  int *nonn = nullptr;
  int *amb = nullptr;
  int *tot = nullptr;
  uint4 *ev = nullptr, *poly = nullptr;
  uint32_t *grp = nullptr;
  int *tote = nullptr;
};

struct SliceBuf {
  uint32_t *cnt = nullptr;
  int2 *tmin = nullptr;
  uint32_t *ext = nullptr;
  uint32_t *rtp = nullptr;
  uint4 *tb8 = nullptr;
  int4 *rt = nullptr;
  size_t cap = 0;
  int tiles = 0, rb = 0, re = 0; long long tf = 0;
  bool scanned = false, cons_done = false, piped = false;
  unsigned *progress = nullptr; size_t progress_cap = 0;
  hipEvent_t scan_done = nullptr, scan_started = nullptr, replay_done = nullptr;
  bool replay_recorded = false;
};

}

struct uvaia_gpu_ctx {
  int device = 0;
  hipStream_t stream = nullptr;
  hipStream_t scan_streams[3] = {};
  unsigned scan_rr = 0;
  int scan_nstreams = 1;
  int scan_nstreams_forced = 0;
  int first_slice_pct = 70;
  hipStream_t scan_stream = nullptr;
  struct DeriveChunk { long long t0, t1; hipEvent_t done; };
  hipStream_t derive_stream = nullptr;
  hipStream_t derive_streams[3] = {};
  int derive_nstreams = 3; bool derive_forced = false;
  std::vector<DeriveChunk> derive_chunks;
  hipEvent_t derive_fence[4] = {};
  size_t derive_pending = 0;
  bool pipeline = false, pipeline_now = false, pipe_used = false;
  int *d_pipe_err = nullptr;
  SliceBuf slice[NBUF];
  bool use_ext = false;
  size_t subslice = 25088;
  bool subslice_forced = false;
  int nq = 0, nq_pad = 0, nchar = 0, W = 0, W4 = 0, P = 4, NQ = 6, acgt = 0, k = 2, qt = 16, n_idx_c = 0, n_idx_m = 0;
  size_t trim = 0;
  size_t max_pool = 0, pool_pad = 0;
  uint32_t *d_qp = nullptr;
  uint32_t *d_qp2 = nullptr;
  int scan_variant = 2;
  uint32_t *d_cls = nullptr;
  uint32_t *d_qpl = nullptr;
  uint32_t *d_stream = nullptr;
  uint32_t *d_sdir = nullptr;
  int NP = 0, NP4 = 0;
  int NR = 0, NR4 = 0, rare_max = -1;
  uint32_t *d_rmask = nullptr;
  int *d_split = nullptr;
  int shard_rank = 0, shard_world = 1; long long shard_pt = 0;
  const uint4 *peer_db[64] = {}; const int *peer_amb[64] = {};
  void *ipc_opened[64][2] = {};
  uint32_t *d_qrare = nullptr;
  int need_e_groups = 0, need_v_groups = 0, need_g_groups = 0, need_r_groups = 0;
  int act_q0 = 0, act_q1 = 0;
  bool serial = false;
  int replay_lq = -1;
  int replay_prio = 1;
  bool head_full = false;
  int replay_half = 32;
  int replay_cus = 0;
  hipStream_t rep_stream = nullptr; hipEvent_t rep_ev[2] = {};
  int scan_R = 2;
  int scan_NW = 8;
  int *d_amb_q = nullptr;
  struct { const void *p; size_t n; } qtab[10] = {};
  unsigned long long *d_stats = nullptr;
  hipEvent_t order_ev[16] = {}; unsigned order_rr = 0;
  hipEvent_t mark_ev[8][3] = {}; bool mark_set[8][3] = {};
  bool fullscan = false;
  size_t cnt_cap = 0;
  uint32_t *d_cp = nullptr;
  uint32_t *d_cpm = nullptr;
  uint32_t *d_qpoly = nullptr;
  uint32_t *d_pmask = nullptr;
  int *d_mindist = nullptr, *d_ball_list = nullptr, *d_ball_cdist = nullptr, *d_ball_n = nullptr; size_t ball_cap = 0;
  uint4 *d_ball_tiles = nullptr; size_t ball_tiles_cap = 0; unsigned long long ball_asked = 0;
  bool ball_fused = true; uint4 *d_ball_ga = nullptr; size_t ball_ga_tiles = 0;
  hipEvent_t ball_ev[4] = {}; double ball_ms[3] = {0., 0., 0.};
  int *d_idx_cols = nullptr; int n_idx = 0, NG4 = 0;
  std::vector<int> idx_cols; uint32_t *d_ball_masks = nullptr; int NH4 = 0;
  uint32_t *d_qg = nullptr;
  unsigned long long *d_ball_key = nullptr;
  uint4 *d_pk = nullptr; int pk_n = 0;
  uint8_t *d_rows = nullptr; size_t rows_cap = 0;
  int *d_row_idx = nullptr; size_t row_idx_cap = 0;
  int *d_rsel = nullptr, *d_rcnt = nullptr; unsigned long long *d_roff = nullptr; uint2 *d_rexc = nullptr;
  size_t rsel_cap = 0, rcnt_cap = 0, roff_cap = 0, rexc_cap = 0;
  std::vector<int> rows_host; std::vector<uint2> rexc_host;
  uint32_t run_cut = 0xFFFFFFu;
  std::vector<hipEvent_t> rows_evs; double rows_ms[3] = {0., 0., 0.};
  struct StageSlot { uint4 *planes = nullptr; int *nonn = nullptr, *side = nullptr; int n_tiles = 0; hipEvent_t copied = nullptr, read = nullptr; bool read_recorded = false; };
  StageSlot wstage[2]; size_t wstage_tiles = 0;
  hipStream_t copy_stream = nullptr;
  int *d_wsel = nullptr; size_t wsel_cap = 0;
  uint4 *d_win4 = nullptr; size_t win4_tiles = 0; int win_n = 0;
  hipEvent_t win_ev[5] = {}; double win_ms[3] = {0., 0., 0.};
  int *d_heap = nullptr, *d_n = nullptr, *d_T = nullptr, *d_snap = nullptr, *d_err = nullptr;
  TileStore batch;
  int4 *d_cnt = nullptr;
  int4 *d_rt = nullptr, *d_tr = nullptr;
  uint8_t *d_entered = nullptr;
  size_t entered_cap = 0;
  uint8_t *d_stage = nullptr;
  uint8_t *h_stage = nullptr;
  hipEvent_t stage_free[2] = {}; bool stage_busy[2] = {};
  size_t pitch = 0;
  TileStore db;
  size_t db_cap = 0, db_n = 0, db_local_tiles = 0;
  struct { const TileStore *store = nullptr; long long tile_first = 0; int n_tiles = 0, n = 0, rbegin = 0, ppad = 0; const int4 *rt = nullptr; } last;
  std::vector<ScanEvt> evts;
  std::vector<hipEvent_t> ev_pool;
  double scan_ms = 0, scan_bytes = 0; long long scan_launches = 0;
  bool profile = true;
  std::string err;
};

namespace {

int fail(uvaia_gpu_ctx *c, int code, const char *fmt, ...)
{
  char buf[512];
  va_list ap; va_start(ap, fmt); vsnprintf(buf, sizeof buf, fmt, ap); va_end(ap);
  if (c) c->err = buf; else g_open_error = buf;
  return code;
}

#define HIP_TRY(call, on_fail) do { hipError_t e_ = (call); if (e_ != hipSuccess) { const int code_ = e_ == hipErrorOutOfMemory ? UVAIA_GPU_ENOMEM : UVAIA_GPU_EHIP; (void)code_; on_fail; } } while (0)
#define HIPCHK(c, call) HIP_TRY(call, return fail((c), code_, "%s failed: %s (%s:%d)", #call, hipGetErrorString(e_), __FILE__, __LINE__))

inline bool owns_tile(const uvaia_gpu_ctx *c, long long t) { return c->shard_world == 1 || (t / c->shard_pt) % c->shard_world == c->shard_rank; }
inline long long dtile_of(const uvaia_gpu_ctx *c, long long t)
{ return c->shard_world == 1 ? t : (t / (c->shard_pt * c->shard_world)) * c->shard_pt + t % c->shard_pt; }
template <class F> inline int for_owned_tiles(const uvaia_gpu_ctx *c, long long gt0, long long gt1, F f)
{
  if (c->shard_world == 1) return gt1 > gt0 ? f(gt0, gt0, gt1 - gt0) : 0;
  for (long long a = gt0; a < gt1;) {
    const long long b = std::min(gt1, (a / c->shard_pt + 1) * c->shard_pt);
    if (owns_tile(c, a)) { const int rc = f(a, dtile_of(c, a), b - a); if (rc) return rc; }
    a = b;
  }
  return 0;
}
inline size_t derived_tiles(const uvaia_gpu_ctx *c, size_t tiles)
{ return c->shard_world == 1 ? tiles : (size_t)((tiles + (size_t)(c->shard_pt * c->shard_world) - 1) / (size_t)(c->shard_pt * c->shard_world)) * (size_t)c->shard_pt; }

void fill_code_table(uint8_t *t)
{
  memset(t, 0xFF, 256);
  const char *inv = "NnXx-?Oo.";
  for (const char *p = inv; *p; p++) t[(unsigned char)*p] = 0;
  static const struct { char c; uint8_t m; } iu[] = {
    {'A',1},{'C',2},{'G',4},{'T',8},{'M',3},{'R',5},{'W',9},{'S',6},{'Y',10},{'K',12},{'V',7},{'H',11},{'D',13},{'B',14}};
  for (auto &e : iu) { t[(unsigned char)e.c] = e.m; t[(unsigned char)(e.c + 32)] = e.m; }
}

// ... 22 lines not shown
```

Measured before the change: 33.08 million.

## Fuse reset into one kernel, parametrize derive waves, track plane-buffer fences

Replaces the memset, init kernel, host memcpy and stream synchronizations in reset with a single fused reset_state_kernel, so reset no longer blocks the host. It also tracks the zeroed entered-flags extent so a later search can skip re-clearing them. The derive_all kernel is templated on 4, 8 or 16 waves per block with precomputed split tables, selectable through a new tuning field; the default stays at 4. It adds per-stream busy and fence tracking for the planes buffers and an export API for the derived tiles, at the risk of ordering bugs now that reset no longer synchronizes.

```diff
diff --git a/include/uvaia_gpu.h b/include/uvaia_gpu.h
--- a/include/uvaia_gpu.h
+++ b/include/uvaia_gpu.h
@@ -54,6 +54,7 @@
   int scan_streams;
   int pipeline;
   int head_scan;
+  int derive_waves;
 } uvaia_gpu_tuning;
 int uvaia_gpu_export_query_table (uvaia_gpu_ctx *ctx, int which, void *out, size_t cap, size_t *n_bytes);
 int uvaia_gpu_open_tuned (uvaia_gpu_ctx **ctx, const uvaia_gpu_query *query, int heap_size, int device, size_t max_pool, const uvaia_gpu_tuning *tuning );
@@ -151,6 +152,7 @@
 size_t uvaia_gpu_db_tile_bytes (const uvaia_gpu_ctx *ctx);
 int    uvaia_gpu_db_clear (uvaia_gpu_ctx *ctx);
 int    uvaia_gpu_db_rederive (uvaia_gpu_ctx *ctx);
+int    uvaia_gpu_db_derived_export (uvaia_gpu_ctx *ctx, size_t n_tiles, void *e, uint32_t *grp, void *poly, int *tot);
 int    uvaia_gpu_db_side_row_ints (void);
 int    uvaia_gpu_db_export (uvaia_gpu_ctx *ctx, size_t first_tile, size_t n_tiles, void *planes, int *non_n, int *side_rows);
 int    uvaia_gpu_db_append_packed (uvaia_gpu_ctx *ctx, const void *planes, const int *non_n, const int *side_rows, int n_ref);
diff --git a/uvaia_amd/capi.py b/uvaia_amd/capi.py
--- a/uvaia_amd/capi.py
+++ b/uvaia_amd/capi.py
@@ -17,7 +17,7 @@
     "uvaia_gpu_state_bytes", "uvaia_gpu_state_export", "uvaia_gpu_state_import", "uvaia_gpu_slice_scan", "uvaia_gpu_slice_replay",
     "uvaia_gpu_entered_flags", "uvaia_gpu_state_range_bytes", "uvaia_gpu_state_export_range", "uvaia_gpu_state_import_range",
     "uvaia_gpu_slice_replay_range", "uvaia_gpu_slice_buffers", "uvaia_gpu_scan_bytes_per_ref", "uvaia_gpu_derived_bytes_per_ref", "uvaia_gpu_scan_variant", "uvaia_gpu_set_query_tile", "uvaia_gpu_packed_bytes_per_ref",
-    "uvaia_gpu_db_tile_bytes", "uvaia_gpu_db_side_row_ints", "uvaia_gpu_db_export", "uvaia_gpu_db_append_packed", "uvaia_gpu_db_clear", "uvaia_gpu_db_rederive",
+    "uvaia_gpu_db_tile_bytes", "uvaia_gpu_db_side_row_ints", "uvaia_gpu_db_export", "uvaia_gpu_db_append_packed", "uvaia_gpu_db_clear", "uvaia_gpu_db_rederive", "uvaia_gpu_db_derived_export",
     "uvaia_gpu_set_active_queries", "uvaia_gpu_max_tolerance", "uvaia_gpu_search_resident_pool",
     "uvaia_gpu_db_set_shard", "uvaia_gpu_shard_rows", "uvaia_gpu_shard_scan", "uvaia_gpu_scan_wait", "uvaia_gpu_replay_wait", "uvaia_gpu_set_snapshot", "uvaia_gpu_shard_replay",
     "uvaia_gpu_mark", "uvaia_gpu_stream_wait_mark", "uvaia_gpu_wait_stream",
@@ -40,7 +40,7 @@
 
 class Tuning(C.Structure):
     _fields_ = [("subslice_refs", C.c_size_t), ("rare_max", C.c_int), ("scan", C.c_int), ("serial", C.c_int),
-                ("scan_tiles_per_wave", C.c_int), ("scan_waves_per_block", C.c_int), ("rederive_streams", C.c_int), ("ball_gather", C.c_int), ("query_tables", C.c_int), ("replay_extras", C.c_int), ("replay_cus", C.c_int), ("scan_streams", C.c_int), ("pipeline", C.c_int), ("head_scan", C.c_int)]
+                ("scan_tiles_per_wave", C.c_int), ("scan_waves_per_block", C.c_int), ("rederive_streams", C.c_int), ("ball_gather", C.c_int), ("query_tables", C.c_int), ("replay_extras", C.c_int), ("replay_cus", C.c_int), ("scan_streams", C.c_int), ("pipeline", C.c_int), ("head_scan", C.c_int), ("derive_waves", C.c_int)]
 
     SCAN = {"auto": 0, "packed": 1, "compressed": 2, "wide": 3}
 
@@ -142,6 +142,7 @@
         "uvaia_gpu_db_tile_bytes": (C.c_size_t, [vp]),
         "uvaia_gpu_db_clear": (C.c_int, [vp]),
         "uvaia_gpu_db_rederive": (C.c_int, [vp]),
+        "uvaia_gpu_db_derived_export": (C.c_int, [vp, C.c_size_t, C.c_void_p, C.c_void_p, C.c_void_p, C.c_void_p]),
         "uvaia_gpu_db_side_row_ints": (C.c_int, []),
         "uvaia_gpu_db_export": (C.c_int, [vp, C.c_size_t, C.c_size_t, C.c_void_p, pi, pi]),
         "uvaia_gpu_db_append_packed": (C.c_int, [vp, C.c_void_p, pi, pi, C.c_int]),
@@ -609,6 +610,17 @@
             self._chk(self.L.uvaia_gpu_export_query_table(self.ctx, int(which), out.ctypes.data_as(C.c_void_p), n.value, C.byref(n)))
         return out
 
+    def db_derived(self, n_tiles):
+        W4 = ((self.nchar + 31) // 32 + 3) // 4
+        counts = self.query_table(10).view(np.int32)
+        NG = int(counts[2]) + int(counts[3])
+        e = np.zeros((n_tiles, W4, 64, 4), dtype=np.uint32)
+        grp = np.zeros((n_tiles, W4, 64), dtype=np.uint32)
+        poly = np.zeros((n_tiles, NG, 3, 64, 4), dtype=np.uint32)
+        tot = np.zeros(n_tiles * 64, dtype=np.int32)
+        self._chk(self.L.uvaia_gpu_db_derived_export(self.ctx, int(n_tiles), e.ctypes.data, grp.ctypes.data, poly.ctypes.data, tot.ctypes.data))
+        return e, grp, poly, tot
+
     def ball_kernel_ms(self, reset=False):
         out = (C.c_double * 3)()
         self.L.uvaia_gpu_ball_kernel_ms(self.ctx, out, int(reset))
diff --git a/uvaia_amd/csrc/host_batch.inc b/uvaia_amd/csrc/host_batch.inc
--- a/uvaia_amd/csrc/host_batch.inc
+++ b/uvaia_amd/csrc/host_batch.inc
@@ -111,6 +111,7 @@
 {
   if (!c || !n_items || !scores || !ordinals) return c ? fail(c, UVAIA_GPU_EINVAL, "NULL output") : UVAIA_GPU_EINVAL;
   HIPCHK(c, hipStreamSynchronize(c->stream));
+  planes_idle(c, true, false);
   const size_t ne = (size_t)c->nq * (c->k + 1);
   std::vector<int> h(ne * HEAP_ENTRY), T(c->nq);
   HIPCHK(c, hipMemcpy(h.data(), c->d_heap, h.size() * sizeof(int), hipMemcpyDeviceToHost));
diff --git a/uvaia_amd/csrc/host_launch.inc b/uvaia_amd/csrc/host_launch.inc
--- a/uvaia_amd/csrc/host_launch.inc
+++ b/uvaia_amd/csrc/host_launch.inc
@@ -154,6 +154,32 @@
   return 0;
 }
 
+constexpr int DERIVE_SPLIT_INTS = 3 * (5 + 9 + 17);
+inline int derive_split_offset(int nwv) { return nwv == 4 ? 0 : nwv == 8 ? 3 * 5 : 3 * (5 + 9); }
+inline void build_derive_split(const uint32_t *cls, const uint32_t *rmask, int W4, int *split)
+{
+  for (int nwv : {4, 8, 16}) {
+    int *s = split + derive_split_offset(nwv);
+    for (int v = 0; v <= nwv; v++) s[v] = (int)((long long)W4 * v / nwv);
+    int nd = 0, nr = 0, w = 0;
+    for (int v = 0; v <= nwv; v++) {
+      for (; w < s[v] * 4; w++) { nd += __builtin_popcount(cls[(size_t)w * 4 + 3]); nr += __builtin_popcount(rmask[(size_t)w]); }
+      s[nwv + 1 + v] = nd; s[2 * (nwv + 1) + v] = nr;
+    }
+  }
+}
+
+inline int planes_slot(const uvaia_gpu_ctx *c, hipStream_t st) { for (int i = 0; i < 3; i++) if (st && st == c->scan_streams[i]) return 1 + i; return 0; }
+inline void planes_touch(uvaia_gpu_ctx *c, hipStream_t st) { const int i = planes_slot(c, st); c->planes_busy[i] = true; c->planes_ev[i] = nullptr; }
+inline void planes_fenced(uvaia_gpu_ctx *c, hipStream_t st, hipEvent_t ev)
+{
+  const int i = planes_slot(c, st);
+  for (int j = 0; j < 4; j++) if (j != i && c->planes_ev[j] == ev) c->planes_ev[j] = nullptr;
+  if (c->planes_busy[i]) c->planes_ev[i] = ev;
+}
+inline void planes_idle(uvaia_gpu_ctx *c, bool main, bool scans)
+{ for (int i = 0; i < 4; i++) if (i == 0 ? main : scans) { c->planes_busy[i] = false; c->planes_ev[i] = nullptr; } }
+
 int take_scan_events(uvaia_gpu_ctx *c, ScanEvt &ev)
 {
   for (hipEvent_t *e : {&ev.a, &ev.b}) {
@@ -215,6 +241,7 @@
   }
   const uint32_t *qp = c->acgt ? c->d_qp : c->d_qp2;
   if (c->scan_variant == 2) {
+    planes_touch(c, stream);
     const int *tote = s.tote + tile_first * 64;
     constexpr int QS = 64;
     if (c->act_q0 % QS) return fail(c, UVAIA_GPU_ESTATE, "the scan works on super-tiles of %d queries: active queries start at a multiple of that", QS);
@@ -290,6 +317,8 @@
 {
   const dim3 grid(L.q1 - L.q0), block(64);
   const size_t lds = (size_t)(c->k + 1) * HEAP_ENTRY * sizeof(int);
+  c->entered_clean = 0;
+  if (L.poly) planes_touch(c, L.stream);
   if (c->fullscan) {
 #define REPLAY(A) hipLaunchKernelGGL((replay_kernel<A>), grid, block, lds, L.stream, c->d_cnt, L.ppad, c->d_rt, c->d_tr, L.nonn, L.rb, L.re, L.ord_base, c->d_heap, c->d_n, c->d_T, c->d_snap, L.entered, c->k)
     if (c->acgt) REPLAY(true); else REPLAY(false);
@@ -349,17 +378,21 @@
 {
   if (!st) st = c->stream;
   if (c->fullscan || c->scan_variant != 2 || n_ref <= 0 || !c->d_split) return 0;
+  if (st == c->stream) planes_touch(c, st);
   const long long a = slot0 / 64, t1 = (slot0 + n_ref - 1) / 64;
   const int nblk = (int)(t1 - a + 1);
-#define DERIVE_ALL(A, V) hipLaunchKernelGGL((derive_all_kernel<A, V>), dim3(nblk), dim3(256), 0, st, s.planes, a, a, c->W4, c->d_cls, c->d_rmask, c->d_split, c->NP4, c->NR4, s.ev, s.tote, s.grp, s.poly)
-  if (c->acgt) { if (v_in_place) DERIVE_ALL(true, false); else DERIVE_ALL(true, true); }
-  else         { if (v_in_place) DERIVE_ALL(false, false); else DERIVE_ALL(false, true); }
+  const int waves = c->derive_waves ? c->derive_waves : 4;
+#define DERIVE_ALL_W(A, V, N) hipLaunchKernelGGL((derive_all_kernel<A, V, N>), dim3(nblk), dim3(64 * N), 0, st, s.planes, a, a, c->W4, c->d_cls, c->d_rmask, c->d_split + derive_split_offset(N), c->NP4, c->NR4, s.ev, s.tote, s.grp, s.poly)
+#define DERIVE_ALL(A, V) { if (waves == 8) DERIVE_ALL_W(A, V, 8); else if (waves == 16) DERIVE_ALL_W(A, V, 16); else DERIVE_ALL_W(A, V, 4); }
+  if (c->acgt) { if (v_in_place) DERIVE_ALL(true, false) else DERIVE_ALL(true, true) }
+  else         { if (v_in_place) DERIVE_ALL(false, false) else DERIVE_ALL(false, true) }
 #undef DERIVE_ALL
-  HIPCHK(c, hipGetLastError());
-  return 0;
-}
-
-int sync_scan_streams(uvaia_gpu_ctx *c) { for (hipStream_t st : c->scan_streams) if (st) HIPCHK(c, hipStreamSynchronize(st)); return 0; }
+#undef DERIVE_ALL_W
+  HIPCHK(c, hipGetLastError());
+  return 0;
+}
+
+int sync_scan_streams(uvaia_gpu_ctx *c) { for (hipStream_t st : c->scan_streams) if (st) HIPCHK(c, hipStreamSynchronize(st)); planes_idle(c, false, true); return 0; }
 int sync_derive_streams(uvaia_gpu_ctx *c) { for (hipStream_t st : c->derive_streams) if (st) HIPCHK(c, hipStreamSynchronize(st)); return 0; }
 
 template <class T> int regrow(uvaia_gpu_ctx *c, T *&p, size_t n) { if (p) hipFree(p); p = nullptr; HIPCHK(c, hipMalloc(&p, n * sizeof(T))); return 0; }
@@ -412,6 +445,7 @@
   }
   { int rc = derive_rows(c, s, slot0, n_ref); if (rc) return rc; }
   HIPCHK(c, hipStreamSynchronize(c->stream));
+  planes_idle(c, true, false);
   int bad = 0;
   HIPCHK(c, hipMemcpy(&bad, c->d_err, sizeof(int), hipMemcpyDeviceToHost));
   if (bad) {
diff --git a/uvaia_amd/csrc/host_open.inc b/uvaia_amd/csrc/host_open.inc
--- a/uvaia_amd/csrc/host_open.inc
+++ b/uvaia_amd/csrc/host_open.inc
@@ -44,7 +44,8 @@
   memset(&tn, 0, sizeof tn);
   if (tune) tn = *tune;
   if (tn.scan < 0 || tn.scan > UVAIA_GPU_SCAN_WIDE || tn.query_tables < 0 || tn.query_tables > 2 || (tn.scan_tiles_per_wave != 0 && tn.scan_tiles_per_wave != 1 && tn.scan_tiles_per_wave != 2 && tn.scan_tiles_per_wave != 4) ||
-      (tn.scan_waves_per_block != 0 && tn.scan_waves_per_block != 4 && tn.scan_waves_per_block != 8) || (tn.subslice_refs != 0 && tn.subslice_refs < 64))
+      (tn.scan_waves_per_block != 0 && tn.scan_waves_per_block != 4 && tn.scan_waves_per_block != 8) || (tn.subslice_refs != 0 && tn.subslice_refs < 64) ||
+      (tn.derive_waves != 0 && tn.derive_waves != 4 && tn.derive_waves != 8 && tn.derive_waves != 16))
     return fail(nullptr, UVAIA_GPU_EINVAL, "bad tuning values");
   if (!out) return fail(nullptr, UVAIA_GPU_EINVAL, "ctx is NULL");
   *out = nullptr;
@@ -75,6 +76,7 @@
   if (tn.scan_streams > 100 && tn.scan_streams < 200) c->first_slice_pct = tn.scan_streams == 199 ? 0 : tn.scan_streams - 100;
   if (tn.pipeline == 2) c->pipeline = true;
   if (tn.head_scan == 2) c->head_full = true;
+  c->derive_waves = tn.derive_waves;
   if (tn.ball_gather == 1 || tn.ball_gather == 2) c->ball_fused = tn.ball_gather == 2;
   if (tn.rederive_streams >= 1 && tn.rederive_streams <= 3) { c->derive_nstreams = tn.rederive_streams; c->derive_forced = true; }
   if (c->nchar > 49000) c->fullscan = true;
@@ -222,13 +224,13 @@
 int uvaia_gpu_reset(uvaia_gpu_ctx *c)
 {
   if (!c) return UVAIA_GPU_EINVAL;
-  HIPCHK(c, hipMemsetAsync(c->d_heap, 0, (size_t)c->nq * (c->k + 1) * HEAP_ENTRY * sizeof(int), c->stream));
-  hipLaunchKernelGGL(init_state_kernel, dim3((c->nq + 255) / 256), dim3(256), 0, c->stream, c->d_T, c->d_n, c->nq, c->nchar);
+  const size_t heap16 = (size_t)c->nq * (c->k + 1) * HEAP_ENTRY * sizeof(int) / 16;
+  const size_t ent = (c->d_entered && c->db_n) ? std::min(c->entered_cap / 64 * 64, ((c->db_n + 63) / 64) * 64) : 0;
+  const size_t work = std::max(std::max(heap16, ent / 16), (size_t)c->nq);
+  hipLaunchKernelGGL(reset_state_kernel, dim3((unsigned)std::min<size_t>(1024, (work + 255) / 256)), dim3(256), 0, c->stream,
+                     reinterpret_cast<uint4 *>(c->d_heap), heap16, c->d_T, c->d_n, c->nq, c->nchar, c->d_snap, reinterpret_cast<uint4 *>(c->d_entered), ent / 16);
   HIPCHK(c, hipGetLastError());
-  HIPCHK(c, hipMemcpyAsync(c->d_snap, &c->nchar, sizeof(int), hipMemcpyHostToDevice, c->stream));
-  if (c->d_entered && c->db_n) HIPCHK(c, hipMemsetAsync(c->d_entered, 0, ((c->db_n + 63) / 64) * 64, c->stream));
-  if (int rc = sync_scan_streams(c)) return rc;
-  HIPCHK(c, hipStreamSynchronize(c->stream));
+  c->entered_clean = ent;
   return 0;
 }
 
diff --git a/uvaia_amd/csrc/host_qprep.inc b/uvaia_amd/csrc/host_qprep.inc
--- a/uvaia_amd/csrc/host_qprep.inc
+++ b/uvaia_amd/csrc/host_qprep.inc
@@ -87,14 +87,9 @@
   c->NR4 = ((c->NR + 31) / 32 + 3) / 4;
   if (c->scan_variant == 2 && (size_t)c->NP4 * 128 + (size_t)c->NR4 * 128 > SCAN3_BIAS - 256) c->scan_variant = 0;
   {
-    int split[15];
-    for (int v = 0; v <= 4; v++) split[v] = (int)((long long)c->W4 * v / 4);
-    for (int v = 0; v <= 4; v++) {
-      int nd = 0, nr = 0;
-      for (int w = 0; w < split[v] * 4; w++) { nd += __builtin_popcount(cls[(size_t)w * 4 + 3]); nr += __builtin_popcount(rmask[(size_t)w]); }
-      split[5 + v] = nd; split[10 + v] = nr;
-    }
-    QALLOC(c->d_split, 15, false);
+    int split[DERIVE_SPLIT_INTS];
+    build_derive_split(cls.data(), rmask.data(), c->W4, split);
+    QALLOC(c->d_split, DERIVE_SPLIT_INTS, false);
     OPENCHK(hipMemcpyAsync(c->d_split, split, sizeof split, hipMemcpyHostToDevice, s));
     OPENCHK(hipStreamSynchronize(s));
     c->qtab[9] = {c->d_split, sizeof split};
diff --git a/uvaia_amd/csrc/host_qtables.inc b/uvaia_amd/csrc/host_qtables.inc
--- a/uvaia_amd/csrc/host_qtables.inc
+++ b/uvaia_amd/csrc/host_qtables.inc
@@ -132,13 +132,8 @@
       OPENCHK(hipMalloc(&c->d_rmask, rmask.size() * 4)); OPENCHK(hipMemcpy(c->d_rmask, rmask.data(), rmask.size() * 4, hipMemcpyHostToDevice));
       c->qtab[3] = {c->d_cls, cls.size() * 4}; c->qtab[4] = {c->d_rmask, rmask.size() * 4}; c->qtab[6] = {c->d_qrare, qrare.size() * 4};
       {
-        int split[15];
-        for (int v = 0; v <= 4; v++) split[v] = (int)((long long)c->W4 * v / 4);
-        for (int v = 0; v <= 4; v++) {
-          int nd = 0, nr = 0;
-          for (int w = 0; w < split[v] * 4; w++) { nd += __builtin_popcount(cls[(size_t)w * 4 + 3]); nr += __builtin_popcount(rmask[(size_t)w]); }
-          split[5 + v] = nd; split[10 + v] = nr;
-        }
+        int split[DERIVE_SPLIT_INTS];
+        build_derive_split(cls.data(), rmask.data(), c->W4, split);
         OPENCHK(hipMalloc(&c->d_split, sizeof split)); OPENCHK(hipMemcpy(c->d_split, split, sizeof split, hipMemcpyHostToDevice));
         c->qtab[9] = {c->d_split, sizeof split};
       }
diff --git a/uvaia_amd/csrc/host_resident.inc b/uvaia_amd/csrc/host_resident.inc
--- a/uvaia_amd/csrc/host_resident.inc
+++ b/uvaia_amd/csrc/host_resident.inc
@@ -12,6 +12,7 @@
   c->db_local_tiles = dtiles;
   c->peer_db[c->shard_rank] = c->db.planes; c->peer_amb[c->shard_rank] = c->db.amb;
   c->db_cap = tiles * 64 - 64;
+  c->entered_clean = 0;
   if (c->entered_cap < tiles * 64) {
     hipFree(c->d_entered); c->d_entered = nullptr;
     HIPCHK(c, hipMalloc(&c->d_entered, tiles * 64)); c->entered_cap = tiles * 64;
@@ -112,6 +113,23 @@
   HIPCHK(c, hipMemcpy(planes, reinterpret_cast<const char *>(c->db.planes) + first_tile * tb, n_tiles * tb, hipMemcpyDeviceToHost));
   HIPCHK(c, hipMemcpy(non_n, c->db.nonn + first_tile * 64, n_tiles * 64 * sizeof(int), hipMemcpyDeviceToHost));
   HIPCHK(c, hipMemcpy(side_rows, c->db.amb + first_tile * 64 * AMB_ROW, n_tiles * 64 * AMB_ROW * sizeof(int), hipMemcpyDeviceToHost));
+  return 0;
+}
+
+int uvaia_gpu_db_derived_export(uvaia_gpu_ctx *c, size_t n_tiles, void *e, uint32_t *grp, void *poly, int *tot)
+{
+  if (!c || !e || !grp || !poly || !tot) return UVAIA_GPU_EINVAL;
+  if (c->fullscan || c->scan_variant != 2 || !c->db.ev) return fail(c, UVAIA_GPU_ESTATE, "only the column-compressed scan keeps planes derived for the query set");
+  if (c->shard_world > 1) return fail(c, UVAIA_GPU_ESTATE, "a context of a reference shard numbers its derived tiles by piece: read them from a plain context");
+  if (n_tiles * 64 > ((c->db_n + 63) / 64) * 64) return fail(c, UVAIA_GPU_EINVAL, "tiles 0..%zu lie outside the database", n_tiles);
+  if (!n_tiles) return 0;
+  { int rc = settle_derive(c); if (rc) return rc; }
+  HIPCHK(c, hipStreamSynchronize(c->stream));
+  const size_t W4 = (size_t)c->W4, NG = (size_t)(c->NP4 + c->NR4);
+  HIPCHK(c, hipMemcpy2D(e, 1024, c->db.ev, 2048, 1024, n_tiles * W4, hipMemcpyDeviceToHost));
+  HIPCHK(c, hipMemcpy(grp, c->db.grp, n_tiles * W4 * 64 * sizeof(uint32_t), hipMemcpyDeviceToHost));
+  if (NG) HIPCHK(c, hipMemcpy(poly, c->db.poly, n_tiles * NG * 3 * 64 * sizeof(uint4), hipMemcpyDeviceToHost));
+  HIPCHK(c, hipMemcpy(tot, c->db.tote, n_tiles * 64 * sizeof(int), hipMemcpyDeviceToHost));
   return 0;
 }
 
@@ -208,15 +226,6 @@
   if (!c) return UVAIA_GPU_EINVAL;
   if (!c->db.planes || !c->db_n || c->fullscan || c->scan_variant != 2) return 0;
   HIPCHK(c, hipSetDevice(c->device));
-  {
-    hipStream_t busy[4] = {c->stream, c->scan_streams[0], c->scan_streams[1], c->scan_streams[2]};
-    for (int i = 0; i < 4; i++) {
-      if (!busy[i]) continue;
-      if (!c->derive_fence[i]) HIPCHK(c, hipEventCreateWithFlags(&c->derive_fence[i], hipEventDisableTiming));
-      HIPCHK(c, hipEventRecord(c->derive_fence[i], busy[i]));
-      for (int j = 0; j < c->derive_nstreams; j++) HIPCHK(c, hipStreamWaitEvent(c->derive_streams[j], c->derive_fence[i], 0));
-    }
-  }
   std::vector<SubSlice> plan;
   if (c->shard_world == 1) plan = plan_subslices(c, 0, c->db_n, c->max_pool);
   else {
@@ -224,20 +233,33 @@
     for (size_t a = (size_t)c->shard_rank * piece; a < c->db_n; a += piece * (size_t)c->shard_world) plan.push_back({a, std::min(piece, c->db_n - a), false});
   }
   const int n_derive_streams = (c->derive_forced || plan.size() <= 3) ? c->derive_nstreams : 1;
+  {
+    hipStream_t busy[4] = {c->stream, c->scan_streams[0], c->scan_streams[1], c->scan_streams[2]};
+    for (int i = 0; i < 4; i++) {
+      if (!busy[i] || !c->planes_busy[i]) continue;
+      hipEvent_t e = c->planes_ev[i];
+      if (!e) {
+        if (!c->derive_fence[i]) HIPCHK(c, hipEventCreateWithFlags(&c->derive_fence[i], hipEventDisableTiming));
+        HIPCHK(c, hipEventRecord(c->derive_fence[i], busy[i]));
+        planes_fenced(c, busy[i], e = c->derive_fence[i]);
+      }
+      for (int j = 0; j < n_derive_streams; j++) HIPCHK(c, hipStreamWaitEvent(c->derive_streams[j], e, 0));
+    }
+  }
   size_t k = 0;
   long long t_done = 0;
   for (const SubSlice &sl : plan) {
     const long long t0 = std::max(t_done, (long long)(sl.first / 64)), t1 = (long long)((sl.first + sl.n + 63) / 64);
     if (t0 >= t1) continue;
     t_done = t1;
+    hipStream_t ds = c->derive_streams[k % (size_t)n_derive_streams];
+    int rc = for_owned_tiles(c, t0, t1, [&](long long, long long lt, long long nt) -> int { return derive_rows(c, c->db, lt * 64, (int)(nt * 64), ds, true); });
+    if (rc) return rc;
     if (k == c->derive_chunks.size()) {
       uvaia_gpu_ctx::DeriveChunk d{0, 0, nullptr};
       HIPCHK(c, hipEventCreateWithFlags(&d.done, hipEventDisableTiming));
       c->derive_chunks.push_back(d);
     }
-    hipStream_t ds = c->derive_streams[k % (size_t)n_derive_streams];
-    int rc = for_owned_tiles(c, t0, t1, [&](long long, long long lt, long long nt) -> int { return derive_rows(c, c->db, lt * 64, (int)(nt * 64), ds, true); });
-    if (rc) return rc;
     c->derive_chunks[k].t0 = t0; c->derive_chunks[k].t1 = t1;
     HIPCHK(c, hipEventRecord(c->derive_chunks[k].done, ds));
     k++;
@@ -305,7 +327,8 @@
   if (c->shard_world > 1) return fail(c, UVAIA_GPU_ESTATE, "a context of a reference shard keeps its own pieces only: use uvaia_gpu_shard_scan / uvaia_gpu_shard_replay (or a group)");
   if (pool < 1 || pool > c->max_pool) return fail(c, UVAIA_GPU_EINVAL, "pool must be in [1, max_pool=%zu]", c->max_pool);
   if (!c->db_n) return 0;
-  HIPCHK(c, hipMemsetAsync(c->d_entered, 0, ((c->db_n + 63) / 64) * 64, c->stream));
+  if (c->entered_clean < ((c->db_n + 63) / 64) * 64) HIPCHK(c, hipMemsetAsync(c->d_entered, 0, ((c->db_n + 63) / 64) * 64, c->stream));
+  c->entered_clean = 0;
   if (!c->fullscan) {
     size_t head = 0;
     if (c->scan_variant == 2 && c->head_full && c->n_idx_c == 0 && c->db_n > 4096 && !c->serial) {
@@ -352,6 +375,7 @@
   if (int rc = sync_scan_streams(c)) return rc;
   HIPCHK(c, hipStreamSynchronize(c->stream));
   if (c->rep_stream) HIPCHK(c, hipStreamSynchronize(c->rep_stream));
+  planes_idle(c, true, true);
   { int rc = pipe_check(c); if (rc) return rc; }
   return collect_events(c);
 }
@@ -506,6 +530,7 @@
   int rc = launch_scan2(c, c->db, b.tf, b.tiles, b.cnt, b.tiles * 64, bytes, ss, b.tmin, b.rb, b.re, b.rt, c->use_ext ? b.ext : nullptr, b.rtp, b.tb8, progress);
   if (rc) return rc;
   HIPCHK(c, hipEventRecord(b.scan_done, ss));
+  planes_fenced(c, ss, b.scan_done);
   return 0;
 }
 
@@ -531,6 +556,7 @@
   if (rc) return rc;
   if (rs != c->stream) { HIPCHK(c, hipEventRecord(c->rep_ev[1], rs)); HIPCHK(c, hipStreamWaitEvent(c->stream, c->rep_ev[1], 0)); }
   HIPCHK(c, hipEventRecord(b.replay_done, c->stream));
+  planes_fenced(c, c->stream, b.replay_done);
   b.replay_recorded = true;
   c->last = {&c->db, b.tf, b.tiles, b.re - b.rb, b.rb, ppad, b.rt};
   return 0;
diff --git a/uvaia_amd/csrc/kernels_replay.inc b/uvaia_amd/csrc/kernels_replay.inc
--- a/uvaia_amd/csrc/kernels_replay.inc
+++ b/uvaia_amd/csrc/kernels_replay.inc
@@ -926,10 +926,16 @@
   if (threadIdx.x == 0) *snap = red[0];
 }
 
-__global__ void init_state_kernel(int *__restrict__ T, int *__restrict__ n, int nq, int nchar)
-{
-  const int i = blockIdx.x * blockDim.x + threadIdx.x;
-  if (i < nq) { T[i] = nchar; n[i] = 0; }
+__global__ __launch_bounds__(256)
+void reset_state_kernel(uint4 *__restrict__ heap, size_t heap16, int *__restrict__ T, int *__restrict__ n, int nq, int nchar,
+                        int *__restrict__ snap, uint4 *__restrict__ entered, size_t entered16)
+{
+  const size_t stride = (size_t)gridDim.x * blockDim.x, i0 = (size_t)blockIdx.x * blockDim.x + threadIdx.x;
+  const uint4 z = make_uint4(0u, 0u, 0u, 0u);
+  for (size_t i = i0; i < heap16; i += stride) heap[i] = z;
+  for (size_t i = i0; i < entered16; i += stride) entered[i] = z;
+  for (size_t i = i0; i < (size_t)nq; i += stride) { T[i] = nchar; n[i] = 0; }
+  if (i0 == 0) *snap = nchar;
 }
 
 template <bool ACGT>
diff --git a/uvaia_amd/csrc/kernels_scan3.inc b/uvaia_amd/csrc/kernels_scan3.inc
--- a/uvaia_amd/csrc/kernels_scan3.inc
+++ b/uvaia_amd/csrc/kernels_scan3.inc
@@ -8,9 +8,10 @@
 }
 struct GatherStage { uint32_t bL, bH, bI; int fill, ow; };
 
+template <int NWV>
 static __device__ __forceinline__ int shared_slot(const int *__restrict__ bit, int word)
 {
-  for (int k = 1; k <= 3; k++) if ((bit[k] & 31) != 0 && (bit[k] >> 5) == word) return k;
+  for (int k = 1; k < NWV; k++) if ((bit[k] & 31) != 0 && (bit[k] >> 5) == word) return k;
   return 0;
 }
 static __device__ __forceinline__ uint32_t take_bit(uint32_t x, int b, int at, uint32_t acc)
@@ -18,17 +19,17 @@
   return (__builtin_amdgcn_ubfe(x, (uint32_t)b, 1u) << at) | acc;
 }
 
-template <bool ACGT, bool WRITE_V>
-__global__ __launch_bounds__(256) __attribute__((amdgpu_waves_per_eu(8, 8)))
+template <bool ACGT, bool WRITE_V, int NWV>
+__global__ __launch_bounds__(64 * NWV) __attribute__((amdgpu_waves_per_eu(8, 8)))
 void derive_all_kernel(const uint4 *__restrict__ tiles, long long tile_base, long long dtile_base, int W4,
                        const uint32_t *__restrict__ cls, const uint32_t *__restrict__ rmask,
                        const int *__restrict__ split, int NP4, int NR4,
                        uint4 *__restrict__ ev, int *__restrict__ tot_e, uint32_t *__restrict__ grp, uint4 *__restrict__ poly)
 {
   constexpr int P = ACGT ? 3 : 4;
-  __shared__ int partial[4][64];
-  __shared__ uint32_t shr[6][3][64];
-  for (int i = threadIdx.x; i < 6 * 3 * 64; i += 256) (&shr[0][0][0])[i] = 0u;
+  __shared__ int partial[NWV][64];
+  __shared__ uint32_t shr[2 * (NWV - 1)][3][64];
+  for (int i = threadIdx.x; i < 2 * (NWV - 1) * 3 * 64; i += 64 * NWV) (&shr[0][0][0])[i] = 0u;
   __syncthreads();
   const int lane = threadIdx.x & 63, wv = __builtin_amdgcn_readfirstlane(threadIdx.x >> 6);
   const long long ptile = tile_base + blockIdx.x, tile = dtile_base + blockIdx.x;
@@ -37,22 +38,24 @@
   const int NG = NP4 + NR4;
   uint32_t *po = reinterpret_cast<uint32_t *>(poly + (size_t)tile * NG * 3 * 64 + lane);
   const int lo = split[wv], hi = split[wv + 1];
-  const int *dbit = split + 5, *rbit = split + 10;
+  const int *dbit = split + (NWV + 1), *rbit = split + 2 * (NWV + 1);
 
   GatherStage D, R;
   D.bL = D.bH = D.bI = 0u; D.fill = dbit[wv] & 31; D.ow = dbit[wv] >> 5;
   R.bL = R.bH = R.bI = 0u; R.fill = rbit[wv] & 31; R.ow = rbit[wv] >> 5;
-  int sw[2][3];
+  int sw[2][2], sk[2][2];
 #pragma unroll
   for (int sec = 0; sec < 2; sec++) {
     const int *bit = sec ? rbit : dbit;
-#pragma unroll
-    for (int k = 1; k <= 3; k++) sw[sec][k - 1] = (bit[k] & 31) != 0 ? (bit[k] >> 5) : -1;
+    sw[sec][0] = (bit[wv] & 31) != 0 ? (bit[wv] >> 5) : -1;
+    sw[sec][1] = (wv + 1 < NWV && (bit[wv + 1] & 31) != 0) ? (bit[wv + 1] >> 5) : -1;
+#pragma unroll
+    for (int e = 0; e < 2; e++) sk[sec][e] = sw[sec][e] >= 0 ? shared_slot<NWV>(bit, sw[sec][e]) : 0;
   }
   auto push_word = [&](GatherStage &g, int sec) {
-    const int k = (sw[sec][0] == g.ow) ? 1 : (sw[sec][1] == g.ow) ? 2 : (sw[sec][2] == g.ow) ? 3 : 0;
+    const int k = (sw[sec][0] == g.ow) ? sk[sec][0] : (sw[sec][1] == g.ow) ? sk[sec][1] : 0;
     if (k) {
-      uint32_t (*dst)[64] = shr[sec * 3 + k - 1];
+      uint32_t (*dst)[64] = shr[sec * (NWV - 1) + k - 1];
       if (g.bL) atomicOr(&dst[0][lane], g.bL);
       if (g.bH) atomicOr(&dst[1][lane], g.bH);
       if (g.bI) atomicOr(&dst[2][lane], g.bI);
@@ -109,20 +112,22 @@
   }
   if (NP4 && D.fill > 0) push_word(D, 0);
   if (NR4 && R.fill > 0) push_word(R, 1);
-  if (wv == 3) {
-    for (int w = (dbit[4] + 31) >> 5; w < NP4 * 4; w++) { uint32_t *d = po + (size_t)(w >> 2) * 3 * 256 + (w & 3); d[0] = 0u; d[256] = 0u; d[512] = 0u; }
-    for (int w = (rbit[4] + 31) >> 5; w < NR4 * 4; w++) { uint32_t *d = po + (size_t)(NP4 + (w >> 2)) * 3 * 256 + (w & 3); d[0] = 0u; d[256] = 0u; d[512] = 0u; }
+  if (wv == NWV - 1) {
+    for (int w = (dbit[NWV] + 31) >> 5; w < NP4 * 4; w++) { uint32_t *d = po + (size_t)(w >> 2) * 3 * 256 + (w & 3); d[0] = 0u; d[256] = 0u; d[512] = 0u; }
+    for (int w = (rbit[NWV] + 31) >> 5; w < NR4 * 4; w++) { uint32_t *d = po + (size_t)(NP4 + (w >> 2)) * 3 * 256 + (w & 3); d[0] = 0u; d[256] = 0u; d[512] = 0u; }
   }
   partial[wv][lane] = te;
   __syncthreads();
-  if (wv == 0) tot_e[tile * 64 + lane] = partial[0][lane] + partial[1][lane] + partial[2][lane] + partial[3][lane];
-  else {
+  if (wv == 0) {
+    int t_all = 0;
+#pragma unroll
+    for (int v = 0; v < NWV; v++) t_all += partial[v][lane];
+    tot_e[tile * 64 + lane] = t_all;
+  } else {
     for (int sec = 0; sec < 2; sec++) {
-      const int *bit = sec ? rbit : dbit;
-      if ((sec ? NR4 : NP4) == 0 || (bit[wv] & 31) == 0) continue;
-      const int w = bit[wv] >> 5;
-      if (shared_slot(bit, w) != wv) continue;
-      const uint32_t (*src)[64] = shr[sec * 3 + wv - 1];
+      if ((sec ? NR4 : NP4) == 0 || sw[sec][0] < 0 || sk[sec][0] != wv) continue;
+      const int w = sw[sec][0];
+      const uint32_t (*src)[64] = shr[sec * (NWV - 1) + wv - 1];
       uint32_t *d = po + (size_t)((sec ? NP4 : 0) + (w >> 2)) * 3 * 256 + (w & 3);
       d[0] = src[0][lane]; d[256] = src[1][lane]; d[512] = src[2][lane];
     }
diff --git a/uvaia_amd/csrc/uvaia_gpu.hip b/uvaia_amd/csrc/uvaia_gpu.hip
--- a/uvaia_amd/csrc/uvaia_gpu.hip
+++ b/uvaia_amd/csrc/uvaia_gpu.hip
@@ -99,6 +99,7 @@
   std::vector<DeriveChunk> derive_chunks;
   hipEvent_t derive_fence[4] = {};
   size_t derive_pending = 0;
+  bool planes_busy[4] = {}; hipEvent_t planes_ev[4] = {};
   bool pipeline = false, pipeline_now = false, pipe_used = false;
   int *d_pipe_err = nullptr;
   SliceBuf slice[NBUF];
@@ -119,6 +120,7 @@
   int NR = 0, NR4 = 0, rare_max = -1;
   uint32_t *d_rmask = nullptr;
   int *d_split = nullptr;
+  int derive_waves = 0;
   int shard_rank = 0, shard_world = 1; long long shard_pt = 0;
   const uint4 *peer_db[64] = {}; const int *peer_amb[64] = {};
   void *ipc_opened[64][2] = {};
@@ -173,6 +175,7 @@
   int4 *d_rt = nullptr, *d_tr = nullptr;
   uint8_t *d_entered = nullptr;
   size_t entered_cap = 0;
+  size_t entered_clean = 0;
   uint8_t *d_stage = nullptr;
   uint8_t *h_stage = nullptr;
   hipEvent_t stage_free[2] = {}; bool stage_busy[2] = {};
```

New measurement: 34.51 million, median of 6. +4.3%, better.
